# XiaoshuiHuang/GMF

Hardware: AMD Instinct MI355X
Metric: correspondences/sec (whole node) (higher is better)
Workload: dtype f32 (split-fp16 MFMA operands, fp32 accumulate; the cross products of the attention's two contractions, S = K Q'^T and O = P V, on block-scaled e4m3 operands wherever the device-side score guard allows)

## Files before the change

### gmf_amd/_lib.py

```python
from __future__ import annotations

import collections
import ctypes as C
import os
import threading
from typing import Dict, Optional

_HERE = os.path.dirname(os.path.abspath(__file__))
LIB_PATH = os.path.join(_HERE, "libgmf_hip.so")

_f32p = C.POINTER(C.c_float)
_i32p = C.POINTER(C.c_int)
_vp = C.c_void_p
_ll = C.c_longlong


class EncoderWeights(C.Structure):
    _fields_ = [
        ("num_layers", C.c_int),
        ("f1_ctx_wst", _vp), ("f1_ctx_vec", _vp),
        ("f1_attn_wst", _vp), ("f1_attn_vec", _vp),
        ("f1_ff_wst", _vp), ("f1_ff_vec", _vp),
        ("ctx_wst", _vp), ("ctx_vec", _vp), ("ctx_wst_stride", C.c_int), ("ctx_vec_stride", C.c_int),
        ("attn_wst", _vp), ("attn_vec", _vp), ("attn_wst_stride", C.c_int), ("attn_vec_stride", C.c_int),
# ... 76 lines not shown
    "gmf_last_error_string": (C.c_char_p, [_vp]),
    "gmf_workspace_bytes": (_ll, [_vp]),
    "gmf_set_workspace": (C.c_int, [_vp, _vp, _ll]),
    "gmf_workspace_wanted": (_ll, [_vp]),
    "gmf_status_read": (C.c_int, [_vp, C.POINTER(C.c_int), C.c_int]),
    "gmf_set_tuning": (C.c_int, [_vp, C.c_char_p, C.c_int]),
    "gmf_get_tuning": (C.c_int, [_vp, C.c_char_p, C.POINTER(C.c_int)]),
    "gmf_set_sigma_device": (C.c_int, [_vp, _vp]),
    "gmf_profile_enable": (C.c_int, [_vp, C.c_int]),
    "gmf_profile_read": (C.c_int, [_vp, C.POINTER(C.c_double), C.POINTER(C.c_int)]),
    "gmf_pack_rows_p32": (C.c_int, [_vp, _vp, _ll, _ll, _ll, C.c_int, C.c_int, C.c_int, _vp, _vp]),
    "gmf_unpack_rows_p32": (C.c_int, [_vp, _vp, C.c_int, C.c_int, C.c_int, _vp, _ll, _ll, _ll, _vp]),
    "gmf_pack_pts8": (C.c_int, [_vp, _vp, _vp, C.c_int, C.c_int, _vp, _vp]),
    "gmf_front_forward": (C.c_int, [_vp, C.c_int, _vp, _vp, _vp, _vp, _vp, _vp, _vp, C.c_int, C.c_int, _vp]),
    "gmf_scattn_forward": (C.c_int, [_vp, _vp, _vp, _vp, _vp, _vp, _vp, _vp, _vp, C.c_int, C.c_int, C.c_float, _vp]),
    "gmf_scattn_forward_dense": (C.c_int, [_vp, _vp, _vp, _vp, _vp, _vp, _vp, _vp, _vp, C.c_int, C.c_int, _vp]),
    "gmf_fusion_ctx_prepare": (C.c_int, [_vp, C.c_int, _vp, _vp, _vp, _vp, C.c_int, C.c_int, C.c_int, C.c_int, C.c_int, _vp]),
    "gmf_fusion_attn_forward": (C.c_int, [_vp, C.c_int, _vp, _vp, _vp, _vp, _vp, C.c_int, C.c_int, C.c_int, _vp]),
    "gmf_fusion_ff_forward": (C.c_int, [_vp, _vp, _vp, _vp, _vp, C.c_int, C.c_int, _vp]),
    "gmf_classifier_forward": (C.c_int, [_vp, _vp, _vp, _vp, _vp, _vp, _vp, C.c_int, C.c_int, _vp]),
    "gmf_encoder_pack_weights": (C.c_int, [_vp, C.POINTER(Tensor), C.c_int, C.c_int, C.c_int, C.POINTER(_vp)]),
    "gmf_packed_encoder_weights": (C.POINTER(EncoderWeights), [_vp]),
    "gmf_packed_encoder_info": (C.c_int, [_vp, _f32p, _f32p, _i32p, _f32p]),
    "gmf_packed_encoder_free": (None, [_vp]),
    "gmf_packed_encoder_bytes": (C.c_longlong, [_vp]),
    "gmf_packed_encoder_place": (C.c_int, [_vp, _vp, _vp, C.c_longlong, _vp]),
    "gmf_fusion_pack_weights": (C.c_int, [_vp, C.POINTER(Tensor), C.c_int, C.c_char_p, C.c_int, C.c_int, C.POINTER(_vp)]),
    "gmf_packed_fusion_weights": (C.POINTER(FusionWeights), [_vp]),
    "gmf_packed_fusion_free": (None, [_vp]),
    "gmf_packed_fusion_bytes": (C.c_longlong, [_vp]),
    "gmf_packed_fusion_place": (C.c_int, [_vp, _vp, _vp, C.c_longlong, _vp]),
    "gmf_encoder_forward": (C.c_int, [_vp, C.POINTER(EncoderWeights), _vp, _vp, _vp, _vp, _vp, C.c_int, C.c_int, C.c_int,
                                      _vp, _vp, _vp, _vp]),
    "gmf_encoder_forward_ragged": (C.c_int, [_vp, C.POINTER(EncoderWeights), _vp, _vp, _vp, _vp, _vp, _i32p, C.c_int, C.c_int,
                                             _vp, _vp, _vp, _vp]),
    "gmf_pose_head_ragged": (C.c_int, [_vp, C.POINTER(PoseParams), C.c_double, _vp, _vp, _vp, _vp, _i32p, C.c_int, _vp, _vp, _vp,
                                       _vp, _vp, _vp, _vp]),
    "gmf_nonlocal_block_forward": (C.c_int, [_vp, C.POINTER(EncoderWeights), C.c_int, C.c_int, _vp, _vp, _vp, _vp, _vp,
                                             C.c_int, C.c_int, C.c_int, _vp]),
    "gmf_fusion_layer_forward": (C.c_int, [_vp, C.c_int, C.c_int, C.c_int, _vp, _vp, _vp, _vp, _vp, _vp, _vp, _vp, _ll, _ll,
                                           _ll, _vp, _ll, _ll, _ll, C.c_int, C.c_int, C.c_int, _vp, _vp, _vp, _vp]),
    "gmf_pose_head": (C.c_int, [_vp, C.POINTER(PoseParams), _vp, _vp, _vp, _vp, _vp, C.c_int, C.c_int, _vp, _vp, _vp,
                                _vp, _vp, _vp, _vp]),
    "gmf_pick_seeds": (C.c_int, [_vp, _vp, _vp, C.c_int, C.c_int, C.c_float, C.c_int, C.c_int, _vp, _vp]),
    "gmf_knn_rows": (C.c_int, [_vp, _vp, _vp, C.c_int, C.c_int, C.c_int, C.c_int, _vp, _vp]),
    "gmf_knn_from_distances": (C.c_int, [_vp, _vp, C.c_int, C.c_int, C.c_int, C.c_int, _vp, _vp]),
    "gmf_nn_match": (C.c_int, [_vp, _vp, _vp, C.c_int, C.c_int, C.c_int, C.c_int, _vp, _vp, _vp]),
    "gmf_nn_match_batched": (C.c_int, [_vp, _vp, _vp, _i32p, _i32p, C.c_int, C.c_int, C.c_int, C.c_int, _vp, _vp, _vp]),
    "gmf_nn_match_mutual_batched": (C.c_int, [_vp, _vp, _vp, _i32p, _i32p, C.c_int, C.c_int, _vp, _vp, _vp, _vp]),
    "gmf_build_correspondences": (C.c_int, [_vp, _vp, _vp, _vp, _vp, _i32p, _i32p, C.c_int, C.c_int, C.c_int, C.c_int, _vp, C.c_float,
                                            _vp, _vp, _vp, _vp, _vp, _vp, _vp, _vp, _vp]),
    "gmf_matching_indices_count": (C.c_int, [_vp, _vp, _vp, _vp, _vp, C.c_int, _ll, _ll, _vp, C.c_double, _vp, _vp, C.POINTER(_ll), _vp]),
    "gmf_matching_indices_fill": (C.c_int, [_vp, _vp, _vp, _vp, _vp, C.c_int, _ll, _ll, _vp, C.c_double, _vp, _vp, _vp]),
    "gmf_inlier_input": (C.c_int, [_vp, _vp, _vp, _vp, _vp, C.c_int, _ll, _vp, _vp, _vp, _vp, C.c_int, _vp, _vp, C.c_int, _vp, _vp, _vp,
                                   _vp, _vp, _vp]),
    "gmf_procrustes_batched": (C.c_int, [_vp, _vp, _vp, _vp, C.c_int, C.c_int, C.c_float, _vp, _vp]),
    "gmf_post_refinement": (C.c_int, [_vp, _vp, _vp, _vp, C.c_int, C.c_int, C.c_float, C.c_int, _vp, _vp]),
    "gmf_weighted_procrustes": (C.c_int, [_vp, _vp, _vp, _vp, _vp, C.c_int, C.c_float, _vp, _vp, _vp]),
    "gmf_global_registration": (C.c_int, [_vp, _vp, _vp, _vp, _vp, C.c_int, C.c_float, C.c_float, C.c_int, C.c_int,
                                          C.c_double, _vp, _vp, _vp, C.c_int, _vp]),
    "gmf_similarity_matrix": (C.c_int, [_vp, _vp, C.c_int, C.c_int, C.c_float, _vp, C.c_int, _vp]),
    "gmf_spectral_matching_loss": (C.c_int, [_vp, _vp, C.c_int, _vp, C.c_int, C.c_int, C.c_int, _vp, _vp]),
    "gmf_spectral_matching_loss_fused": (C.c_int, [_vp, _vp, _vp, C.c_int, C.c_int, C.c_float, C.c_int, _vp, _vp]),
    "gmf_spectral_matching_backward": (C.c_int, [_vp, _vp, _vp, C.c_int, C.c_int, C.c_float, C.c_int, _vp, _vp, _vp]),
    "gmf_classification_loss": (C.c_int, [_vp, _vp, _vp, _vp, C.c_int, C.c_int, C.c_int, _vp, _vp]),
    "gmf_stem_forward": (C.c_int, [_vp, _vp, _ll, _ll, _ll, _ll, _vp, _vp, _vp, C.c_int, C.c_int, C.c_int, _vp]),
# ... 228 lines not shown
```

### gmf_amd/csrc/encoder_kernels.hip

```cpp
#include <algorithm>
#include <type_traits>
#include "enc_common.hpp"
#include "enc_ff.hpp"

namespace gmf {

template <int MODE>
__global__ void __launch_bounds__(256, 2)
k_front(const float* __restrict__ in, const float* __restrict__ wst, const float* __restrict__ vecs,
        float* __restrict__ f_out, float* __restrict__ q_out, float* __restrict__ k_out,
        float* __restrict__ v_out, int N, int tiles) {
  __shared__ __attribute__((aligned(16))) float lds[2 * kStageFloats];
  const int lane = threadIdx.x & 63, wave = threadIdx.x >> 6, h = lane >> 5, i = lane & 31;
  const int pair = blockIdx.y;
  const int tile_raw = blockIdx.x * kWavesPerWG + wave;
  const bool active = tile_raw < tiles;
  const int tile = active ? tile_raw : tiles - 1;
  const size_t toff = ((size_t)pair * tiles + tile) * (32 * C);

  constexpr bool FIRST = (MODE == 1);
  StageStream ss;
  if (MODE == 2) ss.init(lds, lds + kStageFloats, wave, kWavesPerWG, lane, wst + 4 * kStageFloats, 12);
  else ss.init(lds, lds + kStageFloats, wave, kWavesPerWG, lane, wst, 16);
  ss.prime();
// ... 424 lines not shown
               const PairTab* __restrict__ ptab) {
  __shared__ float tr[kCompatLdsFloats];
  compat_build_body<FMT>(tr, blockIdx.x, blockIdx.y, blockIdx.z, pts8, c_dense, N, tiles, inv_sig2, ptab);
}

GMF_DEVINL f32x16 mma3_part(int u, f32x16 acc, f16x8 ah, f16x8 al, f16x8 bh, f16x8 bl) {
  switch (u) {
    case 0: return mfma_h16(al, bh, acc);
    case 1: return mfma_h16(ah, bl, acc);
    default: return mfma_h16(ah, bh, acc);
  }
}


struct FusTile {
  const float* tile;
  GMF_DEVINL void load(float (&fz)[16], int mb, int lane, int h) const { load_block_p32(fz, tile, mb, lane); }
};

struct FusRegs {
  const float (&f)[CF];
  GMF_DEVINL void load(float (&fz)[16], int mb, int lane, int h) const {
#pragma unroll
    for (int r = 0; r < 16; ++r) fz[r] = f[16 * mb + r];
  }
};

constexpr int kTailVecFloats = 3 * C;
GMF_DEVINL void stage_tail_vecs(float* lvec, const float* __restrict__ vecs, const float* __restrict__ next_bias, int wave, int lane) {
  if (wave == 0) dma_piece_1k(vecs, lvec, lane);
  if (wave == 1 && next_bias && lane < 32) dma_piece_1k(next_bias, lvec + 2 * C, lane);
}

template <bool NEXT_PCN, class Stages, class Fus>
GMF_DEVINL void scattn_epilogue_h2(const float (&o)[CF], const bool active, Stages& ss, const float* __restrict__ vecs,
                                   const Fus& fus_tile, float* __restrict__ out_tile, const int lane, const int h,
                                   const float* __restrict__ next_bias = nullptr,
                                   unsigned* __restrict__ stat_next = nullptr, const int pair = 0, const bool row_valid = false) {
    FragH2<8> ox, featx;
    FragH2<4> m1x, m2x;
    if (active) ox.set(o);
#pragma unroll
    for (int mb = 0; mb < 2; ++mb) {
      const f16x8* lw = as_h2(ss.acquire());
      if (!active) continue;
      f32x16 acc = zero16();
      mma_wx_h2<8>(acc, lw, ox);
      float b[16], t1[16];
      load_vec_block(b, vecs, mb, h);
#pragma unroll
      for (int r = 0; r < 16; ++r) t1[r] = relu_nan(fmaf(acc[r], kH2Inv, b[r]));
      m1x.set_block(mb, t1);
    }
    {
      const f16x8* lw = as_h2(ss.acquire());
#pragma unroll
      for (int mb = 0; mb < 2; ++mb) {
        if (!active) continue;
        f32x16 acc = zero16();
        mma_wx_h2<4>(acc, lw + mb * (2 * 4 * 64), m1x);
        float b[16], t2[16];
        load_vec_block(b, vecs + 64, mb, h);
#pragma unroll
        for (int r = 0; r < 16; ++r) t2[r] = relu_nan(fmaf(acc[r], kH2Inv, b[r]));
        m2x.set_block(mb, t2);
      }
    }
#pragma unroll
    for (int st = 0; st < 2; ++st) {
      const f16x8* lw = as_h2(ss.acquire());
#pragma unroll
      for (int hb = 0; hb < 2; ++hb) {
        if (!active) continue;
        const int mb = 2 * st + hb;
        f32x16 acc = zero16();
        mma_wx_h2<4>(acc, lw + hb * (2 * 4 * 64), m2x);
        float b[16], fz[16], tt[16];
        load_vec_block(b, vecs + 128, mb, h);
        fus_tile.load(fz, mb, lane, h);
#pragma unroll
        for (int r = 0; r < 16; ++r) tt[r] = fmaf(acc[r], kH2Inv, b[r]) + fz[r];
        if (NEXT_PCN) featx.set_block(mb, tt);
        else if (active) store_block_p32(out_tile, mb, tt, lane);
      }
    }
    if (NEXT_PCN) {
      float ssq = 0.f;
#pragma unroll
      for (int mb = 0; mb < 4; ++mb) {
        const f16x8* lw = as_h2(ss.acquire());
        if (!active) continue;
        f32x16 acc = zero16();
        mma_wx_h2<8>(acc, lw, featx);
        float b[16], tt[16];
        load_vec_block(b, next_bias, mb, h);
#pragma unroll
        for (int r = 0; r < 16; ++r) { tt[r] = relu_nan(fmaf(acc[r], kH2Inv, b[r])); ssq = fmaf(tt[r], tt[r], ssq); }
        store_block_p32(out_tile, mb, tt, lane);
      }
      if (stat_next && active) pv_stat_raise(stat_next, pair, ssq, row_valid, lane);
    }
}

struct AttnItem { int item, ks; bool split, valid; };
GMF_DEVINL AttnItem attn_item(int L, int n_items, int n_full, int ksplits) {
  const int chunk = n_items >> 3, rem = n_items & 7, xcd = L & 7, kth = L >> 3;
  const int start = (xcd < rem) ? xcd * (chunk + 1) : rem * (chunk + 1) + (xcd - rem) * chunk;
  const int items = chunk + (xcd < rem ? 1 : 0);
  const int nf = min(n_full, items);
  if (kth < nf) return AttnItem{start + kth, 0, false, true};
  const int j = kth - nf, r = j / ksplits;
  return AttnItem{start + nf + r, j - r * ksplits, true, nf + r < items};
}

constexpr float kInvU16 = 1.0f / 65535.0f;
template <int NPROD = 3, int CFMT = 0, int WAVES = 4, bool PVF8 = false>
GMF_DEVINL void scattn_h2p_body(float* lds, const int bid, const float* __restrict__ q_img, const float* __restrict__ k_img,
                                const float* __restrict__ v_img, const float* __restrict__ fus, const float* __restrict__ wst,
                                const float* __restrict__ vecs, float* out, int N, int tiles, int wgs_per_pair,
                                const float* __restrict__ c_dense, int n_items, int n_full, int ksplits,
                                float* __restrict__ part_o, float* __restrict__ part_ml, const float* __restrict__ next_wst,
                                const float* __restrict__ next_bias, const PairTab* __restrict__ ptab = nullptr,
                                const unsigned* __restrict__ v_scale = nullptr,
                                const float* qf_img = nullptr, const float* __restrict__ qw_wst = nullptr,
                                const float* __restrict__ qw_bias = nullptr,
                                unsigned* __restrict__ stat_next = nullptr) {
  static_assert(!PVF8 || NPROD == 3, "the fp8 cross products belong to the three-product form");
  float* const ldsK = lds;
  float* const ldsV = lds + 2 * kStageFloats;
  const int lane = threadIdx.x & 63, h = lane >> 5;
  const int wave = __builtin_amdgcn_readfirstlane(threadIdx.x >> 6);
  const unsigned lane_off16 = lane * 16;
  const AttnItem it = attn_item(bid, n_items, n_full, ksplits);
  if (!it.valid) return;
  const bool split = it.split;
  const int ks = it.ks;
  const int slot = it.item / wgs_per_pair, qblock = it.item - slot * wgs_per_pair;
  const int pair = ptab ? ptab[slot].ord : slot;
  if (ptab) N = ptab[pair].n;
  const int tiles_p = ptab ? (N + 31) >> 5 : tiles;
  if (qblock * WAVES >= tiles_p) return;
  const int t_begin = split ? (tiles_p * ks) / ksplits : 0;
  const int t_end = split ? (tiles_p * (ks + 1)) / ksplits : tiles_p;
  const int tile_raw = qblock * WAVES + wave;
  const bool active = tile_raw < tiles_p;
  const int tile = active ? tile_raw : tiles_p - 1;
  const size_t pbase = (size_t)pair * tiles;
  const size_t toff = (pbase + tile) * (32 * C);

  f16x8 qh[8], ql[8];
  if (NPROD == 3 && WAVES == 4 && qf_img) {
    FragH2<8> fx;
    {
      float fq[CF];
      load_frag_p32<CF>(fq, qf_img + toff, lane);
      fx.set(fq);
    }
#pragma unroll
    for (int st = 0; st < 4; ++st) dma_4k_s(qw_wst + st * kStageFloats + wave * 1024, lds + st * kStageFloats + wave * 1024, lane_off16);
    asm volatile("s_waitcnt vmcnt(0)" ::: "memory");
// ... 418 lines not shown
      tile_step(t, s_a, s_b);
      tile_step(t + 1, s_b, s_a);
    }
    if (t + 1 < t_end) { tile_step(t, s_a, s_b); tile_last(t + 1, s_b); }
    else tile_last(t, s_a);
    }
  }
  if (split) {
    if (active) {
      float of[CF];
#pragma unroll
      for (int db = 0; db < 4; ++db)
#pragma unroll
        for (int r = 0; r < 16; ++r) of[16 * db + r] = oacc[db][r];
      const size_t n_tiles_all = (size_t)(n_items / wgs_per_pair) * tiles;
      const size_t pt = (size_t)ks * n_tiles_all + pbase + tile;
      store_frag_p32<CF>(part_o + pt * (32 * C), of, lane);
      const float lsum = xhalf_sum(l_half);
      if (h == 0) { part_ml[(pt * 32 + (lane & 31)) * 2] = m_run; part_ml[(pt * 32 + (lane & 31)) * 2 + 1] = lsum; }
    }
    return;
  }

  float o[CF];
  {
    const float inv = 1.0f / xhalf_sum(l_half);
#pragma unroll
    for (int db = 0; db < 4; ++db)
#pragma unroll
      for (int r = 0; r < 16; ++r) o[16 * db + r] = oacc[db][r] * inv;
  }
  __syncthreads();
  float* const lvec = lds + 2 * kStageFloats;
  stage_tail_vecs(lvec, vecs, next_wst ? next_bias : nullptr, wave, lane);
  StageStream ss;
  ss.init(lds, lds + kStageFloats, wave, WAVES, lane, wst, 5, next_wst, next_wst ? 4 : 0);
  ss.prime();
  const FusTile ft{fus + toff};
  if (next_wst) scattn_epilogue_h2<true>(o, active, ss, lvec, ft, out + toff, lane, h, lvec + 2 * C, stat_next, pair,
                                         tile_raw * 32 + (lane & 31) < N);
  else scattn_epilogue_h2<false>(o, active, ss, lvec, ft, out + toff, lane, h);
}

GMF_DEVINL bool attn_pv_on(const unsigned* __restrict__ v_scale, const PvGuard& guard, int bid, int n_items, int n_full, int ksplits,
                           int wgs_per_pair, const PairTab* __restrict__ ptab = nullptr) {
  if (!guard.stat) return v_scale != nullptr;
  const AttnItem it = attn_item(bid, n_items, n_full, ksplits);
  const int slot = it.valid ? it.item / wgs_per_pair : 0;
  return pv_planes_on(v_scale, guard, ptab ? ptab[slot].ord : slot);
}

template <int NPROD, int CFMT, bool PVF8 = false>
__global__ void __launch_bounds__(256, 2)
k_scattn_h2p(const float* __restrict__ q_img, const float* __restrict__ k_img, const float* __restrict__ v_img,
             const float* __restrict__ fus, const float* __restrict__ wst, const float* __restrict__ vecs,
             float* out, int N, int tiles, int wgs_per_pair, const float* __restrict__ c_dense,
             int n_items, int n_full, int ksplits, float* __restrict__ part_o, float* __restrict__ part_ml,
             const float* __restrict__ next_wst, const float* __restrict__ next_bias, const PairTab* __restrict__ ptab,
             const unsigned* __restrict__ v_scale, const float* qf_img, const float* __restrict__ qw_wst,
             const float* __restrict__ qw_bias, const PvGuard guard) {
  __shared__ __attribute__((aligned(16))) float lds[4 * kStageFloats];
  tail_priority(blockIdx.x, gridDim.x);
  if (!PVF8 || attn_pv_on(v_scale, guard, blockIdx.x, n_items, n_full, ksplits, wgs_per_pair, ptab))
    scattn_h2p_body<NPROD, CFMT, 4, PVF8>(lds, blockIdx.x, q_img, k_img, v_img, fus, wst, vecs, out, N, tiles, wgs_per_pair, c_dense, n_items,
                                          n_full, ksplits, part_o, part_ml, next_wst, next_bias, ptab, v_scale, qf_img, qw_wst, qw_bias,
                                          guard.stat_next);
  else
    scattn_h2p_body<NPROD, CFMT, 4, false>(lds, blockIdx.x, q_img, k_img, v_img, fus, wst, vecs, out, N, tiles, wgs_per_pair, c_dense, n_items,
                                           n_full, ksplits, part_o, part_ml, next_wst, next_bias, ptab, nullptr, qf_img, qw_wst, qw_bias,
                                           guard.stat_next);
}

__global__ void __launch_bounds__(256, 2)
k_scattn_fast(const float* __restrict__ q_img, const float* __restrict__ k_img, const float* __restrict__ v_img,
              const float* __restrict__ fus, const float* __restrict__ wst, const float* __restrict__ vecs,
              float* __restrict__ out, int N, int tiles, int wgs_per_pair, const float* __restrict__ c_half, int n_items,
              const float* __restrict__ next_wst, const float* __restrict__ next_bias) {
  constexpr int WAVES = 4;
  constexpr int kHiFloats = kStageFloats / 2;
  constexpr int kCFloats = 512;
  __shared__ __attribute__((aligned(16))) float lds[6 * kHiFloats + WAVES * 3 * kCFloats];
  float* const ldsK = lds;
  float* const ldsV = lds + 3 * kHiFloats;
  const int lane = threadIdx.x & 63, h = lane >> 5;
  const int wave = __builtin_amdgcn_readfirstlane(threadIdx.x >> 6);
  float* const ldsC = lds + 6 * kHiFloats + wave * 3 * kCFloats;
  const unsigned lane_off16 = lane * 16;
  const AttnItem it = attn_item(blockIdx.x, n_items, 0x7fffffff, 1);
  if (!it.valid) return;
  const int pair = it.item / wgs_per_pair, qblock = it.item - pair * wgs_per_pair;
  const int tile_raw = qblock * WAVES + wave;
  const bool active = tile_raw < tiles;
  const int tile = active ? tile_raw : tiles - 1;
  const size_t pbase = (size_t)pair * tiles;
  const size_t toff = (pbase + tile) * (32 * C);

  f16x8 qh[8];
  {
    const f16x8* qp = reinterpret_cast<const f16x8*>(q_img + (pbase + tile) * (size_t)kStageFloats) + lane;
#pragma unroll
    for (int s = 0; s < 8; ++s) qh[s] = qp[s * 64];
  }
  const float* gc = c_half + ((pbase + tile) * (size_t)tiles) * kCFloats;
// ... 121 lines not shown
  if (next_wst) scattn_epilogue_h2<true>(o, active, ss, lvec, ft, out + toff, lane, h, lvec + 2 * C);
  else scattn_epilogue_h2<false>(o, active, ss, lvec, ft, out + toff, lane, h);
}

template <int CFMT, bool PVF8 = false>
__global__ void __launch_bounds__(256, 2)
k_small_attn_ff(const int n_attn, const float* __restrict__ q_img, const float* __restrict__ k_img,
                const float* __restrict__ v_img, const float* __restrict__ tail_wst, const float* __restrict__ tail_vecs, int N,
                int tiles, int wgs_per_pair, const float* __restrict__ c_dense, int n_items, int ksplits,
                float* __restrict__ part_o, float* __restrict__ part_ml, const float* __restrict__ x1,
                const float* __restrict__ ff_wst, const float* __restrict__ ff_vecs, float* __restrict__ ff_part, int n_pairs,
                int ff_hs, const unsigned* __restrict__ v_scale, const PvGuard guard,
                const PairTab* __restrict__ ptab) {
  __shared__ __attribute__((aligned(16))) float lds[4 * kStageFloats];
  if ((int)blockIdx.x < n_attn) {
    if (!PVF8 || attn_pv_on(v_scale, guard, blockIdx.x, n_items, 0, ksplits, wgs_per_pair, ptab))
      scattn_h2p_body<3, CFMT, 4, PVF8>(lds, blockIdx.x, q_img, k_img, v_img, x1, tail_wst, tail_vecs, ff_part, N, tiles, wgs_per_pair, c_dense,
                                        n_items, 0, ksplits, part_o, part_ml, nullptr, nullptr, ptab, v_scale);
    else
      scattn_h2p_body<3, CFMT, 4, false>(lds, blockIdx.x, q_img, k_img, v_img, x1, tail_wst, tail_vecs, ff_part, N, tiles, wgs_per_pair, c_dense,
                                         n_items, 0, ksplits, part_o, part_ml, nullptr, nullptr, ptab, nullptr);
  } else {
    const int id = (int)blockIdx.x - n_attn;
    const int z = id % ff_hs, r = id / ff_hs;
    const int pair = r / wgs_per_pair, bx = r - pair * wgs_per_pair;
    if (ptab && bx * 4 >= ((ptab[pair].n + 31) >> 5)) return;
    fusion_ff_h2p_body<true>(lds, bx, pair, n_pairs, z, ff_hs, x1, ff_wst, ff_vecs, ff_part, tiles, ff_part);
  }
}

struct StagesPreloaded {
  const float* base;
  int used, lane;
  GMF_DEVINL void init(float* lds, int wave, int lane_, const float* g, int n_stages, const float* g2 = nullptr) {
    base = lds; used = 0; lane = lane_;
    for (int st = 0; st < n_stages; ++st)
#pragma unroll
      for (int q = 0; q < 4; ++q)
        dma_piece_1k(g + (size_t)st * kStageFloats + (wave + 4 * q) * 256, lds + st * kStageFloats + (wave + 4 * q) * 256, lane_);
    if (g2)
      for (int st = 0; st < 4; ++st)
#pragma unroll
        for (int q = 0; q < 4; ++q)
          dma_piece_1k(g2 + (size_t)st * kStageFloats + (wave + 4 * q) * 256, lds + (n_stages + st) * kStageFloats + (wave + 4 * q) * 256, lane_);
  }
  GMF_DEVINL const float4* acquire() {
    if (used == 0) {
      asm volatile("s_waitcnt vmcnt(0)" ::: "memory");
      __syncthreads();
    }
    const float* cur = base + used * kStageFloats;
    ++used;
    return reinterpret_cast<const float4*>(cur) + lane;
  }
};

__global__ void __launch_bounds__(256, 1)
k_scattn_merge(const float* __restrict__ part_o, const float* __restrict__ part_ml, const float* __restrict__ fus,
               const float* __restrict__ wst, const float* __restrict__ vecs, float* __restrict__ out, int tiles,
               int wgs_per_pair, int n_items, int n_full, int ksplits, const float* __restrict__ next_wst,
               const float* __restrict__ next_bias, const float* __restrict__ ff_part, int ff_hs, const float* __restrict__ x1,
               const float* __restrict__ ff_b2, unsigned* __restrict__ stat_next, int n_rows,
               const PairTab* __restrict__ ptab = nullptr) {
  __shared__ __attribute__((aligned(16))) float lds[9 * kStageFloats + kTailVecFloats];
  const int lane = threadIdx.x & 63, h = lane >> 5, i = lane & 31;
  const int wave = __builtin_amdgcn_readfirstlane(threadIdx.x >> 6);
  const AttnItem it = attn_item(blockIdx.x + 8 * min(n_full, (n_items >> 3) + ((int)(blockIdx.x & 7) < (n_items & 7) ? 1 : 0)),
                                n_items, n_full, 1);
  if (!it.valid) return;
  const int slot = it.item / wgs_per_pair;
  const int pair = ptab ? ptab[slot].ord : slot;
  if (ptab) n_rows = ptab[pair].n;
  const int tiles_p = ptab ? (n_rows + 31) >> 5 : tiles;
  if ((it.item - slot * wgs_per_pair) * 4 >= tiles_p) return;
  const int tile_raw = (it.item - slot * wgs_per_pair) * 4 + wave;
  const bool active = tile_raw < tiles_p;
  const int tile = active ? tile_raw : tiles_p - 1;
  const size_t n_tiles_all = (size_t)(n_items / wgs_per_pair) * tiles;
  const size_t pt0 = (size_t)pair * tiles + tile;
  const size_t toff = pt0 * (32 * C);
  float* const lvec = lds + 9 * kStageFloats;
  stage_tail_vecs(lvec, vecs, next_wst ? next_bias : nullptr, wave, lane);
  vecs = lvec;
  next_bias = lvec + 2 * C;
  StagesPreloaded ss;
  ss.init(lds, wave, lane, wst, 5, next_wst);
  float x2[CF];
  if (ff_part) {
    const float* pt = ff_part + toff;
    const size_t zs = n_tiles_all * (32 * C);
    float acc[CF], xr[CF];
    load_frag_p32<CF>(acc, pt, lane);
    load_frag_p32<CF>(xr, x1 + toff, lane);
    for (int z = 1; z < ff_hs; ++z) {
      float pz[CF];
      load_frag_p32<CF>(pz, pt + (size_t)z * zs, lane);
#pragma unroll
      for (int e = 0; e < CF; ++e) acc[e] += pz[e];
    }
#pragma unroll
    for (int mb = 0; mb < 4; ++mb) {
      float b[16];
      load_vec_block(b, ff_b2, mb, h);
#pragma unroll
      for (int r = 0; r < 16; ++r) x2[16 * mb + r] = fmaf(acc[16 * mb + r], kH2Inv, b[r]) + xr[16 * mb + r];
    }
  }
  float mk[8], lk[8];
  float M = -INFINITY;
#pragma unroll
  for (int k = 0; k < 8; ++k) {
    mk[k] = -INFINITY; lk[k] = 0.f;
    if (k < ksplits) {
      const float2 ml = *reinterpret_cast<const float2*>(part_ml + ((k * n_tiles_all + pt0) * 32 + i) * 2);
      mk[k] = ml.x; lk[k] = ml.y;
    }
  }
#pragma unroll
  for (int k = 0; k < 8; ++k) M = fmaxf(M, mk[k]);
  float o[CF];
#pragma unroll
  for (int e = 0; e < CF; ++e) o[e] = 0.f;
  float l = 0.f;
#pragma unroll
  for (int k0 = 0; k0 < 8; k0 += 4) {
    if (k0 >= ksplits) break;
    float ok[4][CF];
#pragma unroll
    for (int j = 0; j < 4; ++j)
      if (k0 + j < ksplits) load_frag_p32<CF>(ok[j], part_o + ((k0 + j) * n_tiles_all + pt0) * (32 * C), lane);
#pragma unroll
    for (int j = 0; j < 4; ++j) {
      if (k0 + j < ksplits) {
        const float wk = __builtin_amdgcn_exp2f(mk[k0 + j] - M);
        l = fmaf(lk[k0 + j], wk, l);
#pragma unroll
        for (int e = 0; e < CF; ++e) o[e] = fmaf(ok[j][e], wk, o[e]);
      }
    }
  }
  const float inv = 1.0f / l;
#pragma unroll
  for (int e = 0; e < CF; ++e) o[e] *= inv;
  if (ff_part) {
    const FusRegs fp{x2};
    if (next_wst) scattn_epilogue_h2<true>(o, active, ss, vecs, fp, out + toff, lane, h, next_bias, stat_next, pair, tile_raw * 32 + i < n_rows);
    else scattn_epilogue_h2<false>(o, active, ss, vecs, fp, out + toff, lane, h);
    return;
  }
  const FusTile ft{fus + toff};
  if (next_wst) scattn_epilogue_h2<true>(o, active, ss, vecs, ft, out + toff, lane, h, next_bias, stat_next, pair, tile_raw * 32 + i < n_rows);
  else scattn_epilogue_h2<false>(o, active, ss, vecs, ft, out + toff, lane, h);
}

__global__ void __launch_bounds__(256, 1)
k_scattn_merge_tile(const float* __restrict__ part_o, const float* __restrict__ part_ml, const float* __restrict__ wst,
                    const float* __restrict__ vecs, float* __restrict__ out, int tiles, int ksplits,
                    const float* __restrict__ next_wst, const float* __restrict__ next_bias, const float* __restrict__ ff_part,
                    int ff_hs, const float* __restrict__ x1, const float* __restrict__ ff_b2, unsigned* __restrict__ stat_next,
                    int n_rows,
                    const PairTab* __restrict__ ptab) {
  __shared__ __attribute__((aligned(16))) float lds[10 * kStageFloats];
  const int lane = threadIdx.x & 63, h = lane >> 5, i = lane & 31;
  const int wave = __builtin_amdgcn_readfirstlane(threadIdx.x >> 6);
  const int tile = blockIdx.x, pair = blockIdx.y;
  if (ptab) {
    n_rows = ptab[pair].n;
    if (tile >= ((n_rows + 31) >> 5)) return;
  }
  const size_t n_tiles_all = (size_t)gridDim.y * tiles;
  const size_t pt0 = (size_t)pair * tiles + tile;
  const size_t toff = pt0 * (32 * C);
  float* const xch = lds + 9 * kStageFloats;
  f16x8* const xh = reinterpret_cast<f16x8*>(xch);
  StagesPreloaded ss;
  ss.init(lds, wave, lane, wst, 5, next_wst);
// ... 383 lines not shown
  float w3[16];
  load_vec_block(w3, vecs + 64, 0, h);
  float part = 0.f;
#pragma unroll
  for (int r = 0; r < 16; ++r) part = fmaf(h2[r], w3[r], part);
  const float logit = xhalf_sum(part) + vecs[96];

  float ss2 = 0.f;
#pragma unroll
  for (int k = 0; k < CF; ++k) ss2 = fmaf(x[k], x[k], ss2);
  const float nrm2 = xhalf_sum(ss2);
  const bool bad_row = not_finite(nrm2);
  flag_status(status, active && row < N && (not_finite(logit) || bad_row), 1);
  const float inv = 1.0f / fmaxf(sqrtf(nrm2), 1e-12f);

  if (active && row < N) {
    const size_t ro = row0 + row;
    if (h == 0) logits[ro] = logit;
    float4* pn = reinterpret_cast<float4*>(feat_n + ro * C) + h;
#pragma unroll
    for (int g = 0; g < CF / 4; ++g)
      pn[2 * g] = bad_row ? make_float4(0.f, 0.f, 0.f, 0.f)
                          : make_float4(x[4 * g] * inv, x[4 * g + 1] * inv, x[4 * g + 2] * inv, x[4 * g + 3] * inv);
    if (feat_rm) {
      float4* pr = reinterpret_cast<float4*>(feat_rm + ro * C) + h;
#pragma unroll
      for (int g = 0; g < CF / 4; ++g) pr[2 * g] = make_float4(x[4 * g], x[4 * g + 1], x[4 * g + 2], x[4 * g + 3]);
    }
  }
}

__global__ void __launch_bounds__(256, 2)
k_seed_dist(const float* __restrict__ featn_img, const int* __restrict__ seeds, float* __restrict__ dist,
            int N, int tiles, int S, int chunks, const PairTab* __restrict__ ptab) {
  __shared__ __attribute__((aligned(16))) float lds[4 * kStageFloats];
  const int lane = threadIdx.x & 63, h = lane >> 5, i = lane & 31;
  const int wave = __builtin_amdgcn_readfirstlane(threadIdx.x >> 6);
  const int pair = blockIdx.y / chunks, chunk = blockIdx.y - pair * chunks;
  const int Nmax = N, Smax = S;
  N = pair_rows(ptab, pair, N);
  S = ptab ? ptab[pair].S : S;
  const int tiles_p = (N + 31) >> 5;
  if ((int)blockIdx.x * kWavesPerWG * 32 >= S) return;
  const int per = (tiles_p + chunks - 1) / chunks;
  const int t0 = chunk * per, t1 = min(tiles_p, t0 + per);
  const int seed_base = (blockIdx.x * kWavesPerWG + wave) * 32;
  const float* pair_img = featn_img + (size_t)pair * tiles * (32 * C);
  const int my = seed_base + i;
  const int row = (my < S) ? seeds[(size_t)pair * Smax + my] : 0;
  if (t0 >= t1) return;
  FragH2<8> sx;
  {
    const f16x8* rp = reinterpret_cast<const f16x8*>(pair_img + (size_t)(row >> 5) * kStageFloats) + h * 32 + (row & 31);
#pragma unroll
    for (int s8 = 0; s8 < 8; ++s8) { sx.h[s8] = rp[(0 * 8 + s8) * 64]; sx.l[s8] = rp[(1 * 8 + s8) * 64]; }
  }

  StageRing<4> ss;
  ss.init(lds, wave, lane, pair_img + (size_t)t0 * kStageFloats, t1 - t0);
  ss.prime();
  const int ld = tiles * 32;
  float* drow = dist + ((size_t)pair * Smax + seed_base + i) * ld + 4 * h;
  for (int t = t0; t < t1; ++t) {
    const f16x8* lk = as_h2(ss.acquire());
    f32x16 acc = zero16();
#pragma unroll
    for (int s8 = 0; s8 < 8; ++s8) {
      const f16x8 kh = lk[(0 * 8 + s8) * 64], kl = lk[(1 * 8 + s8) * 64];
// ... 112 lines not shown
}

hipError_t launch_scattn_fp32(const float* q, const float* k, const float* v, const float* pts8, const float* fus,
                              const float* wst, const float* vecs, float* out, int B, int N, int tiles, float sigma_d,
                              hipStream_t s) {
  hipLaunchKernelGGL(k_scattn<false>, tile_grid(tiles, B), dim3(256), 0, s, q, k, v, pts8, fus, wst, vecs, out, N, tiles,
                     1.0f / (sigma_d * sigma_d));
  return hipGetLastError();
}

hipError_t launch_small_attn_ff_merge(const float* q, const float* k, const float* v, const float* x1, const float* ff_wst,
                                      const float* ff_vecs, float* ff_part, int ff_hs, const float* tail_vecs, float* out, int B,
                                      int N, int tiles, int ksplits, hipStream_t s, const CompatCache* cc, bool tile_merge) {
  const int wpp = (tiles + 3) / 4, W = wpp * B;
  const int per_xcd = (W >> 3) + ((W & 7) ? 1 : 0);
  const int n_attn = 8 * per_xcd * ksplits, n_ff = W * ff_hs;
  if (cc->fmt == 2 && cc->v_scale)
    hipLaunchKernelGGL((k_small_attn_ff<2, true>), dim3(n_attn + n_ff), dim3(256), 0, s, n_attn, q, k, v, cc->tail_wst_h2, tail_vecs, N, tiles, wpp,
                       cc->dense, W, ksplits, cc->part_o, cc->part_ml, x1, ff_wst, ff_vecs, ff_part, B, ff_hs, cc->v_scale, cc->guard, cc->ptab);
  else if (cc->fmt == 2)
    hipLaunchKernelGGL(k_small_attn_ff<2>, dim3(n_attn + n_ff), dim3(256), 0, s, n_attn, q, k, v, cc->tail_wst_h2, tail_vecs, N, tiles, wpp,
                       cc->dense, W, ksplits, cc->part_o, cc->part_ml, x1, ff_wst, ff_vecs, ff_part, B, ff_hs, (const unsigned*)nullptr, PvGuard{}, cc->ptab);
  else if (cc->v_scale)
    hipLaunchKernelGGL((k_small_attn_ff<0, true>), dim3(n_attn + n_ff), dim3(256), 0, s, n_attn, q, k, v, cc->tail_wst_h2, tail_vecs, N, tiles, wpp,
                       cc->dense, W, ksplits, cc->part_o, cc->part_ml, x1, ff_wst, ff_vecs, ff_part, B, ff_hs, cc->v_scale, cc->guard, cc->ptab);
  else
    hipLaunchKernelGGL(k_small_attn_ff<0>, dim3(n_attn + n_ff), dim3(256), 0, s, n_attn, q, k, v, cc->tail_wst_h2, tail_vecs, N, tiles, wpp,
                       cc->dense, W, ksplits, cc->part_o, cc->part_ml, x1, ff_wst, ff_vecs, ff_part, B, ff_hs, (const unsigned*)nullptr, PvGuard{}, cc->ptab);
  if (tile_merge)
    hipLaunchKernelGGL(k_scattn_merge_tile, dim3(tiles, B), dim3(256), 0, s, cc->part_o, cc->part_ml, cc->tail_wst_h2, tail_vecs, out,
                       tiles, ksplits, cc->next_wst_h2, cc->next_bias, (const float*)ff_part, ff_hs, x1, ff_vecs + 2 * C + 2 * FFH,
                       cc->guard.stat_next, N, cc->ptab);
  else
    hipLaunchKernelGGL(k_scattn_merge, dim3(8 * per_xcd), dim3(256), 0, s, cc->part_o, cc->part_ml, x1, cc->tail_wst_h2, tail_vecs, out,
                       tiles, wpp, W, 0, ksplits, cc->next_wst_h2, cc->next_bias, (const float*)ff_part, ff_hs, x1,
                       ff_vecs + 2 * C + 2 * FFH, cc->guard.stat_next, N, cc->ptab);
  return hipGetLastError();
}

hipError_t launch_scattn_h2p(const float* q, const float* k, const float* v, const float* fus, const float* vecs, float* out, int B,
                             int N, int tiles, hipStream_t s, const CompatCache& cc, int n_full, int ksplits) {
  const int wpp = (tiles + 3) / 4, W = wpp * B;
  const int per_xcd = (W >> 3) + ((W & 7) ? 1 : 0);
  const int max_tail = std::max(0, per_xcd - n_full);
  const dim3 grid(8 * (std::min(n_full, per_xcd) + max_tail * ksplits));
  if (cc.half && max_tail == 0)
    hipLaunchKernelGGL(k_scattn_fast, dim3(8 * per_xcd), dim3(256), 0, s, q, k, v, fus, cc.tail_wst_h2, vecs, out, N, tiles, wpp, cc.dense, W,
                       cc.next_wst_h2, cc.next_bias);
  else if (cc.half)
    hipLaunchKernelGGL((k_scattn_h2p<1, 1>), grid, dim3(256), 0, s, q, k, v, fus, cc.tail_wst_h2, vecs, out, N, tiles, wpp, cc.dense, W,
                       n_full, ksplits, cc.part_o, cc.part_ml, cc.next_wst_h2, cc.next_bias, cc.ptab, (const unsigned*)nullptr, (const float*)nullptr, (const float*)nullptr, (const float*)nullptr, PvGuard{});
  else if (cc.fmt == 2 && cc.v_scale)
    hipLaunchKernelGGL((k_scattn_h2p<3, 2, true>), grid, dim3(256), 0, s, q, k, v, fus, cc.tail_wst_h2, vecs, out, N, tiles, wpp, cc.dense,
                       W, n_full, ksplits, cc.part_o, cc.part_ml, cc.next_wst_h2, cc.next_bias, cc.ptab, cc.v_scale, cc.qf_img, cc.qw_wst, cc.qw_bias, cc.guard);
  else if (cc.fmt == 2)
    hipLaunchKernelGGL((k_scattn_h2p<3, 2>), grid, dim3(256), 0, s, q, k, v, fus, cc.tail_wst_h2, vecs, out, N, tiles, wpp, cc.dense,
                       W, n_full, ksplits, cc.part_o, cc.part_ml, cc.next_wst_h2, cc.next_bias, cc.ptab, (const unsigned*)nullptr, cc.qf_img, cc.qw_wst, cc.qw_bias, PvGuard{});
  else if (cc.v_scale)
    hipLaunchKernelGGL((k_scattn_h2p<3, 0, true>), grid, dim3(256), 0, s, q, k, v, fus, cc.tail_wst_h2, vecs, out, N, tiles, wpp, cc.dense,
                       W, n_full, ksplits, cc.part_o, cc.part_ml, cc.next_wst_h2, cc.next_bias, cc.ptab, cc.v_scale, cc.qf_img, cc.qw_wst, cc.qw_bias, cc.guard);
  else
    hipLaunchKernelGGL((k_scattn_h2p<3, 0>), grid, dim3(256), 0, s, q, k, v, fus, cc.tail_wst_h2, vecs, out, N, tiles, wpp, cc.dense,
                       W, n_full, ksplits, cc.part_o, cc.part_ml, cc.next_wst_h2, cc.next_bias, cc.ptab, (const unsigned*)nullptr, cc.qf_img, cc.qw_wst, cc.qw_bias, PvGuard{});
  if (max_tail > 0)
    hipLaunchKernelGGL(k_scattn_merge, dim3(8 * max_tail), dim3(256), 0, s, cc.part_o, cc.part_ml, fus, cc.tail_wst_h2, vecs, out,
                       tiles, wpp, W, n_full, ksplits, cc.next_wst_h2, cc.next_bias, (const float*)nullptr, 0,
                       (const float*)nullptr, (const float*)nullptr, cc.guard.stat_next, N, cc.ptab);
  return hipGetLastError();
}

hipError_t launch_scattn_h2(const float* q, const float* k, const float* v, const float* pts8, const float* fus, const float* wst,
                            const float* vecs, float* out, int B, int N, int tiles, float sigma_d, hipStream_t s, const float* c_dense) {
  const float inv = 1.0f / (sigma_d * sigma_d);
  const int wpp = (tiles + 3) / 4;
  if (c_dense) hipLaunchKernelGGL(k_scattn_h2<true>, dim3(wpp * B), dim3(256), 0, s, q, k, v, pts8, fus, wst, vecs, out, N, tiles, inv, wpp, c_dense);
  else hipLaunchKernelGGL(k_scattn_h2<false>, dim3(wpp * B), dim3(256), 0, s, q, k, v, pts8, fus, wst, vecs, out, N, tiles, inv, wpp, c_dense);
  return hipGetLastError();
}

hipError_t launch_scattn_dense(const float* q, const float* k, const float* v, const float* compat, const float* fus,
                               const float* wst, const float* vecs, float* out, int B, int N, int tiles, hipStream_t s) {
  hipLaunchKernelGGL(k_scattn<true>, tile_grid(tiles, B), dim3(256), 0, s, q, k, v, compat, fus, wst, vecs, out, N, tiles, 0.f);
  return hipGetLastError();
}

hipError_t launch_ctx_prep(bool pe, const float* ctx, const float* wst, const float* vecs, float* out, int B, int T,
                           int ttiles, int sets, int wst_stride, int vec_stride, hipStream_t s) {
  if (pe) hipLaunchKernelGGL(k_ctx_prep<true>, tile_grid(ttiles, B, sets), dim3(256), 0, s, ctx, wst, vecs, out, T, ttiles, wst_stride, vec_stride);
  else hipLaunchKernelGGL(k_ctx_prep<false>, tile_grid(ttiles, B, sets), dim3(256), 0, s, ctx, wst, vecs, out, T, ttiles, wst_stride, vec_stride);
  return hipGetLastError();
}

hipError_t launch_fusion_attn(bool pe, const float* x, const float* ctx_img, const float* wst, const float* vecs,
                              float* x1, int B, int N, int tiles, int T, int ttiles, hipStream_t s) {
  if (pe) hipLaunchKernelGGL(k_fusion_attn<true>, tile_grid(tiles, B), dim3(256), 0, s, x, ctx_img, wst, vecs, x1, N, tiles, T, ttiles);
  else hipLaunchKernelGGL(k_fusion_attn<false>, tile_grid(tiles, B), dim3(256), 0, s, x, ctx_img, wst, vecs, x1, N, tiles, T, ttiles);
  return hipGetLastError();
}

hipError_t launch_fusion_ff(const float* x1, const float* wst, const float* vecs, float* x2, int B, int tiles, hipStream_t s) {
  hipLaunchKernelGGL(k_fusion_ff, tile_grid(tiles, B), dim3(256), 0, s, x1, wst, vecs, x2, tiles);
  return hipGetLastError();
}

hipError_t launch_head(const float* feat_img, const float* wst, const float* vecs, float* logits, float* feat_n,
                       float* feat_rm, int B, int N, int tiles, hipStream_t s, int* status, const PairTab* ptab, const unsigned* pv_stat,
                       const float* pv_thr2, int n_layers) {
  hipLaunchKernelGGL(k_head, tile_grid(tiles, B), dim3(256), 0, s, feat_img, wst, vecs, logits, feat_n, feat_rm, N, tiles, status, ptab,
                     pv_stat, pv_thr2, n_layers);
  return hipGetLastError();
}

hipError_t launch_seed_dist(const float* featn_img, const int* seeds, float* dist, int B, int N, int S, hipStream_t s, const PairTab* ptab) {
  const int tiles = (N + 31) / 32;
  const int sblocks = (S + 127) / 128;
  int chunks = 1;
  while (chunks < 16 && sblocks * B * chunks < 1024 && tiles / (2 * chunks) >= 4) chunks *= 2;
  hipLaunchKernelGGL(k_seed_dist, dim3(sblocks, B * chunks), dim3(256), 0, s, featn_img, seeds, dist, N, tiles, S, chunks, ptab);
  return hipGetLastError();
}

hipError_t launch_pack_p32(const float* src, float* dst, int B, int n_rows, int K, long sb, long sr, long sk, hipStream_t s, const PairTab* ptab) {
  const int tiles = (n_rows + 31) / 32;
  const long total4 = (long)B * tiles * (K / 8) * 64;
  hipLaunchKernelGGL(k_pack_p32, dim3((unsigned)((total4 + 255) / 256)), dim3(256), 0, s, src, dst, n_rows, tiles, K, sb, sr, sk, total4, ptab);
  return hipGetLastError();
}

hipError_t launch_pack_rows_h2(const float* src, float* dst, int B, int n_rows, hipStream_t s, const PairTab* ptab, const float* copy_src,
                               float* copy_dst, long n_copy) {
  const int tiles = (n_rows + 31) / 32;
  const long total = (long)B * tiles * 8 * 64;
  if (!copy_src || !copy_dst) n_copy = 0;
  if (n_copy > total) return hipErrorInvalidValue;
  hipLaunchKernelGGL(k_pack_rows_h2, dim3((unsigned)((total + 255) / 256)), dim3(256), 0, s, src, dst, n_rows, tiles, total, ptab, copy_src,
                     copy_dst, n_copy);
  return hipGetLastError();
}

hipError_t launch_unpack_p32(const float* src, float* dst, int B, int n_rows, int K, long sb, long sr, long sk, hipStream_t s, int* status) {
  const int tiles = (n_rows + 31) / 32;
  const long total4 = (long)B * tiles * (K / 8) * 64;
  hipLaunchKernelGGL(k_unpack_p32, dim3((unsigned)((total4 + 255) / 256)), dim3(256), 0, s, src, dst, n_rows, tiles, K, sb, sr, sk, total4, status);
  return hipGetLastError();
}

hipError_t launch_pack_pts8(const float* src, const float* tgt, float* dst, int B, int N, hipStream_t s, const PairTab* ptab,
                            unsigned* zero_words, int n_zero) {
  const int Npad = ((N + 31) / 32) * 32;
  const long total = (long)B * Npad;
  hipLaunchKernelGGL(k_pack_pts8, dim3((unsigned)((std::max(total, (long)n_zero) + 255) / 256)), dim3(256), 0, s, src, tgt, dst, N, Npad, total, ptab,
// ... 6 lines not shown
```

### gmf_amd/csrc/gmf_api.cpp

```cpp
#include "../../include/gmf_hip.h"

#include <hip/hip_runtime.h>

#include <cmath>
#include <cstdint>
#include <cstdio>
#include <algorithm>
#include <cstring>
#include <new>
#include <string>
#include <utility>
#include <vector>

#include "api_common.hpp"
#include "launchers_pose.hpp"
#include "launchers_solvers.hpp"
#include "launchers_spectral.hpp"
#include "launchers_pointcloud.hpp"
#include "launchers_sparse.hpp"
#include "launchers_dgr_input.hpp"
#include "launchers_correspondence.hpp"
#include "launchers_posegraph.hpp"

namespace {
// ... 195 lines not shown
    t.wide_attn_tile = value != 0;
    return GMF_OK;
  }
  if (std::strcmp(name, "small_merge_tile") == 0) {
    GMF_REQUIRE(value == 0 || value == 1, GMF_ERR_BAD_ARG, "set_tuning: small_merge_tile must be 0 or 1");
    t.small_merge_tile = value != 0;
    return GMF_OK;
  }
  if (std::strcmp(name, "mid_grid_roles") == 0) {
    GMF_REQUIRE(value >= 0 && value <= 4096, GMF_ERR_BAD_ARG, "set_tuning: mid_grid_roles out of range (0..4096)");
    t.mid_grid_roles = value;
    return GMF_OK;
  }
  if (std::strcmp(name, "q_in_attention") == 0) {
    GMF_REQUIRE(value == 0 || value == 1, GMF_ERR_BAD_ARG, "set_tuning: q_in_attention must be 0 or 1");
    t.q_in_attention = value != 0;
    return GMF_OK;
  }
  if (std::strcmp(name, "pv_fp8") == 0) {
    GMF_REQUIRE(value >= 0 && value <= 2, GMF_ERR_BAD_ARG, "set_tuning: pv_fp8 must be 0 (three f16 products), 1 (guarded, default) or 2 (always)");
    t.pv_fp8 = value;
    return GMF_OK;
  }
  if (std::strcmp(name, "compat_format") == 0) {
    GMF_REQUIRE(value == 0 || value == 2, GMF_ERR_BAD_ARG, "set_tuning: compat_format must be 0 (fp32) or 2 (16-bit fixed point of c)");
    t.compat_format = value;
    return GMF_OK;
  }
  if (std::strcmp(name, "precision") == 0) {
    GMF_REQUIRE(value >= 0 && value <= 2, GMF_ERR_BAD_ARG, "set_tuning: precision must be 0 (parity), 1 or 2 (throughput numerics)");
    t.precision = value;
    return GMF_OK;
  }
  if (std::strcmp(name, "spectral_col_splits") == 0) {
    GMF_REQUIRE(value >= 0 && value <= gmf::kSmMaxSplits, GMF_ERR_BAD_ARG, "set_tuning: spectral_col_splits out of range (0..32)");
    t.spectral_col_splits = value;
    return GMF_OK;
  }
  return fail(h, GMF_ERR_BAD_ARG, std::string("gmf: set_tuning: unknown knob ") + name);
}

int gmf_get_tuning(gmf_handle* h, const char* name, int* value) {
  GMF_REQUIRE(h && name && value, GMF_ERR_BAD_ARG, "get_tuning: null pointer");
  std::lock_guard<std::mutex> lock(h->mu);
  const gmf::Tuning& t = h->tune;
  const struct { const char* name; int v; } tab[] = {
      {"scattn_variant", t.scattn_variant}, {"front_output_split", t.front_split ? 1 : 0}, {"ff_hidden_splits", t.ff_split},
      {"attn_key_splits", t.key_splits}, {"attn_tail_split", t.tail_split ? 1 : 0}, {"small_grid_roles", t.small_roles ? 1 : 0},
      {"fused_linear", t.fused_linear ? 1 : 0}, {"compat_cache", t.use_cache ? 1 : 0}, {"conv_lds_patch", t.conv_patch}, {"conv_small_grid", t.conv_small ? 1 : 0}, {"small_prologue_roles", t.small_prologue ? 1 : 0}, {"small_fattn_tile", t.small_fattn_tile ? 1 : 0},
      {"nms_binned", t.nms_binned}, {"topk_select", t.topk_select ? 1 : 0}, {"wide_attn_tile", t.wide_attn_tile ? 1 : 0},
      {"small_merge_tile", t.small_merge_tile ? 1 : 0}, {"mid_grid_roles", t.mid_grid_roles}, {"pv_fp8", t.pv_fp8}, {"q_in_attention", t.q_in_attention ? 1 : 0},
      {"compat_format", t.compat_format}, {"precision", t.precision}, {"spectral_col_splits", t.spectral_col_splits}};
  for (const auto& e : tab) {
    if (std::strcmp(name, e.name) == 0) { *value = e.v; return GMF_OK; }
  }
  return fail(h, GMF_ERR_BAD_ARG, std::string("gmf: get_tuning: unknown knob ") + name);
}

int gmf_profile_enable(gmf_handle* h, int on) {
  GMF_REQUIRE(h, GMF_ERR_BAD_ARG, "profile_enable: null handle");
  h->profile = (on != 0);
  h->prof_used = 0;
  return GMF_OK;
}

int gmf_profile_read(gmf_handle* h, double* scattn_ms_total, int* scattn_launches) {
  GMF_REQUIRE(h && scattn_ms_total && scattn_launches, GMF_ERR_BAD_ARG, "profile_read: null pointer");
  SetDevice sd(h);
  double total = 0.0;
  for (size_t i = 0; i < h->prof_used; ++i) {
    GMF_HIP(hipEventSynchronize(h->prof_events[i].second));
    float ms = 0.f;
    GMF_HIP(hipEventElapsedTime(&ms, h->prof_events[i].first, h->prof_events[i].second));
    total += ms;
  }
  *scattn_ms_total = total;
  *scattn_launches = (int)h->prof_used;
  h->prof_used = 0;
  return GMF_OK;
}

void gmf_destroy(gmf_handle* h) {
  if (!h) return;
  for (auto& e : h->prof_events) { (void)hipEventDestroy(e.first); (void)hipEventDestroy(e.second); }
  int prev = -1;
// ... 313 lines not shown
    std::stable_sort(by_len.begin(), by_len.end(), [&](int a, int c) { return n_points[a] > n_points[c]; });
    const int runs = B < 8 ? 1 : 8;
    std::vector<std::vector<int>> run(runs);
    std::vector<double> load(runs, 0.0);
    std::vector<int> cap(runs);
    for (int r = 0; r < runs; ++r) cap[r] = B / runs + (r < B % runs ? 1 : 0);
    for (int b : by_len) {
      int best = -1;
      for (int r = 0; r < runs; ++r)
        if ((int)run[r].size() < cap[r] && (best < 0 || load[r] < load[best])) best = r;
      run[best].push_back(b);
      load[best] += (double)n_points[b] * (double)n_points[b];
    }
    int slot_i = 0;
    for (int r = 0; r < runs; ++r)
      for (int b : run[r]) tab[slot_i++].ord = b;
  }
  *n_max = nm;
  *n_sum = row;
  if (s_max) *s_max = sm;
  return GMF_OK;
}

static int upload_pair_table(gmf_handle* h, gmf::PairTab* dtab, int B, hipStream_t st) {
  gmf_handle::PtabSlot& slot = h->ptab_ring[h->ptab_cur];
  GMF_HIP(hipMemcpyAsync(dtab, slot.host, (size_t)B * sizeof(gmf::PairTab), hipMemcpyHostToDevice, st));
  GMF_HIP(hipEventRecord(slot.ev, st));
  slot.pending = true;
  return GMF_OK;
}

static int encoder_forward_impl(gmf_handle* h, const gmf_encoder_weights* w, const float* corr_pos, const float* src_keypts,
                                const float* tgt_keypts, const float* p_tokens, const float* q_tokens, int B, int N, int T,
                                float* logits, float* feat_n, float* feat, gmf_stream_t stream, const int* n_points);

int gmf_encoder_forward(gmf_handle* h, const gmf_encoder_weights* w, const float* corr_pos, const float* src_keypts,
                        const float* tgt_keypts, const float* p_tokens, const float* q_tokens, int B, int N, int T,
                        float* logits, float* feat_n, float* feat, gmf_stream_t stream) {
  GMF_REQUIRE(h, GMF_ERR_BAD_ARG, "encoder_forward: null handle");
  GMF_REQUIRE(B > 0 && N > 0 && T > 0, GMF_ERR_UNSUPPORTED_SHAPE, "encoder_forward: empty input");
  return encoder_forward_impl(h, w, corr_pos, src_keypts, tgt_keypts, p_tokens, q_tokens, B, N, T, logits, feat_n, feat, stream, nullptr);
}

int gmf_encoder_forward_ragged(gmf_handle* h, const gmf_encoder_weights* w, const float* corr_pos, const float* src_keypts,
                               const float* tgt_keypts, const float* p_tokens, const float* q_tokens, const int* n_points, int B,
                               int T, float* logits, float* feat_n, float* feat, gmf_stream_t stream) {
  GMF_REQUIRE(h, GMF_ERR_BAD_ARG, "encoder_forward_ragged: null handle");
  GMF_REQUIRE(n_points, GMF_ERR_BAD_ARG, "encoder_forward_ragged: null n_points");
  GMF_REQUIRE(B > 0 && T > 0, GMF_ERR_UNSUPPORTED_SHAPE, "encoder_forward_ragged: empty input");
  return encoder_forward_impl(h, w, corr_pos, src_keypts, tgt_keypts, p_tokens, q_tokens, B, 0, T, logits, feat_n, feat, stream, n_points);
}

static int encoder_forward_impl(gmf_handle* h, const gmf_encoder_weights* w, const float* corr_pos, const float* src_keypts,
                                const float* tgt_keypts, const float* p_tokens, const float* q_tokens, int B, int N, int T,
                                float* logits, float* feat_n, float* feat, gmf_stream_t stream, const int* n_points) {
  if (int rc = check_weights(h, w)) return rc;
  GMF_REQUIRE(corr_pos && src_keypts && tgt_keypts && p_tokens && q_tokens && logits && feat_n, GMF_ERR_BAD_ARG,
              "encoder_forward: null pointer");
  SetDevice sd(h, stream);
  hipStream_t st = S(stream);
  const bool ragged = n_points != nullptr;
  int min_tiles = 0;
  if (ragged) {
    long long n_sum = 0;
    if (int rc = build_pair_table(h, n_points, B, -1.0, 0, &N, &n_sum, nullptr)) return rc;
    min_tiles = tiles_of(*std::min_element(n_points, n_points + B));
  }
  const int L = w->num_layers;
  const int tiles = tiles_of(N), tt = tiles_of(T);
  const EncoderPlan p = plan_encoder(h->tune, w, B, N, T, L, min_tiles, cu_count());
  GMF_REQUIRE(p.fused() || !ragged, GMF_ERR_UNSUPPORTED_SHAPE,
              "encoder_forward_ragged: ragged batches run on the default path only (split-fp16 weight images, at least two layers, the "
              "compat cache, \"fused_linear\" = 1, \"scattn_variant\" = 18)");
  const size_t act = p.act, tok = p.tok;
  gmf::PairTab* ptab;
  float *featA, *featB, *f, *q, *k, *v, *x1, *x2, *pts8, *pimg, *qimg, *f1ctx, *x1t, *imgfeat, *ctxall, *c_dense, *ff_part, *part_o,
      *part_ml;
  unsigned *v_scale, *fstat;
  if (int rc = arena_carve(h, {arena_buf(ptab, ragged ? (size_t)B : 0), arena_buf(featA, act), arena_buf(featB, act), arena_buf(f, act),
                               arena_buf(q, act), arena_buf(k, act), arena_buf(v, act), arena_buf(x1, act), arena_buf(x2, act),
                               arena_buf(pts8, (size_t)B * tiles * 32 * 8), arena_buf(pimg, tok), arena_buf(qimg, tok),
                               arena_buf(f1ctx, tok), arena_buf(x1t, tok), arena_buf(imgfeat, tok),
                               arena_buf(ctxall, (size_t)(L > 0 ? L : 1) * tok),
                               arena_buf(v_scale, (size_t)B * tiles * 128),
                               arena_buf(fstat, (size_t)(L + 1) * B * gmf::kPvStatStride),
                               arena_buf(c_dense, p.cache_floats),
                               arena_buf(ff_part, p.max_splits == 8 ? 8 * act : 0),
                               arena_buf(part_o, p.max_splits * act),
// ... 12 lines not shown
                                    zero_words, n_zero));
    GMF_HIP(gmf::launch_pro_fattn_compat(q_tokens, f1ctx, w->f1_attn_wst_h2, w->f1_attn_vec, x1t, B, T, tt, pts8, c_dense, N, tiles,
                                         w->sigma_d, st, ptab));
    gmf::PvGuard g0;
    if (p.guard) g0.stat_next = fstat;
    GMF_HIP(gmf::launch_pro_ff_front(x1t, w->f1_ff_wst_h2, w->f1_ff_vec, imgfeat, B, tt, part_o, p.f1_ff_hs, corr_pos, w->front_wst_h2,
                                     w->front_vec, f, q, k, v, N, tiles, st, ptab, g0));
    if (p.f1_ff_hs > 1) GMF_HIP(gmf::launch_ff_reduce_h2(part_o, x1t, w->f1_ff_vec, imgfeat, B, tt, p.f1_ff_hs, st));
    GMF_HIP(gmf::launch_ctx_prep_h2(true, imgfeat, w->ctx_wst_h2, w->ctx_vec, ctxall, B, T, tt, L, w->ctx_wst_stride, w->ctx_vec_stride, st));
  } else {
    if (p.f1_h2) {
      GMF_HIP(gmf::launch_ctx_prep_h2(false, p_tokens, w->f1_ctx_wst_h2, w->f1_ctx_vec, f1ctx, B, T, tt, 1, 0, 0, st, true));
      GMF_HIP(gmf::launch_fusion_attn_h2(false, q_tokens, f1ctx, w->f1_attn_wst_h2, w->f1_attn_vec, x1t, B, T, tt, T, tt, st, true));
      GMF_HIP(gmf::launch_fusion_ff_h2(x1t, w->f1_ff_wst_h2, w->f1_ff_vec, imgfeat, B, tt, st, part_o, p.f1_ff_hs));
    } else {
      GMF_HIP(gmf::launch_pack_p32(p_tokens, pimg, B, T, kC, (long)T * kC, kC, 1, st));
      GMF_HIP(gmf::launch_pack_p32(q_tokens, qimg, B, T, kC, (long)T * kC, kC, 1, st));
      GMF_HIP(gmf::launch_ctx_prep(false, pimg, w->f1_ctx_wst, w->f1_ctx_vec, f1ctx, B, T, tt, 1, 0, 0, st));
      GMF_HIP(gmf::launch_fusion_attn(false, qimg, f1ctx, w->f1_attn_wst, w->f1_attn_vec, x1t, B, T, tt, T, tt, st));
      GMF_HIP(gmf::launch_fusion_ff(x1t, w->f1_ff_wst, w->f1_ff_vec, imgfeat, B, tt, st));
    }
    if (L > 0) {
      if (p.form != EncoderPlan::kFp32) GMF_HIP(gmf::launch_ctx_prep_h2(true, imgfeat, w->ctx_wst_h2, w->ctx_vec, ctxall, B, T, tt, L,
                                                                         w->ctx_wst_stride, w->ctx_vec_stride, st));
      else GMF_HIP(gmf::launch_ctx_prep(true, imgfeat, w->ctx_wst, w->ctx_vec, ctxall, B, T, tt, L, w->ctx_wst_stride,
                                        w->ctx_vec_stride, st));
    }
    GMF_HIP(gmf::launch_pack_pts8(src_keypts, tgt_keypts, pts8, B, N, st, ptab, zero_words, n_zero));
    if (p.cache) GMF_HIP(gmf::launch_compat_build(pts8, c_dense, B, N, tiles, w->sigma_d, p.fmt, st, ptab));
  }

  float* cur = featA;
  float* nxt = featB;
  if (p.fused()) {
    if (!p.prologue) {
      gmf::PvGuard g0;
      if (p.guard) g0.stat_next = fstat;
      GMF_HIP(gmf::launch_front_h2(3, p.front_split, corr_pos, w->front_wst_h2, w->front_vec, f, q, k, v, B, N, tiles, st, ptab, nullptr, g0));
    }
    for (int l = 0; l < L; ++l) {
      cc.guard = gmf::PvGuard{};
      if (p.guard) cc.guard = gmf::PvGuard{fstat + (size_t)l * B * gmf::kPvStatStride, w->pv_guard + l, fstat + (size_t)(l + 1) * B * gmf::kPvStatStride};
      const float* fw = w->front_wst_h2 + (size_t)l * w->front_wst_stride;
      const float* fv = w->front_vec + (size_t)l * w->front_vec_stride;
      const float* aw = w->attn_wst_h2 + (size_t)l * w->attn_wst_stride;
      const float* av = w->attn_vec + (size_t)l * w->attn_vec_stride;
      const float* ffw = w->ff_wst_h2 + (size_t)l * w->ff_wst_stride;
      const float* ffv = w->ff_vec + (size_t)l * w->ff_vec_stride;
      const float* ctx_l = ctxall + (size_t)l * tok;
      const bool last = (l + 1 == L);
      cc.tail_wst_h2 = w->tail_wst_h2 + (size_t)l * w->tail_wst_stride;
      cc.next_wst_h2 = last ? nullptr : w->front_wst_h2 + (size_t)(l + 1) * w->front_wst_stride;
      cc.next_bias = last ? nullptr : w->front_vec + (size_t)(l + 1) * w->front_vec_stride;
      if (p.form == EncoderPlan::kLinear) {
        cc.qf_img = p.q_in_attn ? f : nullptr;
        cc.qw_wst = p.q_in_attn ? fw + 4 * kTileFloats : nullptr;
        cc.qw_bias = p.q_in_attn ? fv + kC : nullptr;
        GMF_HIP(gmf::launch_linear_h2(p.roles, f, fw, fv, ctx_l, aw, av, ffw, ffv, p.q_in_attn ? nullptr : q, k, v, x2, B, N, tiles, T, tt,
                                      st, p.one_product, ptab, cc.v_scale, cc.guard));
      } else if (p.form == EncoderPlan::kSmall3) {
        GMF_HIP(gmf::launch_small_front_fattn(f, fw, fv, ctx_l, aw, av, q, k, v, x1, B, N, tiles, T, tt, st, cc.v_scale, cc.guard,
                                              h->tune.small_fattn_tile, ptab));
        hipEvent_t e0 = nullptr, e1 = nullptr;
        if (int rc = prof_begin(h, st, &e0, &e1)) return rc;
        GMF_HIP(gmf::launch_small_attn_ff_merge(q, k, v, x1, ffw, ffv, ff_part, p.ff_hs, w->tail_vec + (size_t)l * w->tail_vec_stride,
                                                last ? cur : f, B, N, tiles, p.attn_ks, st, &cc, h->tune.small_merge_tile));
        if (e1) GMF_HIP(hipEventRecord(e1, st));
        continue;
      } else {
        GMF_HIP(gmf::launch_front_h2(2, p.front_split, f, fw, fv, f, q, k, v, B, N, tiles, st, nullptr, cc.v_scale, cc.guard));
        GMF_HIP(gmf::launch_fusion_attn_h2(true, f, ctx_l, aw, av, x1, B, N, tiles, T, tt, st));
        GMF_HIP(gmf::launch_fusion_ff_h2(x1, ffw, ffv, x2, B, tiles, st, part_o, p.ff_hs));
      }
      if (int rc = run_scattn(h, w, p, l, q, k, v, pts8, x2, last ? cur : f, B, N, st, nullptr, cc)) return rc;
    }
    GMF_HIP(gmf::launch_head(cur, w->head_wst, w->head_vec, logits, feat_n, feat, B, N, tiles, st, h->status_dev, ptab,
                             p.guard ? fstat : nullptr, p.guard ? w->pv_guard : nullptr, L));
    return GMF_OK;
  }
  if (L == 0) {
    GMF_HIP(gmf::launch_front(1, corr_pos, w->front_wst, w->front_vec, cur, q, k, v, B, N, tiles, st));
  }
  for (int l = 0; l < L; ++l) {
    const float* in = (l == 0) ? corr_pos : cur;
    if (p.form == EncoderPlan::kStages)
      GMF_HIP(gmf::launch_front_h2(l == 0 ? 1 : 0, p.front_split, in, w->front_wst_h2 + (size_t)l * w->front_wst_stride,
                                   w->front_vec + (size_t)l * w->front_vec_stride, f, q, k, v, B, N, tiles, st));
    else GMF_HIP(gmf::launch_front(l == 0 ? 1 : 0, in, w->front_wst + (size_t)l * w->front_wst_stride,
                                   w->front_vec + (size_t)l * w->front_vec_stride, f, q, k, v, B, N, tiles, st));
    cc.tail_wst_h2 = w->tail_wst_h2 ? w->tail_wst_h2 + (size_t)l * w->tail_wst_stride : nullptr;
    if (int rc = run_block_tail(h, w, p, l, f, q, k, v, pts8, ctxall + (size_t)l * tok, x1, x2, nxt, B, N, T, st, nullptr, cc)) return rc;
    float* t = cur; cur = nxt; nxt = t;
  }
  GMF_HIP(gmf::launch_head(cur, w->head_wst, w->head_vec, logits, feat_n, feat, B, N, tiles, st, h->status_dev));
  return GMF_OK;
}

int gmf_nonlocal_block_forward(gmf_handle* h, const gmf_encoder_weights* w, int layer, int apply_pointcn,
                               const float* feat_img, const float* pts8, const float* attention,
                               const float* image_feat_img, float* out_img, int B, int N, int T, gmf_stream_t stream) {
  GMF_REQUIRE(h, GMF_ERR_BAD_ARG, "nonlocal_block_forward: null handle");
  if (int rc = check_weights(h, w)) return rc;
  GMF_REQUIRE(feat_img && image_feat_img && out_img, GMF_ERR_BAD_ARG, "nonlocal_block_forward: null pointer");
  GMF_REQUIRE((pts8 != nullptr) != (attention != nullptr), GMF_ERR_BAD_ARG, "nonlocal_block_forward: pass exactly one of pts8 / attention");
  GMF_REQUIRE(layer >= 0 && layer < w->num_layers, GMF_ERR_BAD_ARG, "nonlocal_block_forward: layer out of range");
  GMF_REQUIRE(B > 0 && N > 0 && T > 0, GMF_ERR_UNSUPPORTED_SHAPE, "nonlocal_block_forward: empty input");
  GMF_REQUIRE(apply_pointcn == 0 || apply_pointcn == 1, GMF_ERR_BAD_ARG, "nonlocal_block_forward: bad flag");
  SetDevice sd(h, stream);
  hipStream_t st = S(stream);
  const int tiles = tiles_of(N), tt = tiles_of(T);
  const EncoderPlan p = plan_encoder(h->tune, w, B, N, T, 1, 0, cu_count(), attention != nullptr);
  float *f, *q, *k, *v, *x1, *x2, *ctx;
  if (int rc = arena_carve(h, {arena_buf(f, p.act), arena_buf(q, p.act), arena_buf(k, p.act), arena_buf(v, p.act), arena_buf(x1, p.act),
                               arena_buf(x2, p.act), arena_buf(ctx, p.tok)}))
    return rc;
  if (p.form == EncoderPlan::kStages) {
    GMF_HIP(gmf::launch_front_h2(apply_pointcn ? 0 : 2, p.front_split, feat_img, w->front_wst_h2 + (size_t)layer * w->front_wst_stride,
                                 w->front_vec + (size_t)layer * w->front_vec_stride, f, q, k, v, B, N, tiles, st));
    GMF_HIP(gmf::launch_ctx_prep_h2(true, image_feat_img, w->ctx_wst_h2 + (size_t)layer * w->ctx_wst_stride,
                                    w->ctx_vec + (size_t)layer * w->ctx_vec_stride, ctx, B, T, tt, 1, 0, 0, st));
  } else {
    GMF_HIP(gmf::launch_front(apply_pointcn ? 0 : 2, feat_img, w->front_wst + (size_t)layer * w->front_wst_stride,
                              w->front_vec + (size_t)layer * w->front_vec_stride, f, q, k, v, B, N, tiles, st));
    GMF_HIP(gmf::launch_ctx_prep(true, image_feat_img, w->ctx_wst + (size_t)layer * w->ctx_wst_stride,
                                 w->ctx_vec + (size_t)layer * w->ctx_vec_stride, ctx, B, T, tt, 1, 0, 0, st));
  }
  gmf::CompatCache cc{nullptr, w->tail_wst_h2 ? w->tail_wst_h2 + (size_t)layer * w->tail_wst_stride : nullptr, nullptr, nullptr};
  return run_block_tail(h, w, p, layer, f, q, k, v, pts8, ctx, x1, x2, out_img, B, N, T, st, attention, cc);
// ... 49 lines not shown
    if (ff_wst_h2 && ff_hs_w > 1) {
      GMF_HIP(gmf::launch_fusion_ff_w_h2(x1, ff_wst_h2, ff_vec, x2, B, tiles, st, ff_part_w, ff_hs_w, out, o_sb, o_sr, o_sk, N, h->status_dev));
      return GMF_OK;
    }
    if (ff_wst_h2) GMF_HIP(gmf::launch_fusion_ff_w_h2(x1, ff_wst_h2, ff_vec, x2, B, tiles, st, ff_part_w, ff_hs_w));
    else GMF_HIP(gmf::launch_fusion_ff_w(x1, ff_wst, ff_vec, x2, B, tiles, st));
  }
  GMF_HIP(gmf::launch_unpack_p32(x2, out, B, N, latent_dim, o_sb, o_sr, o_sk, st, h->status_dev));
  return GMF_OK;
}

int gmf_pick_seeds(gmf_handle* h, const float* src_keypts, const float* scores, int B, int N, float nms_radius,
                   int use_nms, int num_seeds, int* seeds_out, gmf_stream_t stream) {
  GMF_REQUIRE(h && src_keypts && scores && seeds_out, GMF_ERR_BAD_ARG, "pick_seeds: null pointer");
  GMF_REQUIRE(B > 0 && N > 0 && num_seeds > 0 && num_seeds <= N, GMF_ERR_UNSUPPORTED_SHAPE, "pick_seeds: need 0 < num_seeds <= N");
  GMF_REQUIRE((size_t)num_seeds * 8 <= 156 * 1024, GMF_ERR_UNSUPPORTED_SHAPE, "pick_seeds: more than 19968 seeds (the winners' list lives in the LDS)");
  SetDevice sd(h, stream);
  hipStream_t st = S(stream);
  const float* keys = scores;
  float *kbuf, *scr;
  if (int rc = arena_carve(h, {arena_buf(kbuf, use_nms ? (size_t)B * N : 0), arena_buf(scr, use_nms ? gmf::nms_scratch_floats(B, N) : 0)}))
    return rc;
  if (use_nms) {
    GMF_HIP(gmf::launch_nms_keys(h->tune, src_keypts, scores, kbuf, B, N, nms_radius, st, scr));
    keys = kbuf;
  }
  GMF_HIP(gmf::launch_sort_topk(h->tune, keys, seeds_out, B, N, num_seeds, st));
  return GMF_OK;
}

static int pose_head_impl(gmf_handle* h, const gmf_pose_params* p, const float* feat_n, const float* src_keypts,
                          const float* tgt_keypts, const float* logits, const int* seeds_in, int B, int N, float* final_trans,
                          float* final_labels, int* seeds_out, int* knn_out, float* seed_trans, float* fitness,
                          gmf_stream_t stream, const int* n_points, double ratio);

int gmf_pose_head(gmf_handle* h, const gmf_pose_params* p, const float* feat_n, const float* src_keypts,
                  const float* tgt_keypts, const float* logits, const int* seeds_in, int B, int N, float* final_trans,
                  float* final_labels, int* seeds_out, int* knn_out, float* seed_trans, float* fitness,
                  gmf_stream_t stream) {
  GMF_REQUIRE(h && p, GMF_ERR_BAD_ARG, "pose_head: null pointer");
  GMF_REQUIRE(B > 0 && N > 1, GMF_ERR_UNSUPPORTED_SHAPE, "pose_head: need N > 1");
  return pose_head_impl(h, p, feat_n, src_keypts, tgt_keypts, logits, seeds_in, B, N, final_trans, final_labels, seeds_out, knn_out,
                        seed_trans, fitness, stream, nullptr, 0.0);
}

int gmf_pose_head_ragged(gmf_handle* h, const gmf_pose_params* p, double ratio, const float* feat_n, const float* src_keypts,
                         const float* tgt_keypts, const float* logits, const int* n_points, int B, float* final_trans,
                         float* final_labels, int* seeds_out, int* knn_out, float* seed_trans, float* fitness,
                         gmf_stream_t stream) {
  GMF_REQUIRE(h && p && n_points, GMF_ERR_BAD_ARG, "pose_head_ragged: null pointer");
  GMF_REQUIRE(B > 0, GMF_ERR_UNSUPPORTED_SHAPE, "pose_head_ragged: empty batch");
  GMF_REQUIRE(ratio > 0.0 && ratio <= 1.0, GMF_ERR_BAD_ARG, "pose_head_ragged: ratio must be in (0, 1]");
  GMF_REQUIRE(logits, GMF_ERR_BAD_ARG, "pose_head_ragged: the seeds come from the logits (no caller-provided seeds)");
  return pose_head_impl(h, p, feat_n, src_keypts, tgt_keypts, logits, nullptr, B, 0, final_trans, final_labels, seeds_out, knn_out,
                        seed_trans, fitness, stream, n_points, ratio);
}

static int pose_head_impl(gmf_handle* h, const gmf_pose_params* p, const float* feat_n, const float* src_keypts,
                          const float* tgt_keypts, const float* logits, const int* seeds_in, int B, int N, float* final_trans,
                          float* final_labels, int* seeds_out, int* knn_out, float* seed_trans, float* fitness,
                          gmf_stream_t stream, const int* n_points, double ratio) {
  GMF_REQUIRE(feat_n && src_keypts && tgt_keypts && final_trans && final_labels, GMF_ERR_BAD_ARG, "pose_head: null pointer");
  GMF_REQUIRE(seeds_in || logits, GMF_ERR_BAD_ARG, "pose_head: need logits or seeds_in");
  const bool ragged = n_points != nullptr;
  int Sn = p->num_seeds;
  const int k = p->k, iters = p->num_iterations;
  long long n_sum = (long long)B * N;
  SetDevice sd(h, stream);
  if (ragged) {
    if (int rc = build_pair_table(h, n_points, B, ratio, k, &N, &n_sum, &Sn)) return rc;
    for (int b = 0; b < B; ++b) {
      GMF_REQUIRE(n_points[b] > k, GMF_ERR_UNSUPPORTED_SHAPE, "pose_head_ragged: every pair needs more than k correspondences (k = min(k, N - 1) "
                                                               "per pair is not supported in a ragged batch: run such a pair on its own)");
      GMF_REQUIRE((int)((double)n_points[b] * ratio) >= 1, GMF_ERR_UNSUPPORTED_SHAPE, "pose_head_ragged: a pair would have no seed (int(n * ratio) = 0)");
    }
  }
  GMF_REQUIRE(B > 0 && N > 1, GMF_ERR_UNSUPPORTED_SHAPE, "pose_head: need N > 1");
  GMF_REQUIRE(Sn > 0 && Sn <= N, GMF_ERR_UNSUPPORTED_SHAPE, "pose_head: need 0 < num_seeds <= N");
  GMF_REQUIRE(k > 0 && k <= 64 && k <= N - 1, GMF_ERR_UNSUPPORTED_SHAPE, "pose_head: need 0 < k <= min(64, N-1)");
  GMF_REQUIRE(iters > 0 && iters <= 64, GMF_ERR_BAD_ARG, "pose_head: bad num_iterations");
  GMF_REQUIRE(seeds_in || (size_t)Sn * 8 <= 156 * 1024, GMF_ERR_UNSUPPORTED_SHAPE, "pose_head: more than 19968 seeds per pair (the winners' list lives in the LDS)");
  GMF_REQUIRE((p->sigma > 0.f || h->sigma_dev) && p->sigma_d > 0.f, GMF_ERR_BAD_ARG, "pose_head: sigma, sigma_d must be positive");
  hipStream_t st = S(stream);
  const size_t BS = (size_t)B * Sn;
  float *fimg, *dmat, *keys, *snaps, *sT, *fit;
  int *seeds, *knn, *counts, *best, *stop_it;
  unsigned char* conv;
  double* hsum;
  gmf::PairTab* ptab;
  if (int rc = arena_carve(h, {arena_buf(fimg, (size_t)B * tiles_of(N) * kTileFloats),
                               arena_buf(dmat, BS * tiles_of(N) * 32),
                               arena_buf(keys, (size_t)B * N), arena_buf(seeds, BS), arena_buf(knn, BS * k),
                               arena_buf(snaps, BS * iters * k), arena_buf(conv, BS * iters), arena_buf(sT, BS * 16),
                               arena_buf(counts, BS), arena_buf(fit, BS), arena_buf(best, (size_t)B), arena_buf(hsum, BS * 15),
                               arena_buf(stop_it, 1), arena_buf(ptab, ragged ? (size_t)B : 0)}))
    return rc;
  if (ragged) {
    if (int rc = upload_pair_table(h, ptab, B, st)) return rc;
    if (seeds_out) GMF_HIP(hipMemsetAsync(seeds_out, 0, BS * sizeof(int), st));
    if (knn_out) GMF_HIP(hipMemsetAsync(knn_out, 0, BS * k * sizeof(int), st));
    if (seed_trans) GMF_HIP(hipMemsetAsync(seed_trans, 0, BS * 16 * sizeof(float), st));
    if (fitness) GMF_HIP(hipMemsetAsync(fitness, 0, BS * sizeof(float), st));
  }
  if (seeds_out) seeds = seeds_out;
  if (knn_out) knn = knn_out;
  if (seed_trans) sT = seed_trans;
  if (fitness) fit = fitness;

  const int* seeds_use = seeds_in;
  const bool preset = !seeds_in && p->use_nms;
  GMF_HIP(gmf::launch_pack_rows_h2(feat_n, fimg, B, N, st, ptab, preset ? logits : nullptr, preset ? keys : nullptr,
                                   preset ? (ptab ? (long)n_sum : (long)B * N) : 0));
  if (!seeds_in) {
    const float* kk = logits;
    if (p->use_nms) {
      float* scr = (BS * N >= gmf::nms_scratch_floats(B, N)) ? dmat : nullptr;
      GMF_HIP(gmf::launch_nms_keys(h->tune, src_keypts, logits, keys, B, N, p->nms_radius, st, scr, ptab, (long)n_sum, true));
      kk = keys;
    }
    GMF_HIP(gmf::launch_sort_topk(h->tune, kk, seeds, B, N, Sn, st, ptab));
    seeds_use = seeds;
  } else if (seeds_out) {
    GMF_HIP(hipMemcpyAsync(seeds_out, seeds_in, BS * sizeof(int), hipMemcpyDeviceToDevice, st));
  }
  GMF_HIP(gmf::launch_seed_dist(fimg, seeds_use, dmat, B, N, Sn, st, ptab));
  GMF_HIP(gmf::launch_knn_seeds(feat_n, seeds_use, dmat, knn, B, N, Sn, k, st, ptab));
  GMF_HIP(gmf::launch_seed_power(feat_n, src_keypts, tgt_keypts, knn, snaps, conv, hsum, B, N, Sn, k, iters, p->sigma, p->sigma_d, st, ptab, h->sigma_dev));
  GMF_HIP(gmf::launch_seed_kabsch(src_keypts, tgt_keypts, knn, snaps, conv, sT, B, N, Sn, k, iters, hsum, stop_it, st, ptab));
  GMF_HIP(gmf::launch_score_hyp(src_keypts, tgt_keypts, sT, counts, B, N, Sn, p->inlier_threshold, st, ptab));
  GMF_HIP(gmf::launch_finalize_pose(src_keypts, tgt_keypts, sT, counts, fit, final_trans, final_labels, best, B, N, Sn,
                                    p->inlier_threshold, p->refine_threshold, p->refine_iters, st, ptab));
  return GMF_OK;
}

int gmf_knn_from_distances(gmf_handle* h, const float* dist, int B, int N, int Sn, int k, int* knn_out, gmf_stream_t stream) {
  GMF_REQUIRE(h && dist && knn_out, GMF_ERR_BAD_ARG, "knn_from_distances: null pointer");
  GMF_REQUIRE(B > 0 && N > 1 && Sn > 0 && k > 0 && k <= 63 && k <= N - 1, GMF_ERR_UNSUPPORTED_SHAPE,
              "knn_from_distances: need 0 < k <= min(63, N - 1)");
  SetDevice sd(h, stream);
  GMF_HIP(gmf::launch_knn_seeds(nullptr, nullptr, dist, knn_out, B, N, Sn, k, S(stream), nullptr));
  return GMF_OK;
}

int gmf_knn_rows(gmf_handle* h, const float* feat_n, const int* rows, int B, int N, int Sn, int k, int* knn_out,
                 gmf_stream_t stream) {
  GMF_REQUIRE(h && feat_n && rows && knn_out, GMF_ERR_BAD_ARG, "knn_rows: null pointer");
  GMF_REQUIRE(B > 0 && N > 1 && Sn > 0 && k > 0 && k <= N - 1, GMF_ERR_UNSUPPORTED_SHAPE, "knn_rows: need 0 < k <= N-1");
  SetDevice sd(h, stream);
  hipStream_t st = S(stream);
  if (k > 63) {
    GMF_REQUIRE((size_t)N * 4 <= 150 * 1024, GMF_ERR_UNSUPPORTED_SHAPE, "knn_rows: k > 63 needs N <= 38400 (the in-LDS kNN)");
    GMF_HIP(gmf::launch_knn_seeds(feat_n, rows, nullptr, knn_out, B, N, Sn, k, st));
    return GMF_OK;
  }
  const int tiles = tiles_of(N);
  const size_t ld = (size_t)tiles * 32;
  const size_t cap = (size_t)1 << 30;
  const bool whole = (size_t)B * Sn * ld <= cap;
  const int slice = whole ? Sn : (int)std::max<size_t>(1, std::min<size_t>((size_t)Sn, cap / ld));
  float *fimg, *dmat;
  if (int rc = arena_carve(h, {arena_buf(fimg, (size_t)B * tiles * kTileFloats), arena_buf(dmat, (size_t)(whole ? B : 1) * slice * ld)}))
// ... 908 lines not shown
```

### gmf_amd/csrc/launchers.hpp

```cpp
#pragma once
#include <hip/hip_runtime.h>

namespace gmf {

struct PairTab { int row0, n, S, k, ord, pad0, pad1, pad2; };

constexpr int kPvStatStride = 32;
struct PvGuard {
  const unsigned* stat = nullptr;
  const float* thr2 = nullptr;
  unsigned* stat_next = nullptr;
};

struct CompatCache {
  const float* dense;
  const float* tail_wst_h2;
  float* part_o;
  float* part_ml;
  const float* next_wst_h2 = nullptr;
  const float* next_bias = nullptr;
  bool half = false;
  const PairTab* ptab = nullptr;
  int fmt = 0;
  unsigned* v_scale = nullptr;
  const float* qf_img = nullptr;
  const float* qw_wst = nullptr;
  const float* qw_bias = nullptr;
  PvGuard guard;
};

struct Tuning {
  int scattn_variant = 18;
  bool use_cache = true;
  int key_splits = 0;
  bool tail_split = false;
  int ff_split = 0;
  bool front_split = true;
  bool wide_attn_tile = true;
  bool small_merge_tile = true;
  bool small_fattn_tile = true;
  bool small_roles = true;
  bool fused_linear = true;
  int conv_patch = 1;
  bool small_prologue = true;
  bool conv_small = true;
  int nms_binned = 1;
  bool topk_select = true;
  int mid_grid_roles = 512;
  bool q_in_attention = true;
  int pv_fp8 = 1;
  int compat_format = 0;
  int precision = 0;
  int spectral_col_splits = 0;
};

hipError_t launch_compat_build(const float* pts8, float* c_dense, int B, int N, int tiles, float sigma_d, int fmt, hipStream_t s,
                               const PairTab* ptab = nullptr);
hipError_t launch_front(int mode, const float* in, const float* wst, const float* vecs, float* f, float* q, float* k,
                        float* v, int B, int N, int tiles, hipStream_t s);
hipError_t launch_scattn_fp32(const float* q, const float* k, const float* v, const float* pts8, const float* fus,
                              const float* wst, const float* vecs, float* out, int B, int N, int tiles, float sigma_d,
                              hipStream_t s);
hipError_t launch_scattn_h2(const float* q, const float* k, const float* v, const float* pts8, const float* fus, const float* wst,
                            const float* vecs, float* out, int B, int N, int tiles, float sigma_d, hipStream_t s, const float* c_dense);
hipError_t launch_scattn_h2p(const float* q, const float* k, const float* v, const float* fus, const float* vecs, float* out, int B,
                             int N, int tiles, hipStream_t s, const CompatCache& cc, int n_full, int ksplits);
hipError_t launch_scattn_dense(const float* q, const float* k, const float* v, const float* compat, const float* fus,
                               const float* wst, const float* vecs, float* out, int B, int N, int tiles, hipStream_t s);
hipError_t launch_ctx_prep(bool pe, const float* ctx, const float* wst, const float* vecs, float* out, int B, int T,
                           int ttiles, int sets, int wst_stride, int vec_stride, hipStream_t s);
hipError_t launch_fusion_attn(bool pe, const float* x, const float* ctx_img, const float* wst, const float* vecs,
                              float* x1, int B, int N, int tiles, int T, int ttiles, hipStream_t s);
hipError_t launch_fusion_ff(const float* x1, const float* wst, const float* vecs, float* x2, int B, int tiles, hipStream_t s);
hipError_t launch_head(const float* feat_img, const float* wst, const float* vecs, float* logits, float* feat_n,
                       float* feat_rm, int B, int N, int tiles, hipStream_t s, int* status = nullptr, const PairTab* ptab = nullptr,
                       const unsigned* pv_stat = nullptr, const float* pv_thr2 = nullptr, int n_layers = 0);
hipError_t launch_ctx_prep_w(bool pe, const float* ctx, const float* wst, const float* vecs, float* out, int B, int T,
                             int ttiles, hipStream_t s);
hipError_t launch_fusion_attn_w(bool pe, const float* x, const float* ctx_img, const float* wst, const float* vecs,
                                float* x1, int B, int N, int tiles, int T, int ttiles, hipStream_t s);
hipError_t launch_fusion_ff_w(const float* x1, const float* wst, const float* vecs, float* x2, int B, int tiles, hipStream_t s);
hipError_t launch_ctx_prep_w_h2(bool pe, const float* ctx, const float* wst_h2, const float* vecs, float* out, int B, int T,
                                int ttiles, hipStream_t s, bool rowmajor = false);
hipError_t launch_fusion_attn_w_h2(bool pe, const float* x, const float* ctx_img, const float* wst_h2, const float* vecs,
                                   float* x1, int B, int N, int tiles, int T, int ttiles, hipStream_t s, bool tile_form = true);
hipError_t launch_fusion_ff_w_h2(const float* x1, const float* wst_h2, const float* vecs, float* x2, int B, int tiles, hipStream_t s,
                                 float* part = nullptr, int hs = 1, float* out_rm = nullptr, long o_sb = 0, long o_sr = 0,
                                 long o_sk = 0, int n_rows = 0, int* status = nullptr);
int plan_ff_split_w(int base_wgs);
hipError_t launch_front_h2(int mode, bool split, const float* in, const float* wst, const float* vecs, float* f, float* q, float* k,
                           float* v, int B, int N, int tiles, hipStream_t s, const PairTab* ptab = nullptr, unsigned* v_scale = nullptr,
                           PvGuard guard = {});
hipError_t launch_linear_h2(bool roles, const float* f, const float* front_wst, const float* front_vec, const float* ctx_img,
                            const float* attn_wst, const float* attn_vec, const float* ff_wst, const float* ff_vec, float* q,
                            float* k, float* v, float* x2, int B, int N, int tiles, int T, int ttiles, hipStream_t s, bool one_product = false,
                            const PairTab* ptab = nullptr, unsigned* v_scale = nullptr, PvGuard guard = {});
hipError_t launch_small_front_fattn(const float* f, const float* front_wst, const float* front_vec, const float* ctx_img,
                                    const float* attn_wst, const float* attn_vec, float* q, float* k, float* v, float* x1, int B,
                                    int N, int tiles, int T, int ttiles, hipStream_t s, unsigned* v_scale = nullptr, PvGuard guard = {},
                                    bool tile_role = true, const PairTab* ptab = nullptr);
hipError_t launch_small_attn_ff_merge(const float* q, const float* k, const float* v, const float* x1, const float* ff_wst,
                                      const float* ff_vecs, float* ff_part, int ff_hs, const float* tail_vecs, float* out, int B,
                                      int N, int tiles, int ksplits, hipStream_t s, const CompatCache* cc, bool tile_merge = true);
hipError_t launch_ctx_prep_h2(bool pe, const float* ctx, const float* wst, const float* vecs, float* out, int B, int T,
                              int ttiles, int sets, int wst_stride, int vec_stride, hipStream_t s, bool rowmajor = false);
hipError_t launch_fusion_attn_h2(bool pe, const float* x, const float* ctx_img, const float* wst, const float* vecs,
                                 float* x1, int B, int N, int tiles, int T, int ttiles, hipStream_t s, bool rowmajor = false);
hipError_t launch_pro_ctx_pts(const float* p_tokens, const float* wst, const float* vecs, float* f1ctx, int B, int T, int ttiles,
                              const float* src, const float* tgt, float* pts8, int N, hipStream_t s, const PairTab* ptab,
                              unsigned* zero_words, int n_zero);
hipError_t launch_pro_fattn_compat(const float* q_tokens, const float* f1ctx, const float* wst, const float* vecs, float* x1t, int B,
                                   int T, int ttiles, const float* pts8, float* c_dense, int N, int tiles, float sigma_d,
                                   hipStream_t s, const PairTab* ptab);
hipError_t launch_pro_ff_front(const float* x1t, const float* wst, const float* vecs, float* imgfeat, int B, int ttiles, float* part,
                               int hs, const float* corr_pos, const float* fwst, const float* fvecs, float* f, float* q, float* k,
                               float* v, int N, int tiles, hipStream_t s, const PairTab* ptab, PvGuard guard);
hipError_t launch_ff_reduce_h2(const float* part, const float* x1, const float* vecs, float* x2, int B, int tiles, int hs, hipStream_t s);
hipError_t launch_fusion_ff_h2(const float* x1, const float* wst, const float* vecs, float* x2, int B, int tiles, hipStream_t s,
                               float* part = nullptr, int hs = 1);
int padded_desc_width(int d);
hipError_t launch_nn_match(const float* F0, const float* F1, float* f0_img, float* f1_img, float* norm2, unsigned long long* best, int* idx,
                           float* dist, int N0, int N1, int d, int mode, hipStream_t s);
struct MatchPair { int row0, n0, key0, n1, tile0, stage0, stages, wg0, wgx, ks, pad0, pad1; };
struct MatchTotals { long tiles0, stages, wgs, rows0; int tps; };
bool plan_nn_match_batched(const int* off0, const int* off1, int B, int K, MatchPair* tab, MatchTotals* tot);
hipError_t launch_nn_match_batched(const float* F0, const float* F1, float* f0_img, float* f1_img, float* norm2, unsigned long long* best,
                                   const MatchPair* tab, int B, const MatchTotals& tot, int d, int mode, int global_index, int* idx,
                                   float* dist, hipStream_t s);
hipError_t launch_seed_dist(const float* featn_img, const int* seeds, float* dist, int B, int N, int S, hipStream_t s, const PairTab* ptab = nullptr);
hipError_t launch_pack_p32(const float* src, float* dst, int B, int n_rows, int K, long sb, long sr, long sk, hipStream_t s, const PairTab* ptab = nullptr);
hipError_t launch_pack_rows_h2(const float* src, float* dst, int B, int n_rows, hipStream_t s, const PairTab* ptab = nullptr,
                               const float* copy_src = nullptr, float* copy_dst = nullptr, long n_copy = 0);
hipError_t launch_unpack_p32(const float* src, float* dst, int B, int n_rows, int K, long sb, long sr, long sk, hipStream_t s, int* status = nullptr);
hipError_t launch_pack_pts8(const float* src, const float* tgt, float* dst, int B, int N, hipStream_t s, const PairTab* ptab = nullptr,
                            unsigned* zero_words = nullptr, int n_zero = 0);

size_t similarity_image_floats(int B, int N);
int sm_fused_parts_per_pair(int B, int N);
int sm_parts_per_pair(int B, int N);
int classification_parts(int B, int N);
int transformation_slices(int B, int N);
hipError_t launch_similarity_matrix(const float* feat_n, float* img, float* M, int B, int N, int ldm, float sigma,
                                    hipStream_t s, const float* sigma_dev = nullptr);
hipError_t launch_sm_loss_fused(const float* feat_n, const float* gt, float* img, double* part, double* pair_loss, int B,
                                int N, float sigma, int balanced, float* out, hipStream_t s, const float* sigma_dev = nullptr);
hipError_t launch_sm_loss(const float* M, int ldm, const float* gt, double* part, double* pair_loss, int B, int N,
                          int balanced, float* out, hipStream_t s);
int sm_backward_parts(int B, int N);
hipError_t launch_sm_backward(const float* feat_n, const float* gt, float* img, float* timg, float* consts, double* dsig_part,
                              int B, int N, float sigma, int balanced, float* dF, float* dsigma, hipStream_t s,
                              const float* sigma_dev = nullptr);
hipError_t launch_classification_loss(const float* pred, const float* gt, const float* weight, double* part, int B, int N,
                                      int balanced, float* out, hipStream_t s);
hipError_t launch_transformation_loss(const float* trans, const float* gt_trans, const float* src, const float* tgt,
                                      const float* probs, double* part, int B, int N, float re_thre, float te_thre,
                                      float* out, hipStream_t s);

int gemm_ksplits(bool ta, bool tb, const float* A, const float* B, int M, int N, int K, long lda, long ldb, long sA, long sB,
                 int batch);
hipError_t launch_gemm_f32(bool ta, bool tb, const float* A, const float* B, float* C, const float* bias, const float* R, int M, int N,
                           int K, long lda, long ldb, long ldc, long sA, long sB, long sC, int batch, float alpha, float* part,
                           int ksplits, int relu, hipStream_t s);
// ... 36 lines not shown
```

### gmf_amd/csrc/launchers_pose.hpp

```cpp
#pragma once
#include <hip/hip_runtime.h>
#include "launchers.hpp"

namespace gmf {

hipError_t launch_nms_keys(const Tuning& tune, const float* src, const float* scores, float* keys, int B, int N, float R, hipStream_t s,
                           float* scratch = nullptr,
                           const PairTab* ptab = nullptr, long total_rows = 0,
                           bool keys_preset = false);
size_t nms_scratch_floats(int B, int N);
hipError_t launch_sort_topk(const Tuning& tune, const float* keys, int* out_idx, int B, int N, int S, hipStream_t s, const PairTab* ptab = nullptr);
hipError_t launch_knn_seeds(const float* feat_n, const int* seeds, const float* dist_in, int* knn_idx, int B, int N, int S,
                            int k, hipStream_t s, const PairTab* ptab = nullptr);
hipError_t launch_seed_power(const float* feat_n , const float* src, const float* tgt, const int* knn_idx, float* snaps,
                             unsigned char* conv, double* hsum, int B, int N, int S, int k, int iters, float sigma,
                             float sigma_d, hipStream_t s, const PairTab* ptab = nullptr, const float* sigma_dev = nullptr);
hipError_t launch_seed_kabsch(const float* src, const float* tgt, const int* knn_idx, const float* snaps,
                              const unsigned char* conv, float* seed_T, int B, int N, int S, int k, int iters,
                              const double* hsum, int* stop_scratch, hipStream_t s, const PairTab* ptab = nullptr);
hipError_t launch_stop_iteration(const unsigned char* conv, int B, int S, int iters, int* stop_out, hipStream_t s);
hipError_t launch_score_hyp(const float* src, const float* tgt, const float* seed_T, int* counts, int B, int N, int S,
                            float tau, hipStream_t s, const PairTab* ptab = nullptr);
hipError_t launch_finalize_pose(const float* src, const float* tgt, const float* seed_T, const int* counts, float* fitness,
                                float* final_T, float* labels, int* best, int B, int N, int S, float tau, float refine_thr,
                                int refine_iters, hipStream_t s, const PairTab* ptab = nullptr);
hipError_t launch_post_refine(const float* T_in, const float* src, const float* tgt, float* T_out, int B, int N, float thr,
                              int iters, hipStream_t s);
hipError_t launch_rigid_transform(const float* A, const float* Bp, const float* w, float* T, int n, int k,
                                  float weight_threshold, hipStream_t s);
hipError_t launch_weighted_procrustes(const float* X, const float* Y, const float* w, const int* offsets, int B, float eps,
                                      float* R, float* t, hipStream_t s);
hipError_t launch_global_registration(const float* X, const float* Y, const float* w, const int* offsets, int B, float eps,
                                      float qsize, int max_iter, int max_break, double ratio, float* R, float* t,
                                      float* stats, int max_n, hipStream_t s);

hipError_t launch_tl_backward(const float* trans, const float* src, const float* tgt, const float* probs, float* g_trans,
                              int B, int N, hipStream_t s);
hipError_t launch_pose_best_backward(const float* feat_n, const float* src, const float* tgt, const int* knn_idx,
                                     const float* fitness, const float* snaps, const unsigned char* conv, const float* g_T,
                                     float* g_feat, float* g_sigma, int B, int N, int S, int k, int iters, float sigma,
                                     float sigma_d, const int* stop_batch, hipStream_t s, const float* sigma_dev = nullptr);
hipError_t launch_wp_backward(const float* X, const float* Y, const float* w, const int* offsets, int B, float eps,
                              const float* g_R, const float* g_t, float* g_w, hipStream_t s);

}
```

### gmf_amd/csrc/pose_kernels.hip

```cpp
#include <hip/hip_runtime.h>
#include <stdint.h>
#include <math.h>
#include <algorithm>
#include <type_traits>

#include "launchers_pose.hpp"
#include "mfma_core.hpp"
#include "kabsch.hpp"

namespace gmf {

#define GMF_DEVINL __device__ __forceinline__

GMF_DEVINL int pair_seeds(const PairTab* pt, int pair, int S) { return pt ? pt[pair].S : S; }

GMF_DEVINL void write_T(float* T, const double* R, const double* ca, const double* cb) {
#pragma unroll
  for (int r = 0; r < 3; ++r) {
    const float r0 = (float)R[3 * r], r1 = (float)R[3 * r + 1], r2 = (float)R[3 * r + 2];
    T[4 * r + 0] = r0; T[4 * r + 1] = r1; T[4 * r + 2] = r2;
    T[4 * r + 3] = (float)cb[r] - (r0 * (float)ca[0] + r1 * (float)ca[1] + r2 * (float)ca[2]);
  }
  T[12] = 0.f; T[13] = 0.f; T[14] = 0.f; T[15] = 1.f;
}
// ... 635 lines not shown
  float last_v = -INFINITY; int last_i = -1;
  for (int it = 0; it <= k; ++it) {
    float rv = INFINITY; int ri = 0x7fffffff;
    for (int j = tid; j < N; j += 256) {
      const float v = dr[j];
      const bool behind = v > last_v || (v == last_v && j > last_i);
      if (behind && (v < rv || (v == rv && j < ri))) { rv = v; ri = j; }
    }
#pragma unroll
    for (int o = 32; o > 0; o >>= 1) {
      const float ov = __shfl_xor(rv, o, 64); const int oi = __shfl_xor(ri, o, 64);
      if (ov < rv || (ov == rv && oi < ri)) { rv = ov; ri = oi; }
    }
    const int buf = it & 1;
    if (lane == 0) { red_v[buf][wave] = rv; red_i[buf][wave] = ri; }
    __syncthreads();
    float wv = red_v[buf][0]; int wi = red_i[buf][0];
#pragma unroll
    for (int w = 1; w < 4; ++w) {
      const float ov = red_v[buf][w]; const int oi = red_i[buf][w];
      if (ov < wv || (ov == wv && oi < wi)) { wv = ov; wi = oi; }
    }
    if (it > 0 && tid == 0) out[it - 1] = (wi < N) ? wi : min(it, N - 1);
    last_v = wv; last_i = wi;
  }
}

constexpr int kKMax = 64;

__global__ void __launch_bounds__(64, 3)
k_seed_power(const float* __restrict__ feat_n, const float* __restrict__ src, const float* __restrict__ tgt,
             const int* __restrict__ knn_idx, float* __restrict__ snaps, unsigned char* __restrict__ conv,
             double* __restrict__ hsum, int N, int S, int k, int iters, float inv_sigma2, float inv_sigmad2,
             const PairTab* __restrict__ ptab, const float* __restrict__ sigma_dev) {
  inv_sigma2 = sigma_inv2(inv_sigma2, sigma_dev);
  extern __shared__ __attribute__((aligned(16))) float seed_smem[];
  float* const P = seed_smem;
  float* const vec = P + kKMax * 8;
  float* const Mx = vec + kKMax;
  const int ld = k + 1;
  const int pair = blockIdx.y, s = blockIdx.x, a = threadIdx.x;
  const int lane = a, h = lane >> 5, i = lane & 31;
  if (s >= pair_seeds(ptab, pair, S)) return;
  const int* nb = knn_idx + ((size_t)pair * S + s) * k;
  const size_t row0 = pair_row0(ptab, pair, N);
  N = gmf::pair_rows(ptab, pair, N);
  const float* pair_rows = feat_n + row0 * 128;
  {
    float4 z = make_float4(0.f, 0.f, 0.f, 0.f);
    float4* Pz = reinterpret_cast<float4*>(P);
    Pz[2 * a] = z; Pz[2 * a + 1] = z;
  }
  if (a < k) {
    const int j = nb[a];
    const float* ps = src + (row0 + j) * 3;
    const float* pt = tgt + (row0 + j) * 3;
    P[a * 8 + 0] = ps[0]; P[a * 8 + 1] = ps[1]; P[a * 8 + 2] = ps[2];
    P[a * 8 + 4] = pt[0]; P[a * 8 + 5] = pt[1]; P[a * 8 + 6] = pt[2];
  }
  auto row_frag = [&](float (&x)[64], const int row) {
    if (row >= 0 && row < N) {
      const float4* p = reinterpret_cast<const float4*>(pair_rows + (size_t)row * 128) + h;
#pragma unroll
      for (int g = 0; g < 16; ++g) {
        const float4 t = p[8 * (g >> 2) + 2 * (g & 3)];
        x[4 * g + 0] = t.x; x[4 * g + 1] = t.y; x[4 * g + 2] = t.z; x[4 * g + 3] = t.w;
      }
// ... 29 lines not shown
        Mx[ar * ld + b] = m;
        if (mirror) Mx[b * ld + ar] = m;
      }
    }
  };
  gmf::f16x8 ah[8], al[8], bh[8], bl[8];
#pragma unroll
  for (int s8 = 0; s8 < 8; ++s8) { gmf::split8h(fa + 8 * s8, ah[s8], al[s8]); gmf::split8h(fb + 8 * s8, bh[s8], bl[s8]); }
  {
    gmf::f32x16 g = gmf::zero16();
#pragma unroll
    for (int s8 = 0; s8 < 8; ++s8) gmf::mma3(g, ah[s8], al[s8], ah[s8], al[s8]);
    emit_tile(g, 0, 0, false);
  }
  if (k > 32) {
    gmf::f32x16 g = gmf::zero16();
#pragma unroll
    for (int s8 = 0; s8 < 8; ++s8) {
      g = gmf::mfma_h16(bh[s8], al[s8], g);
      g = gmf::mfma_h16(bl[s8], ah[s8], g);
      g = gmf::mfma_h16(bh[s8], ah[s8], g);
    }
    emit_tile(g, 1, 0, true);
    g = gmf::zero16();
#pragma unroll
    for (int s8 = 0; s8 < 8; ++s8) gmf::mma3(g, bh[s8], bl[s8], bh[s8], bl[s8]);
    emit_tile(g, 1, 1, false);
  }
  vec[a] = 1.0f;
  __syncthreads();
  float last = 1.0f;
  float* sn = snaps + ((size_t)pair * S + s) * iters * k;
  unsigned char* cv = conv + ((size_t)pair * S + s) * iters;
  auto power = [&](auto kk_tag) {
    constexpr int KK = decltype(kk_tag)::value;
    float mrow[KK];
#pragma unroll
    for (int b = 0; b < KK; ++b) mrow[b] = (a < k && b < k) ? Mx[a * ld + b] : 0.f;
    const float4* v4 = reinterpret_cast<const float4*>(vec);
    for (int it = 0; it < iters; ++it) {
      float v = 0.f;
#pragma unroll
      for (int q = 0; q < KK / 4; ++q) {
        const float4 t = v4[q];
        v = fmaf(mrow[4 * q + 0], t.x, v); v = fmaf(mrow[4 * q + 1], t.y, v);
        v = fmaf(mrow[4 * q + 2], t.z, v); v = fmaf(mrow[4 * q + 3], t.w, v);
      }
      float n2 = (a < k) ? v * v : 0.f;
#pragma unroll
      for (int o = 32; o > 0; o >>= 1) n2 += __shfl_xor(n2, o, 64);
      v = v / (sqrtf(n2) + 1e-6f);
      const bool close = (a >= k) || (fabsf(v - last) <= 1e-8f + 1e-5f * fabsf(last));
      const bool all_close = __all(close);
      __syncthreads();
      if (a < k) { vec[a] = v; sn[it * k + a] = v; }
      if (a == 0) cv[it] = all_close ? 1 : 0;
      last = v;
      __syncthreads();
    }
  };
  if (k <= 40) power(std::integral_constant<int, 40>{});
  else power(std::integral_constant<int, 64>{});
  if (!hsum) return;
  {
    float sv = 0.f;
    for (int r = 0; r < k; ++r) sv += vec[r];
    const float inv = 1.0f / (sv + 1e-6f);
    float wf = (a < k) ? last * inv : 0.f;
    wf = (wf < 0.f) ? 0.f : wf;
    const double w = wf;
    double pa[3], pb[3];
#pragma unroll
    for (int c = 0; c < 3; ++c) { pa[c] = (a < k) ? P[a * 8 + c] : 0.0; pb[c] = (a < k) ? P[a * 8 + 4 + c] : 0.0; }
    const double sw = wave_sum(w);
    double ca[3], cb[3];
#pragma unroll
    for (int c = 0; c < 3; ++c) { ca[c] = wave_sum(w * pa[c]) / (sw + 1e-6); cb[c] = wave_sum(w * pb[c]) / (sw + 1e-6); }
    double H[9];
#pragma unroll
    for (int r = 0; r < 3; ++r)
#pragma unroll
      for (int c = 0; c < 3; ++c) H[3 * r + c] = wave_sum(w * (pa[r] - ca[r]) * (pb[c] - cb[c]));
    if (a < 15) {
      double* o = hsum + ((size_t)pair * S + s) * 15;
      double val = 0.0;
#pragma unroll
      for (int e = 0; e < 15; ++e) if (a == e) val = (e < 3) ? ca[e] : (e < 6) ? cb[e - 3] : H[e - 6];
      o[a] = val;
    }
  }
}

__global__ void __launch_bounds__(1024)
k_stop_iteration(const unsigned char* __restrict__ conv, int total_seeds, int iters, int* __restrict__ stop_out) {
  __shared__ unsigned long long red[16];
// ... 2 lines not shown
  const size_t n16 = total >> 4;
  const uint4* c16 = reinterpret_cast<const uint4*>(conv);
  for (size_t c = threadIdx.x; c < n16; c += blockDim.x) {
    const uint4 v = c16[c];
    const unsigned w[4] = {v.x, v.y, v.z, v.w};
    int it = (int)((c << 4) % (size_t)iters);
#pragma unroll
    for (int q = 0; q < 4; ++q)
#pragma unroll
      for (int e = 0; e < 4; ++e) {
        if (((w[q] >> (8 * e)) & 0xffu) == 0) bad |= 1ull << it;
        it = (it + 1 == iters) ? 0 : it + 1;
      }
  }
  for (size_t p = (n16 << 4) + threadIdx.x; p < total; p += blockDim.x)
    if (conv[p] == 0) bad |= 1ull << (int)(p % (size_t)iters);
#pragma unroll
  for (int o = 32; o > 0; o >>= 1) bad |= __shfl_xor(bad, o, 64);
  if ((threadIdx.x & 63) == 0) red[threadIdx.x >> 6] = bad;
  __syncthreads();
  if (threadIdx.x == 0) {
    for (int w = 1; w < (int)(blockDim.x >> 6); ++w) bad |= red[w];
    int first = iters - 1;
    for (int it = 0; it < iters - 1; ++it)
      if (!((bad >> it) & 1ull)) { first = it; break; }
    *stop_out = first;
  }
}

__global__ void __launch_bounds__(64)
k_seed_kabsch(const float* __restrict__ src, const float* __restrict__ tgt, const int* __restrict__ knn_idx,
              const float* __restrict__ snaps, const unsigned char* __restrict__ conv, float* __restrict__ seed_T,
              int N, int S, int k, int iters, const double* __restrict__ hsum, const int* __restrict__ stop_batch,
              const PairTab* __restrict__ ptab) {
  __shared__ int stop_it;
  const int pair = blockIdx.y;
  const int S_p = pair_seeds(ptab, pair, S);
  if ((int)blockIdx.x * 64 >= S_p) return;
  if (threadIdx.x == 0) stop_it = iters - 1;
  __syncthreads();
  if (stop_batch) {
    if (threadIdx.x == 0) stop_it = *stop_batch;
  } else {
    const unsigned char* cv = conv + (size_t)pair * S * iters;
    int first = iters - 1;
    for (int it = 0; it < iters - 1; ++it) {
      bool ok = true;
      for (int s2 = threadIdx.x; s2 < S_p; s2 += 64) ok = ok && (cv[(size_t)s2 * iters + it] != 0);
      if (__all(ok)) { first = it; break; }
    }
    if (threadIdx.x == 0) stop_it = first;
  }
  __syncthreads();
  const int s = blockIdx.x * 64 + threadIdx.x;
  if (s >= S_p) return;
  if (hsum && stop_it == iters - 1) {
    const double* hs = hsum + ((size_t)pair * S + s) * 15;
    double ca[3], cb[3], H[9], R[9];
#pragma unroll
    for (int e = 0; e < 3; ++e) { ca[e] = hs[e]; cb[e] = hs[3 + e]; }
#pragma unroll
    for (int e = 0; e < 9; ++e) H[e] = hs[6 + e];
    kabsch_rotation_from_H(H, R);
    write_T(seed_T + ((size_t)pair * S + s) * 16, R, ca, cb);
    return;
  }
  const int* nb = knn_idx + ((size_t)pair * S + s) * k;
  const float* v = snaps + (((size_t)pair * S + s) * iters + stop_it) * k;
  float sv = 0.f;
  for (int r = 0; r < k; ++r) sv += v[r];
  const float inv = 1.0f / (sv + 1e-6f);
  const float* ps = src + pair_row0(ptab, pair, N) * 3;
  const float* pt = tgt + pair_row0(ptab, pair, N) * 3;
  double sw = 0, ca[3] = {0, 0, 0}, cb[3] = {0, 0, 0};
// ... 571 lines not shown
                            int k, hipStream_t s, const PairTab* ptab) {
  const int ld = ((N + 31) / 32) * 32;
  if (dist_in && N > 256 * 64) {
    hipLaunchKernelGGL(k_knn_select_stream, dim3(S, B), dim3(256), 0, s, dist_in, knn_idx, N, S, k, ptab, ld);
    return hipGetLastError();
  }
  if ((size_t)N * 4 > 150 * 1024) return hipErrorInvalidValue;
  {
    hipError_t e = hipFuncSetAttribute(reinterpret_cast<const void*>(k_knn_seeds), hipFuncAttributeMaxDynamicSharedMemorySize, 150 * 1024);
    if (e != hipSuccess) return e;
  }
  if (dist_in && N <= 256 * 8) {
    hipLaunchKernelGGL(k_knn_select_fast<8>, dim3(S, B), dim3(256), 0, s, dist_in, knn_idx, N, S, k, ptab, ld);
    return hipGetLastError();
  }
  if (dist_in && N <= 256 * 20) {
    hipLaunchKernelGGL(k_knn_select_fast<20>, dim3(S, B), dim3(256), 0, s, dist_in, knn_idx, N, S, k, ptab, ld);
    return hipGetLastError();
  }
  if (dist_in && N <= 256 * 32) {
    hipLaunchKernelGGL(k_knn_select_fast<32>, dim3(S, B), dim3(256), 0, s, dist_in, knn_idx, N, S, k, ptab, ld);
    return hipGetLastError();
  }
  if (dist_in && N <= 256 * 64) {
    hipLaunchKernelGGL(k_knn_select_fast<64>, dim3(S, B), dim3(256), 0, s, dist_in, knn_idx, N, S, k, ptab, ld);
    return hipGetLastError();
  }
  hipLaunchKernelGGL(k_knn_seeds, dim3(S, B), dim3(256), (size_t)N * 4, s, feat_n, seeds, dist_in, knn_idx, N, S, k, ptab, ld);
  return hipGetLastError();
}

hipError_t launch_seed_power(const float* feat_n, const float* src, const float* tgt, const int* knn_idx, float* snaps,
                             unsigned char* conv, double* hsum, int B, int N, int S, int k, int iters, float sigma,
                             float sigma_d, hipStream_t s, const PairTab* ptab, const float* sigma_dev) {
  if (k > kKMax) return hipErrorInvalidValue;
  const size_t lds_bytes = (size_t)(kKMax * 8 + kKMax + k * (k + 1)) * sizeof(float);
  hipLaunchKernelGGL(k_seed_power, dim3(S, B), dim3(64), lds_bytes, s, feat_n, src, tgt, knn_idx, snaps, conv, hsum, N, S, k,
                     iters, 1.0f / (sigma * sigma), 1.0f / (sigma_d * sigma_d), ptab, sigma_dev);
  return hipGetLastError();
}

hipError_t launch_seed_kabsch(const float* src, const float* tgt, const int* knn_idx, const float* snaps,
                              const unsigned char* conv, float* seed_T, int B, int N, int S, int k, int iters,
                              const double* hsum, int* stop_scratch, hipStream_t s, const PairTab* ptab) {
  const int* stop_batch = nullptr;
  if (B > 1 && stop_scratch && !ptab) {
    hipLaunchKernelGGL(k_stop_iteration, dim3(1), dim3(1024), 0, s, conv, B * S, iters, stop_scratch);
    stop_batch = stop_scratch;
  }
  hipLaunchKernelGGL(k_seed_kabsch, dim3((S + 63) / 64, B), dim3(64), 0, s, src, tgt, knn_idx, snaps, conv, seed_T, N, S, k, iters,
                     hsum, stop_batch, ptab);
  return hipGetLastError();
}

hipError_t launch_stop_iteration(const unsigned char* conv, int B, int S, int iters, int* stop_out, hipStream_t s) {
  hipLaunchKernelGGL(k_stop_iteration, dim3(1), dim3(1024), 0, s, conv, B * S, iters, stop_out);
  return hipGetLastError();
}

hipError_t launch_score_hyp(const float* src, const float* tgt, const float* seed_T, int* counts, int B, int N, int S,
                            float tau, hipStream_t s, const PairTab* ptab) {
  float t = tau * tau;
  if (tau > 0.f) {
    while (sqrtf(t) >= tau && t > 0.f) t = nextafterf(t, 0.f);
    while (sqrtf(t) < tau) t = nextafterf(t, INFINITY);
  } else {
    t = 0.f;
  }
  hipLaunchKernelGGL(k_score_hyp, dim3((S + kHypPerWG - 1) / kHypPerWG, B), dim3(256), 0, s, src, tgt, seed_T, counts, N, S, t, ptab);
  return hipGetLastError();
}

hipError_t launch_finalize_pose(const float* src, const float* tgt, const float* seed_T, const int* counts, float* fitness,
                                float* final_T, float* labels, int* best, int B, int N, int S, float tau, float refine_thr,
                                int refine_iters, hipStream_t s, const PairTab* ptab) {
  hipLaunchKernelGGL(k_finalize_pose, dim3(B), dim3(N <= 2048 ? 256 : 1024), 0, s, src, tgt, seed_T, counts, fitness, final_T, labels, best, N, S,
                     tau, refine_thr, refine_iters, ptab);
  return hipGetLastError();
}

hipError_t launch_post_refine(const float* T_in, const float* src, const float* tgt, float* T_out, int B, int N, float thr,
                              int iters, hipStream_t s) {
  hipLaunchKernelGGL(k_post_refine, dim3(B), dim3(N <= 2048 ? 256 : 1024), 0, s, T_in, src, tgt, T_out, N, thr, iters);
  return hipGetLastError();
// ... 25 lines not shown
```

### gmf_amd/pointdsc.py

```python
from __future__ import annotations

import torch
import torch.nn.functional as F
from torch import nn

from . import _lib, packing
from ._util import WeightWatcher, handle_and_stream, params_version, require_cuda_f32
from .fusion_layer import FusionLayer
from .losses import similarity_matrix


class _BasicBlock(nn.Module):
    def __init__(self, inp, planes, stride=1):
        super().__init__()
        self.conv1 = nn.Conv2d(inp, planes, 3, stride, 1, bias=False)
        self.bn1 = nn.BatchNorm2d(planes)
        self.relu = nn.ReLU(inplace=True)
        self.conv2 = nn.Conv2d(planes, planes, 3, 1, 1, bias=False)
        self.bn2 = nn.BatchNorm2d(planes)
        self.downsample = None
        if stride != 1 or inp != planes:
            self.downsample = nn.Sequential(nn.Conv2d(inp, planes, 1, stride, bias=False), nn.BatchNorm2d(planes))

    def forward(self, x):
# ... 356 lines not shown
        key = (self._watch.version(), device)
        if self._packed is None or self._packed_version != key:
            self._packed = packing.PackedEncoder(self._hot_state(), self.encoder.num_layers, device)
            self._packed_version = key
        return self._packed

    def set_precision(self, mode: str):
        levels = {"parity": 0, "parity_strict": 0, "throughput": 1, "throughput_max": 2}
        if mode not in levels:
            raise ValueError("gmf_amd.PointDSC.set_precision: mode must be 'parity', 'parity_strict', 'throughput' or 'throughput_max'")
        self._precision = levels[mode]
        self._strict = mode == "parity_strict"

    def _call_tuned(self, h, fn, *args):
        import ctypes as C
        want = {}
        if getattr(self, "_precision", 0):
            want[b"precision"] = self._precision
        if getattr(self, "_strict", False):
            want[b"pv_fp8"] = 0
        prev = {}
        for knob, val in want.items():
            cur = C.c_int(0)
            h.call("gmf_get_tuning", knob, C.byref(cur))
            if cur.value != val:
                prev[knob] = cur.value
                h.call("gmf_set_tuning", knob, val)
        try:
            h.call(fn, *args)
        finally:
            for knob, val in prev.items():
                h.call("gmf_set_tuning", knob, val)

    def encode(self, corr_pos, src_keypts, tgt_keypts, p_tokens, q_tokens, want_features=False):
        if self.training:
            raise RuntimeError("gmf_amd.PointDSC.encode is the eval() inference path (BatchNorm folded from running statistics); in train() "
                               "mode call the module with autograd enabled (the differentiable forward), or call eval() first")
        corr_pos = require_cuda_f32(corr_pos, "corr_pos").contiguous()
        src = require_cuda_f32(src_keypts, "src_keypts").contiguous()
        tgt = require_cuda_f32(tgt_keypts, "tgt_keypts").contiguous()
        p_tokens = require_cuda_f32(p_tokens, "p_tokens").contiguous()
        q_tokens = require_cuda_f32(q_tokens, "q_tokens").contiguous()
        B, N, D = corr_pos.shape
        T = p_tokens.shape[1]
        if D != self.encoder.layer0.weight.shape[1]:
            raise RuntimeError(f"gmf_amd.PointDSC: corr_pos last dim {D} != in_dim {self.encoder.layer0.weight.shape[1]}")
        if p_tokens.shape != (B, T, 128) or q_tokens.shape != (B, T, 128):
            raise RuntimeError("gmf_amd.PointDSC: image tokens must be [B,T,128] for both images")
        if src.shape != (B, N, 3) or tgt.shape != (B, N, 3):
            raise RuntimeError("gmf_amd.PointDSC: src_keypts/tgt_keypts must be [B,N,3]")
        pw = self._weights(corr_pos.device)
        dev = corr_pos.device
        logits = torch.empty((B, N), device=dev)
        feat_n = torch.empty((B, N, 128), device=dev)
        feat = torch.empty((B, N, 128), device=dev) if want_features else None
        h, st = handle_and_stream(corr_pos, check=True)
        self._call_tuned(h, "gmf_encoder_forward", pw.struct, corr_pos.data_ptr(), src.data_ptr(), tgt.data_ptr(),
                         p_tokens.data_ptr(), q_tokens.data_ptr(), B, N, T, logits.data_ptr(), feat_n.data_ptr(),
                         None if feat is None else feat.data_ptr(), st)
        return logits, feat_n, feat

    def _pose_params(self, N, testing, sigmas=None, device=None):
        S = int(N * self.ratio)
        k = min(self.k, N - 1)
        pp = _lib.PoseParams()
        pp.num_seeds, pp.k, pp.num_iterations = S, k, self.num_iterations
        pp.use_nms = 1 if testing else 0
        pp.refine_iters = 20 if testing else 0
        if sigmas is None:
            pw = self._weights(device)
            sigmas = (pw.sigma, pw.sigma_d)
        pp.sigma, pp.sigma_d = sigmas
        pp.inlier_threshold, pp.nms_radius = float(self.inlier_threshold), float(self.nms_radius)
        pp.refine_threshold = 0.10 if self.inlier_threshold == 0.10 else 1.2
        return pp, S, k

    def pose_head(self, feat_n, src_keypts, tgt_keypts, logits, testing, seeds=None, return_aux=False, sigmas=None):
        B, N, _ = feat_n.shape
        pp, S, k = self._pose_params(N, testing, sigmas, feat_n.device)
        dev = feat_n.device
        final_T = torch.empty((B, 4, 4), device=dev)
        labels = torch.empty((B, N), device=dev)
        seeds_out = torch.empty((B, S), device=dev, dtype=torch.int32)
        aux = {}
        if return_aux:
            aux = {"knn_idx": torch.empty((B, S, k), device=dev, dtype=torch.int32),
                   "seed_trans": torch.empty((B, S, 4, 4), device=dev), "fitness": torch.empty((B, S), device=dev)}
        seeds_in = None if seeds is None else seeds.to(torch.int32).contiguous()
        h, st = handle_and_stream(feat_n)
        h.call("gmf_pose_head", pp, feat_n.data_ptr(), src_keypts.data_ptr(), tgt_keypts.data_ptr(), logits.data_ptr(),
               None if seeds_in is None else seeds_in.data_ptr(), B, N, final_T.data_ptr(), labels.data_ptr(),
               seeds_out.data_ptr(), aux["knn_idx"].data_ptr() if return_aux else None,
               aux["seed_trans"].data_ptr() if return_aux else None, aux["fitness"].data_ptr() if return_aux else None, st)
        aux["seeds"] = seeds_out
        return final_T, labels, aux

    def _forward_train(self, data):
        from . import train as T
        corr_pos = require_cuda_f32(data["corr_pos"], "corr_pos")
        src = require_cuda_f32(data["src_keypts"], "src_keypts").contiguous()
        tgt = require_cuda_f32(data["tgt_keypts"], "tgt_keypts").contiguous()
        if "p_tokens" in data:
            p_tok, q_tok = data["p_tokens"], data["q_tokens"]
        else:
            enc = self.encoder.image_encoder
            p_tok = enc(data["p_image"]).flatten(2).permute(0, 2, 1).contiguous()
            q_tok = enc(data["q_image"]).flatten(2).permute(0, 2, 1).contiguous()
        B, N, _ = corr_pos.shape
        if getattr(self, "sigma_on_device", False):
            if getattr(self, "_sigma_d_host", None) is None:
                self._sigma_d_host = float(self.sigma_spat)
            sigma, sigma_d = T.SIGMA_ON_DEVICE, self._sigma_d_host
        else:
            sigma, sigma_d = float(self.sigma.detach()), float(self.sigma_spat)
        compat = T.compat_dense(src, tgt, sigma_d)
        feat = T.encoder_train(self.encoder, corr_pos, compat, p_tok, q_tok)
        feat_n = T.normalize_rows(feat.reshape(B * N, -1)).reshape(B, N, -1)
        M = T.similarity_matrix_train(feat_n, self.sigma, sigma)
        logits = T.classifier_train(self.classification, feat)
        self.last_logits, self.last_features = logits, feat_n
        final_trans = T.pose_head_train(self, feat_n, self.sigma, src, tgt, logits.detach().contiguous(), (sigma, sigma_d))
        return {"final_trans": final_trans, "final_labels": logits, "M": M}

    def forward_ragged(self, data):
        if self.training:
            raise RuntimeError("gmf_amd.PointDSC.forward_ragged is the eval() test-mode path")
# ... 34 lines not shown
        final_T = torch.empty((B, 4, 4), device=dev)
        labels = torch.empty(total, device=dev)
        pp, _, _ = self._pose_params(max(n_points), True, None, dev)
        h, st = handle_and_stream(cp, check=True)
        self._call_tuned(h, "gmf_encoder_forward_ragged", pw.struct, cp.data_ptr(), sk.data_ptr(), tk.data_ptr(), p_tok.data_ptr(),
                         q_tok.data_ptr(), npts, B, T, logits.data_ptr(), feat_n.data_ptr(), None, st)
        h.call("gmf_pose_head_ragged", pp, float(self.ratio), feat_n.data_ptr(), sk.data_ptr(), tk.data_ptr(), logits.data_ptr(), npts, B,
               final_T.data_ptr(), labels.data_ptr(), None, None, None, None, st)
        self.last_logits, self.last_features = logits, feat_n
        return {"final_trans": final_T, "final_labels": list(torch.split(labels, n_points)), "logits": list(torch.split(logits, n_points)),
                "M": None}

    def forward(self, data):
        if isinstance(data.get("corr_pos"), (list, tuple)) or "n_points" in data:
            return self.forward_ragged(data)
        if self.training and torch.is_grad_enabled():
            if "testing" in data.keys():
                raise RuntimeError("gmf_amd.PointDSC: test mode (`testing` key) in train() mode with autograd enabled - call eval() "
                                   "or torch.no_grad() for inference")
            return self._forward_train(data)
        corr_pos, src_keypts, tgt_keypts = data["corr_pos"], data["src_keypts"], data["tgt_keypts"]
        testing = "testing" in data.keys()
        if "p_tokens" in data:
            p_tok, q_tok = data["p_tokens"], data["q_tokens"]
        else:
            with torch.no_grad():
                p_img, q_img = data["p_image"], data["q_image"]
                if p_img.shape == q_img.shape:
                    tok = self.encoder.image_tokens(torch.cat([p_img, q_img]))
                    p_tok, q_tok = tok[:p_img.shape[0]], tok[p_img.shape[0]:]
                else:
                    p_tok, q_tok = self.encoder.image_tokens(p_img), self.encoder.image_tokens(q_img)
        with torch.no_grad():
            logits, feat_n, feat = self.encode(corr_pos, src_keypts, tgt_keypts, p_tok, q_tok, want_features=not testing)
            self.last_logits, self.last_features = logits, feat_n
            src = src_keypts.contiguous()
            tgt = tgt_keypts.contiguous()
            final_trans, labels, _ = self.pose_head(feat_n, src, tgt, logits, testing)
            M = None
            if not testing:
                M = similarity_matrix(feat_n, self._weights(feat_n.device).sigma)
        return {"final_trans": final_trans, "final_labels": labels if testing else logits, "M": M}

    def pick_seeds(self, dists, scores, R, max_num, src_keypts=None):
        if src_keypts is None:
            raise RuntimeError("gmf_amd.PointDSC.pick_seeds: pass src_keypts=...; the N x N `dists` matrix is never materialised")
        src = require_cuda_f32(src_keypts, "src_keypts").contiguous()
        scores = require_cuda_f32(scores, "scores").contiguous()
        B, N = scores.shape
        out = torch.empty((B, max_num), device=src.device, dtype=torch.int32)
        h, st = handle_and_stream(src)
        h.call("gmf_pick_seeds", src.data_ptr(), scores.data_ptr(), B, N, float(R), 1, int(max_num), out.data_ptr(), st)
        return out.long()

    def post_refinement(self, initial_trans, src_keypts, tgt_keypts, weights=None):
        T = require_cuda_f32(initial_trans, "initial_trans").contiguous()
        src = require_cuda_f32(src_keypts, "src_keypts").contiguous()
        tgt = require_cuda_f32(tgt_keypts, "tgt_keypts").contiguous()
        B, N = src.shape[0], src.shape[1]
        out = torch.empty_like(T)
        thr = 0.10 if self.inlier_threshold == 0.10 else 1.2
        h, st = handle_and_stream(T)
        h.call("gmf_post_refinement", T.data_ptr(), src.data_ptr(), tgt.data_ptr(), B, N, thr, 20, out.data_ptr(), st)
        return out
```

### include/gmf_hip.h

```cpp
#ifndef GMF_HIP_H_
#define GMF_HIP_H_

#ifdef __cplusplus
extern "C" {
#endif

typedef struct gmf_handle gmf_handle;
typedef void* gmf_stream_t;

enum {
  GMF_OK = 0,
  GMF_ERR_BAD_ARG = -1,
  GMF_ERR_UNSUPPORTED_SHAPE = -2,
  GMF_ERR_HIP = -3,
  GMF_ERR_NO_DEVICE = -4,
  GMF_ERR_OOM = -5,
  GMF_ERR_WORKSPACE = -6
};

#define GMF_ABI_VERSION 5

int gmf_abi_version(void);
int gmf_create(int device, gmf_handle** out);
void gmf_destroy(gmf_handle* h);
// ... 64 lines not shown
  int ndim;
  long long shape[4];
} gmf_tensor;
#define GMF_PACK_DEVICE_TENSORS 1
#define GMF_PACK_STANDALONE_BLOCK 2
#define GMF_PACK_HOST_BLOCK 4
typedef struct gmf_packed_encoder gmf_packed_encoder;
int gmf_encoder_pack_weights(gmf_handle* h, const gmf_tensor* tensors, int n_tensors, int num_layers, int flags,
                             gmf_packed_encoder** out);
const struct gmf_encoder_weights* gmf_packed_encoder_weights(const gmf_packed_encoder* p);
int gmf_packed_encoder_info(const gmf_packed_encoder* p, float* sigma, float* sigma_d, int* split_fp16, float* max_abs_scaled);
void gmf_packed_encoder_free(gmf_packed_encoder* p);
long long gmf_packed_encoder_bytes(const gmf_packed_encoder* p);
int gmf_packed_encoder_place(gmf_handle* h, gmf_packed_encoder* p, void* device_dst, long long bytes, gmf_stream_t stream);

typedef struct gmf_fusion_weights {
  int latent_dim, d_head, pe, split_fp16;
  float max_abs_scaled;
  const float *ctx_wst, *ctx_vec, *attn_wst, *attn_vec, *ff_wst, *ff_vec;
  const float *ctx_wst_h2, *attn_wst_h2, *ff_wst_h2;
} gmf_fusion_weights;
typedef struct gmf_packed_fusion gmf_packed_fusion;
int gmf_fusion_pack_weights(gmf_handle* h, const gmf_tensor* tensors, int n_tensors, const char* prefix, int pe, int flags,
                            gmf_packed_fusion** out);
const gmf_fusion_weights* gmf_packed_fusion_weights(const gmf_packed_fusion* p);
void gmf_packed_fusion_free(gmf_packed_fusion* p);
long long gmf_packed_fusion_bytes(const gmf_packed_fusion* p);
int gmf_packed_fusion_place(gmf_handle* h, gmf_packed_fusion* p, void* device_dst, long long bytes, gmf_stream_t stream);

int gmf_encoder_forward(gmf_handle* h, const gmf_encoder_weights* w, const float* corr_pos, const float* src_keypts,
                        const float* tgt_keypts, const float* p_tokens, const float* q_tokens, int B, int N, int T,
                        float* logits, float* feat_n, float* feat, gmf_stream_t stream);

int gmf_encoder_forward_ragged(gmf_handle* h, const gmf_encoder_weights* w, const float* corr_pos, const float* src_keypts,
                               const float* tgt_keypts, const float* p_tokens, const float* q_tokens, const int* n_points, int B,
                               int T, float* logits, float* feat_n, float* feat, gmf_stream_t stream);

int gmf_nonlocal_block_forward(gmf_handle* h, const gmf_encoder_weights* w, int layer, int apply_pointcn,
                               const float* feat_img, const float* pts8, const float* attention,
                               const float* image_feat_img, float* out_img, int B, int N, int T, gmf_stream_t stream);

int gmf_fusion_layer_forward(gmf_handle* h, int pe, int latent_dim, int d_head, const float* ctx_wst, const float* ctx_vec,
                             const float* attn_wst, const float* attn_vec, const float* ff_wst, const float* ff_vec,
                             const float* data, const float* queries, long long q_sb, long long q_sr, long long q_sk,
                             float* out, long long o_sb, long long o_sr, long long o_sk, int B, int N, int T,
                             gmf_stream_t stream, const float* ff_wst_h2, const float* ctx_wst_h2, const float* attn_wst_h2);

typedef struct gmf_pose_params {
  int num_seeds;
  int k;
  int num_iterations;
  int use_nms;
  int refine_iters;
  float sigma;
  float sigma_d;
  float inlier_threshold;
  float nms_radius;
  float refine_threshold;
} gmf_pose_params;

int gmf_pose_head(gmf_handle* h, const gmf_pose_params* p, const float* feat_n, const float* src_keypts,
                  const float* tgt_keypts, const float* logits, const int* seeds_in, int B, int N, float* final_trans,
                  float* final_labels, int* seeds_out, int* knn_out, float* seed_trans, float* fitness,
                  gmf_stream_t stream);

int gmf_pose_head_ragged(gmf_handle* h, const gmf_pose_params* p, double ratio, const float* feat_n, const float* src_keypts,
                         const float* tgt_keypts, const float* logits, const int* n_points, int B, float* final_trans,
                         float* final_labels, int* seeds_out, int* knn_out, float* seed_trans, float* fitness,
                         gmf_stream_t stream);

int gmf_pick_seeds(gmf_handle* h, const float* src_keypts, const float* scores, int B, int N, float nms_radius,
                   int use_nms, int num_seeds, int* seeds_out, gmf_stream_t stream);

int gmf_knn_rows(gmf_handle* h, const float* feat_n, const int* rows, int B, int N, int S, int k, int* knn_out,
                 gmf_stream_t stream);

int gmf_knn_from_distances(gmf_handle* h, const float* dist, int B, int N, int S, int k, int* knn_out, gmf_stream_t stream);

int gmf_nn_match(gmf_handle* h, const float* F0, const float* F1, int N0, int N1, int d, int mode, int* idx_out,
                 float* dist_out, gmf_stream_t stream);

int gmf_nn_match_batched(gmf_handle* h, const float* F0, const float* F1, const int* off0, const int* off1, int B, int d, int mode,
                         int global_index, int* idx_out, float* dist_out, gmf_stream_t stream);

int gmf_nn_match_mutual_batched(gmf_handle* h, const float* F0, const float* F1, const int* off0, const int* off1, int B, int d,
                                int* idx_out, float* dist_out, unsigned char* mutual_out, gmf_stream_t stream);

int gmf_build_correspondences(gmf_handle* h, const float* F0, const float* F1, const float* src_keypts, const float* tgt_keypts,
                              const int* off0, const int* off1, int B, int d, int use_mutual, int in_dim, const float* gt_trans,
                              float inlier_threshold, int* out_offsets, long long* corr_out, float* src_out, float* tgt_out,
                              float* corr_pos_out, float* src_desc_out, float* tgt_desc_out, float* labels_out, gmf_stream_t stream);

int gmf_matching_indices_count(gmf_handle* h, const float* xyz0, const int* off0, const float* xyz1, const int* off1, int B,
                               long long total0, long long total1, const double* T, double radius, long long* row_start,
                               long long* pair_offsets, long long* num_pairs, gmf_stream_t stream);
int gmf_matching_indices_fill(gmf_handle* h, const float* xyz0, const int* off0, const float* xyz1, const int* off1, int B,
                              long long total0, long long total1, const double* T, double radius, const long long* row_start,
// ... 192 lines not shown
```

Measured before the change: 9.764 million.

## Fuse classifier head and seed image packing into last attention epilogue

Adds a HEAD variant of the scattered-attention epilogue and merge kernel. For the last encoder layer, it computes the classifier MLP logits, the L2-normalised features and an fp16 hi/lo seed image directly in registers, so no separate head kernel or repacking pass is needed. The pose head gets a seeded entry point that reuses this image and the NMS keys, and the stop-iteration kernel is replaced with a device word zeroed in the seed-distance kernel. The risks are extra register pressure in the attention kernel and new API paths and buffers that must stay consistent across the encoder and the pose head.

```diff
diff --git a/gmf_amd/_lib.py b/gmf_amd/_lib.py
--- a/gmf_amd/_lib.py
+++ b/gmf_amd/_lib.py
@@ -132,6 +132,11 @@
     "gmf_packed_fusion_place": (C.c_int, [_vp, _vp, _vp, C.c_longlong, _vp]),
     "gmf_encoder_forward": (C.c_int, [_vp, C.POINTER(EncoderWeights), _vp, _vp, _vp, _vp, _vp, C.c_int, C.c_int, C.c_int,
                                       _vp, _vp, _vp, _vp]),
+    "gmf_seed_image_floats": (_ll, [C.c_int, C.c_int]),
+    "gmf_encoder_forward_seeded": (C.c_int, [_vp, C.POINTER(EncoderWeights), _vp, _vp, _vp, _vp, _vp, C.c_int, C.c_int, C.c_int,
+                                             _vp, _vp, _vp, _vp, _vp, _vp]),
+    "gmf_pose_head_seeded": (C.c_int, [_vp, C.POINTER(PoseParams), _vp, _vp, _vp, _vp, _vp, C.c_int, C.c_int, _vp, _vp, _vp, _vp, _vp,
+                                       _vp, _vp, _vp, _vp]),
     "gmf_encoder_forward_ragged": (C.c_int, [_vp, C.POINTER(EncoderWeights), _vp, _vp, _vp, _vp, _vp, _i32p, C.c_int, C.c_int,
                                              _vp, _vp, _vp, _vp]),
     "gmf_pose_head_ragged": (C.c_int, [_vp, C.POINTER(PoseParams), C.c_double, _vp, _vp, _vp, _vp, _i32p, C.c_int, _vp, _vp, _vp,
diff --git a/gmf_amd/csrc/encoder_kernels.hip b/gmf_amd/csrc/encoder_kernels.hip
--- a/gmf_amd/csrc/encoder_kernels.hip
+++ b/gmf_amd/csrc/encoder_kernels.hip
@@ -480,11 +480,97 @@
   if (wave == 1 && next_bias && lane < 32) dma_piece_1k(next_bias, lvec + 2 * C, lane);
 }
 
-template <bool NEXT_PCN, class Stages, class Fus>
+struct HeadRows {
+  const HeadFuse* hd;
+  const float* vecs;
+  size_t row0;
+  int row, n_rows;
+  size_t img_tile;
+};
+
+template <class Stages>
+GMF_DEVINL void head_rows_epilogue(const float (&x)[CF], const bool active, Stages& ss, const HeadRows& hr, const int lane, const int h) {
+  const HeadFuse& hd = *hr.hd;
+  float h1[16], h2[16];
+  float logit = 0.f, nrm2 = 0.f;
+  {
+    const float4* lw = ss.acquire();
+    if (active) {
+      f32x16 acc = zero16();
+      mma_wx<CF>(acc, lw, x);
+      float b[16];
+      load_vec_block(b, hr.vecs, 0, h);
+#pragma unroll
+      for (int r = 0; r < 16; ++r) h1[r] = fmaxf(acc[r] + b[r], 0.f);
+    }
+  }
+  {
+    const float4* lw = ss.acquire();
+    if (active) {
+      f32x16 acc = zero16();
+      mma_wx<16>(acc, lw, h1);
+      float b[16];
+      load_vec_block(b, hr.vecs + 32, 0, h);
+#pragma unroll
+      for (int r = 0; r < 16; ++r) h2[r] = fmaxf(acc[r] + b[r], 0.f);
+      float w3[16];
+      load_vec_block(w3, hr.vecs + 64, 0, h);
+      float part = 0.f;
+#pragma unroll
+      for (int r = 0; r < 16; ++r) part = fmaf(h2[r], w3[r], part);
+      logit = xhalf_sum(part) + hr.vecs[96];
+      float ss2 = 0.f;
+#pragma unroll
+      for (int k = 0; k < CF; ++k) ss2 = fmaf(x[k], x[k], ss2);
+      nrm2 = xhalf_sum(ss2);
+    }
+  }
+  const bool in_pair = active && hr.row < hr.n_rows;
+  const bool bad_row = not_finite(nrm2);
+  flag_status(hd.status, in_pair && (not_finite(logit) || bad_row), 1);
+  if (!active) return;
+  const float inv = 1.0f / fmaxf(sqrtf(nrm2), 1e-12f);
+  const bool zero_row = bad_row || !in_pair;
+  if (in_pair) {
+    const size_t ro = hr.row0 + hr.row;
+    if (h == 0) {
+      hd.logits[ro] = logit;
+      if (hd.keys) hd.keys[ro] = logit;
+    }
+    float4* pn = reinterpret_cast<float4*>(hd.feat_n + ro * C) + h;
+#pragma unroll
+    for (int g = 0; g < CF / 4; ++g)
+      pn[2 * g] = bad_row ? make_float4(0.f, 0.f, 0.f, 0.f)
+                          : make_float4(x[4 * g] * inv, x[4 * g + 1] * inv, x[4 * g + 2] * inv, x[4 * g + 3] * inv);
+    if (hd.feat_rm) {
+      float4* pr = reinterpret_cast<float4*>(hd.feat_rm + ro * C) + h;
+#pragma unroll
+      for (int g = 0; g < CF / 4; ++g) pr[2 * g] = make_float4(x[4 * g], x[4 * g + 1], x[4 * g + 2], x[4 * g + 3]);
+    }
+  }
+  if (hd.seed_img) {
+    f16x8* img = reinterpret_cast<f16x8*>(hd.seed_img + hr.img_tile * kStageFloats);
+#pragma unroll
+    for (int s8 = 0; s8 < 8; ++s8) {
+      float v[8];
+#pragma unroll
+      for (int j = 0; j < 8; ++j) v[j] = zero_row ? 0.f : x[8 * s8 + j] * inv;
+      f16x8 hi, lo;
+      split8h(v, hi, lo);
+      img[(0 * 8 + s8) * 64 + lane] = hi;
+      img[(1 * 8 + s8) * 64 + lane] = lo;
+    }
+  }
+}
+
+template <bool NEXT_PCN, class Stages, class Fus, bool HEAD = false>
 GMF_DEVINL void scattn_epilogue_h2(const float (&o)[CF], const bool active, Stages& ss, const float* __restrict__ vecs,
                                    const Fus& fus_tile, float* __restrict__ out_tile, const int lane, const int h,
                                    const float* __restrict__ next_bias = nullptr,
-                                   unsigned* __restrict__ stat_next = nullptr, const int pair = 0, const bool row_valid = false) {
+                                   unsigned* __restrict__ stat_next = nullptr, const int pair = 0, const bool row_valid = false,
+                                   const HeadRows* head = nullptr) {
+    static_assert(!(NEXT_PCN && HEAD), "the head follows the last layer");
+    float headx[HEAD ? CF : 1];
     FragH2<8> ox, featx;
     FragH2<4> m1x, m2x;
     if (active) ox.set(o);
@@ -529,9 +615,13 @@
 #pragma unroll
         for (int r = 0; r < 16; ++r) tt[r] = fmaf(acc[r], kH2Inv, b[r]) + fz[r];
         if (NEXT_PCN) featx.set_block(mb, tt);
-        else if (active) store_block_p32(out_tile, mb, tt, lane);
-      }
-    }
+        else if (HEAD) {
+#pragma unroll
+          for (int r = 0; r < 16; ++r) headx[16 * mb + r] = tt[r];
+        } else if (active) store_block_p32(out_tile, mb, tt, lane);
+      }
+    }
+    if constexpr (HEAD) head_rows_epilogue(headx, active, ss, *head, lane, h);
     if (NEXT_PCN) {
       float ssq = 0.f;
 #pragma unroll
@@ -562,7 +652,7 @@
 }
 
 constexpr float kInvU16 = 1.0f / 65535.0f;
-template <int NPROD = 3, int CFMT = 0, int WAVES = 4, bool PVF8 = false>
+template <int NPROD = 3, int CFMT = 0, int WAVES = 4, bool PVF8 = false, bool HEAD = false>
 GMF_DEVINL void scattn_h2p_body(float* lds, const int bid, const float* __restrict__ q_img, const float* __restrict__ k_img,
                                 const float* __restrict__ v_img, const float* __restrict__ fus, const float* __restrict__ wst,
                                 const float* __restrict__ vecs, float* out, int N, int tiles, int wgs_per_pair,
@@ -572,8 +662,10 @@
                                 const unsigned* __restrict__ v_scale = nullptr,
                                 const float* qf_img = nullptr, const float* __restrict__ qw_wst = nullptr,
                                 const float* __restrict__ qw_bias = nullptr,
-                                unsigned* __restrict__ stat_next = nullptr) {
+                                unsigned* __restrict__ stat_next = nullptr,
+                                const HeadFuse* head = nullptr) {
   static_assert(!PVF8 || NPROD == 3, "the fp8 cross products belong to the three-product form");
+  static_assert(!HEAD || (NPROD == 3 && WAVES == 4), "the head runs behind the parity epilogue");
   float* const ldsK = lds;
   float* const ldsV = lds + 2 * kStageFloats;
   const int lane = threadIdx.x & 63, h = lane >> 5;
@@ -1058,6 +1150,23 @@
   }
   __syncthreads();
   float* const lvec = lds + 2 * kStageFloats;
+  if (HEAD && head->wst) {
+    if (head->pv_stat && head->status && qblock == 0 && threadIdx.x == 0) {
+      bool tripped = false;
+      for (int l = 0; l < head->n_layers; ++l)
+        tripped |= !(__uint_as_float(head->pv_stat[((size_t)l * head->n_pairs + pair) * kPvStatStride]) <= head->pv_thr2[l]);
+      if (tripped) __hip_atomic_fetch_or(head->status, 2, __ATOMIC_RELAXED, __HIP_MEMORY_SCOPE_SYSTEM);
+    }
+    stage_tail_vecs(lvec, vecs, head->vecs, wave, lane);
+    StageStream ss;
+    ss.init(lds, lds + kStageFloats, wave, WAVES, lane, wst, 5, head->wst, 2);
+    ss.prime();
+    const FusTile ft{fus + toff};
+    const HeadRows hr{head, lvec + 2 * C, ptab ? (size_t)ptab[pair].row0 : (size_t)pair * N, tile_raw * 32 + (lane & 31), N, pbase + tile};
+    if constexpr (HEAD)
+      scattn_epilogue_h2<false, StageStream, FusTile, true>(o, active, ss, lvec, ft, nullptr, lane, h, nullptr, nullptr, pair, false, &hr);
+    return;
+  }
   stage_tail_vecs(lvec, vecs, next_wst ? next_bias : nullptr, wave, lane);
   StageStream ss;
   ss.init(lds, lds + kStageFloats, wave, WAVES, lane, wst, 5, next_wst, next_wst ? 4 : 0);
@@ -1084,17 +1193,18 @@
              int n_items, int n_full, int ksplits, float* __restrict__ part_o, float* __restrict__ part_ml,
              const float* __restrict__ next_wst, const float* __restrict__ next_bias, const PairTab* __restrict__ ptab,
              const unsigned* __restrict__ v_scale, const float* qf_img, const float* __restrict__ qw_wst,
-             const float* __restrict__ qw_bias, const PvGuard guard) {
+             const float* __restrict__ qw_bias, const PvGuard guard, const HeadFuse head) {
   __shared__ __attribute__((aligned(16))) float lds[4 * kStageFloats];
+  constexpr bool HEAD = NPROD == 3 && CFMT == 0;
   tail_priority(blockIdx.x, gridDim.x);
   if (!PVF8 || attn_pv_on(v_scale, guard, blockIdx.x, n_items, n_full, ksplits, wgs_per_pair, ptab))
-    scattn_h2p_body<NPROD, CFMT, 4, PVF8>(lds, blockIdx.x, q_img, k_img, v_img, fus, wst, vecs, out, N, tiles, wgs_per_pair, c_dense, n_items,
-                                          n_full, ksplits, part_o, part_ml, next_wst, next_bias, ptab, v_scale, qf_img, qw_wst, qw_bias,
-                                          guard.stat_next);
+    scattn_h2p_body<NPROD, CFMT, 4, PVF8, HEAD>(lds, blockIdx.x, q_img, k_img, v_img, fus, wst, vecs, out, N, tiles, wgs_per_pair, c_dense, n_items,
+                                                n_full, ksplits, part_o, part_ml, next_wst, next_bias, ptab, v_scale, qf_img, qw_wst, qw_bias,
+                                                guard.stat_next, &head);
   else
-    scattn_h2p_body<NPROD, CFMT, 4, false>(lds, blockIdx.x, q_img, k_img, v_img, fus, wst, vecs, out, N, tiles, wgs_per_pair, c_dense, n_items,
-                                           n_full, ksplits, part_o, part_ml, next_wst, next_bias, ptab, nullptr, qf_img, qw_wst, qw_bias,
-                                           guard.stat_next);
+    scattn_h2p_body<NPROD, CFMT, 4, false, HEAD>(lds, blockIdx.x, q_img, k_img, v_img, fus, wst, vecs, out, N, tiles, wgs_per_pair, c_dense, n_items,
+                                                 n_full, ksplits, part_o, part_ml, next_wst, next_bias, ptab, nullptr, qf_img, qw_wst, qw_bias,
+                                                 guard.stat_next, &head);
 }
 
 __global__ void __launch_bounds__(256, 2)
@@ -1282,14 +1392,14 @@
 struct StagesPreloaded {
   const float* base;
   int used, lane;
-  GMF_DEVINL void init(float* lds, int wave, int lane_, const float* g, int n_stages, const float* g2 = nullptr) {
+  GMF_DEVINL void init(float* lds, int wave, int lane_, const float* g, int n_stages, const float* g2 = nullptr, int n2 = 4) {
     base = lds; used = 0; lane = lane_;
     for (int st = 0; st < n_stages; ++st)
 #pragma unroll
       for (int q = 0; q < 4; ++q)
         dma_piece_1k(g + (size_t)st * kStageFloats + (wave + 4 * q) * 256, lds + st * kStageFloats + (wave + 4 * q) * 256, lane_);
     if (g2)
-      for (int st = 0; st < 4; ++st)
+      for (int st = 0; st < n2; ++st)
 #pragma unroll
         for (int q = 0; q < 4; ++q)
           dma_piece_1k(g2 + (size_t)st * kStageFloats + (wave + 4 * q) * 256, lds + (n_stages + st) * kStageFloats + (wave + 4 * q) * 256, lane_);
@@ -1305,13 +1415,14 @@
   }
 };
 
+template <bool HEAD>
 __global__ void __launch_bounds__(256, 1)
 k_scattn_merge(const float* __restrict__ part_o, const float* __restrict__ part_ml, const float* __restrict__ fus,
                const float* __restrict__ wst, const float* __restrict__ vecs, float* __restrict__ out, int tiles,
                int wgs_per_pair, int n_items, int n_full, int ksplits, const float* __restrict__ next_wst,
                const float* __restrict__ next_bias, const float* __restrict__ ff_part, int ff_hs, const float* __restrict__ x1,
                const float* __restrict__ ff_b2, unsigned* __restrict__ stat_next, int n_rows,
-               const PairTab* __restrict__ ptab = nullptr) {
+               const PairTab* __restrict__ ptab, const HeadFuse head) {
   __shared__ __attribute__((aligned(16))) float lds[9 * kStageFloats + kTailVecFloats];
   const int lane = threadIdx.x & 63, h = lane >> 5, i = lane & 31;
   const int wave = __builtin_amdgcn_readfirstlane(threadIdx.x >> 6);
@@ -1330,11 +1441,12 @@
   const size_t pt0 = (size_t)pair * tiles + tile;
   const size_t toff = pt0 * (32 * C);
   float* const lvec = lds + 9 * kStageFloats;
-  stage_tail_vecs(lvec, vecs, next_wst ? next_bias : nullptr, wave, lane);
+  stage_tail_vecs(lvec, vecs, HEAD ? head.vecs : next_wst ? next_bias : nullptr, wave, lane);
   vecs = lvec;
   next_bias = lvec + 2 * C;
   StagesPreloaded ss;
-  ss.init(lds, wave, lane, wst, 5, next_wst);
+  if (HEAD) ss.init(lds, wave, lane, wst, 5, head.wst, 2);
+  else ss.init(lds, wave, lane, wst, 5, next_wst);
   float x2[CF];
   if (ff_part) {
     const float* pt = ff_part + toff;
@@ -1392,6 +1504,18 @@
   const float inv = 1.0f / l;
 #pragma unroll
   for (int e = 0; e < CF; ++e) o[e] *= inv;
+  if constexpr (HEAD) {
+    if (head.pv_stat && head.status && it.item == slot * wgs_per_pair && threadIdx.x == 0) {
+      bool tripped = false;
+      for (int l = 0; l < head.n_layers; ++l)
+        tripped |= !(__uint_as_float(head.pv_stat[((size_t)l * head.n_pairs + pair) * kPvStatStride]) <= head.pv_thr2[l]);
+      if (tripped) __hip_atomic_fetch_or(head.status, 2, __ATOMIC_RELAXED, __HIP_MEMORY_SCOPE_SYSTEM);
+    }
+    const HeadRows hr{&head, next_bias, ptab ? (size_t)ptab[pair].row0 : (size_t)pair * n_rows, tile_raw * 32 + i, n_rows, pt0};
+    const FusTile ft{fus + toff};
+    scattn_epilogue_h2<false, StagesPreloaded, FusTile, true>(o, active, ss, vecs, ft, nullptr, lane, h, nullptr, nullptr, pair, false, &hr);
+    return;
+  }
   if (ff_part) {
     const FusRegs fp{x2};
     if (next_wst) scattn_epilogue_h2<true>(o, active, ss, vecs, fp, out + toff, lane, h, next_bias, stat_next, pair, tile_raw * 32 + i < n_rows);
@@ -1841,8 +1965,9 @@
 
 __global__ void __launch_bounds__(256, 2)
 k_seed_dist(const float* __restrict__ featn_img, const int* __restrict__ seeds, float* __restrict__ dist,
-            int N, int tiles, int S, int chunks, const PairTab* __restrict__ ptab) {
+            int N, int tiles, int S, int chunks, const PairTab* __restrict__ ptab, unsigned long long* __restrict__ zero_word) {
   __shared__ __attribute__((aligned(16))) float lds[4 * kStageFloats];
+  if (zero_word && blockIdx.x == 0 && blockIdx.y == 0 && threadIdx.x == 0) *zero_word = 0ull;
   const int lane = threadIdx.x & 63, h = lane >> 5, i = lane & 31;
   const int wave = __builtin_amdgcn_readfirstlane(threadIdx.x >> 6);
   const int pair = blockIdx.y / chunks, chunk = blockIdx.y - pair * chunks;
@@ -2021,11 +2146,13 @@
                        tiles, ksplits, cc->next_wst_h2, cc->next_bias, (const float*)ff_part, ff_hs, x1, ff_vecs + 2 * C + 2 * FFH,
                        cc->guard.stat_next, N, cc->ptab);
   else
-    hipLaunchKernelGGL(k_scattn_merge, dim3(8 * per_xcd), dim3(256), 0, s, cc->part_o, cc->part_ml, x1, cc->tail_wst_h2, tail_vecs, out,
+    hipLaunchKernelGGL(k_scattn_merge<false>, dim3(8 * per_xcd), dim3(256), 0, s, cc->part_o, cc->part_ml, x1, cc->tail_wst_h2, tail_vecs, out,
                        tiles, wpp, W, 0, ksplits, cc->next_wst_h2, cc->next_bias, (const float*)ff_part, ff_hs, x1,
-                       ff_vecs + 2 * C + 2 * FFH, cc->guard.stat_next, N, cc->ptab);
+                       ff_vecs + 2 * C + 2 * FFH, cc->guard.stat_next, N, cc->ptab, HeadFuse{});
   return hipGetLastError();
 }
+
+bool scattn_h2p_fuses_head(const CompatCache& cc) { return !cc.half && cc.fmt == 0; }
 
 hipError_t launch_scattn_h2p(const float* q, const float* k, const float* v, const float* fus, const float* vecs, float* out, int B,
                              int N, int tiles, hipStream_t s, const CompatCache& cc, int n_full, int ksplits) {
@@ -2033,28 +2160,33 @@
   const int per_xcd = (W >> 3) + ((W & 7) ? 1 : 0);
   const int max_tail = std::max(0, per_xcd - n_full);
   const dim3 grid(8 * (std::min(n_full, per_xcd) + max_tail * ksplits));
+  if (cc.head.wst && (!scattn_h2p_fuses_head(cc) || cc.next_wst_h2)) return hipErrorInvalidValue;
   if (cc.half && max_tail == 0)
     hipLaunchKernelGGL(k_scattn_fast, dim3(8 * per_xcd), dim3(256), 0, s, q, k, v, fus, cc.tail_wst_h2, vecs, out, N, tiles, wpp, cc.dense, W,
                        cc.next_wst_h2, cc.next_bias);
   else if (cc.half)
     hipLaunchKernelGGL((k_scattn_h2p<1, 1>), grid, dim3(256), 0, s, q, k, v, fus, cc.tail_wst_h2, vecs, out, N, tiles, wpp, cc.dense, W,
-                       n_full, ksplits, cc.part_o, cc.part_ml, cc.next_wst_h2, cc.next_bias, cc.ptab, (const unsigned*)nullptr, (const float*)nullptr, (const float*)nullptr, (const float*)nullptr, PvGuard{});
+                       n_full, ksplits, cc.part_o, cc.part_ml, cc.next_wst_h2, cc.next_bias, cc.ptab, (const unsigned*)nullptr, (const float*)nullptr, (const float*)nullptr, (const float*)nullptr, PvGuard{}, HeadFuse{});
   else if (cc.fmt == 2 && cc.v_scale)
     hipLaunchKernelGGL((k_scattn_h2p<3, 2, true>), grid, dim3(256), 0, s, q, k, v, fus, cc.tail_wst_h2, vecs, out, N, tiles, wpp, cc.dense,
-                       W, n_full, ksplits, cc.part_o, cc.part_ml, cc.next_wst_h2, cc.next_bias, cc.ptab, cc.v_scale, cc.qf_img, cc.qw_wst, cc.qw_bias, cc.guard);
+                       W, n_full, ksplits, cc.part_o, cc.part_ml, cc.next_wst_h2, cc.next_bias, cc.ptab, cc.v_scale, cc.qf_img, cc.qw_wst, cc.qw_bias, cc.guard, HeadFuse{});
   else if (cc.fmt == 2)
     hipLaunchKernelGGL((k_scattn_h2p<3, 2>), grid, dim3(256), 0, s, q, k, v, fus, cc.tail_wst_h2, vecs, out, N, tiles, wpp, cc.dense,
-                       W, n_full, ksplits, cc.part_o, cc.part_ml, cc.next_wst_h2, cc.next_bias, cc.ptab, (const unsigned*)nullptr, cc.qf_img, cc.qw_wst, cc.qw_bias, PvGuard{});
+                       W, n_full, ksplits, cc.part_o, cc.part_ml, cc.next_wst_h2, cc.next_bias, cc.ptab, (const unsigned*)nullptr, cc.qf_img, cc.qw_wst, cc.qw_bias, PvGuard{}, HeadFuse{});
   else if (cc.v_scale)
     hipLaunchKernelGGL((k_scattn_h2p<3, 0, true>), grid, dim3(256), 0, s, q, k, v, fus, cc.tail_wst_h2, vecs, out, N, tiles, wpp, cc.dense,
-                       W, n_full, ksplits, cc.part_o, cc.part_ml, cc.next_wst_h2, cc.next_bias, cc.ptab, cc.v_scale, cc.qf_img, cc.qw_wst, cc.qw_bias, cc.guard);
+                       W, n_full, ksplits, cc.part_o, cc.part_ml, cc.next_wst_h2, cc.next_bias, cc.ptab, cc.v_scale, cc.qf_img, cc.qw_wst, cc.qw_bias, cc.guard, cc.head);
   else
     hipLaunchKernelGGL((k_scattn_h2p<3, 0>), grid, dim3(256), 0, s, q, k, v, fus, cc.tail_wst_h2, vecs, out, N, tiles, wpp, cc.dense,
-                       W, n_full, ksplits, cc.part_o, cc.part_ml, cc.next_wst_h2, cc.next_bias, cc.ptab, (const unsigned*)nullptr, cc.qf_img, cc.qw_wst, cc.qw_bias, PvGuard{});
-  if (max_tail > 0)
-    hipLaunchKernelGGL(k_scattn_merge, dim3(8 * max_tail), dim3(256), 0, s, cc.part_o, cc.part_ml, fus, cc.tail_wst_h2, vecs, out,
+                       W, n_full, ksplits, cc.part_o, cc.part_ml, cc.next_wst_h2, cc.next_bias, cc.ptab, (const unsigned*)nullptr, cc.qf_img, cc.qw_wst, cc.qw_bias, PvGuard{}, cc.head);
+  if (max_tail > 0 && cc.head.wst)
+    hipLaunchKernelGGL(k_scattn_merge<true>, dim3(8 * max_tail), dim3(256), 0, s, cc.part_o, cc.part_ml, fus, cc.tail_wst_h2, vecs,
+                       (float*)nullptr, tiles, wpp, W, n_full, ksplits, (const float*)nullptr, (const float*)nullptr, (const float*)nullptr, 0,
+                       (const float*)nullptr, (const float*)nullptr, (unsigned*)nullptr, N, cc.ptab, cc.head);
+  else if (max_tail > 0)
+    hipLaunchKernelGGL(k_scattn_merge<false>, dim3(8 * max_tail), dim3(256), 0, s, cc.part_o, cc.part_ml, fus, cc.tail_wst_h2, vecs, out,
                        tiles, wpp, W, n_full, ksplits, cc.next_wst_h2, cc.next_bias, (const float*)nullptr, 0,
-                       (const float*)nullptr, (const float*)nullptr, cc.guard.stat_next, N, cc.ptab);
+                       (const float*)nullptr, (const float*)nullptr, cc.guard.stat_next, N, cc.ptab, HeadFuse{});
   return hipGetLastError();
 }
 
@@ -2100,12 +2232,13 @@
   return hipGetLastError();
 }
 
-hipError_t launch_seed_dist(const float* featn_img, const int* seeds, float* dist, int B, int N, int S, hipStream_t s, const PairTab* ptab) {
+hipError_t launch_seed_dist(const float* featn_img, const int* seeds, float* dist, int B, int N, int S, hipStream_t s, const PairTab* ptab,
+                            unsigned long long* zero_word) {
   const int tiles = (N + 31) / 32;
   const int sblocks = (S + 127) / 128;
   int chunks = 1;
   while (chunks < 16 && sblocks * B * chunks < 1024 && tiles / (2 * chunks) >= 4) chunks *= 2;
-  hipLaunchKernelGGL(k_seed_dist, dim3(sblocks, B * chunks), dim3(256), 0, s, featn_img, seeds, dist, N, tiles, S, chunks, ptab);
+  hipLaunchKernelGGL(k_seed_dist, dim3(sblocks, B * chunks), dim3(256), 0, s, featn_img, seeds, dist, N, tiles, S, chunks, ptab, zero_word);
   return hipGetLastError();
 }
 
diff --git a/gmf_amd/csrc/gmf_api.cpp b/gmf_amd/csrc/gmf_api.cpp
--- a/gmf_amd/csrc/gmf_api.cpp
+++ b/gmf_amd/csrc/gmf_api.cpp
@@ -251,6 +251,11 @@
     t.precision = value;
     return GMF_OK;
   }
+  if (std::strcmp(name, "fused_head") == 0) {
+    GMF_REQUIRE(value == 0 || value == 1, GMF_ERR_BAD_ARG, "set_tuning: fused_head must be 0 or 1");
+    t.fused_head = value != 0;
+    return GMF_OK;
+  }
   if (std::strcmp(name, "spectral_col_splits") == 0) {
     GMF_REQUIRE(value >= 0 && value <= gmf::kSmMaxSplits, GMF_ERR_BAD_ARG, "set_tuning: spectral_col_splits out of range (0..32)");
     t.spectral_col_splits = value;
@@ -269,7 +274,8 @@
       {"fused_linear", t.fused_linear ? 1 : 0}, {"compat_cache", t.use_cache ? 1 : 0}, {"conv_lds_patch", t.conv_patch}, {"conv_small_grid", t.conv_small ? 1 : 0}, {"small_prologue_roles", t.small_prologue ? 1 : 0}, {"small_fattn_tile", t.small_fattn_tile ? 1 : 0},
       {"nms_binned", t.nms_binned}, {"topk_select", t.topk_select ? 1 : 0}, {"wide_attn_tile", t.wide_attn_tile ? 1 : 0},
       {"small_merge_tile", t.small_merge_tile ? 1 : 0}, {"mid_grid_roles", t.mid_grid_roles}, {"pv_fp8", t.pv_fp8}, {"q_in_attention", t.q_in_attention ? 1 : 0},
-      {"compat_format", t.compat_format}, {"precision", t.precision}, {"spectral_col_splits", t.spectral_col_splits}};
+      {"compat_format", t.compat_format}, {"precision", t.precision}, {"spectral_col_splits", t.spectral_col_splits},
+      {"fused_head", t.fused_head ? 1 : 0}};
   for (const auto& e : tab) {
     if (std::strcmp(name, e.name) == 0) { *value = e.v; return GMF_OK; }
   }
@@ -649,7 +655,20 @@
 
 static int encoder_forward_impl(gmf_handle* h, const gmf_encoder_weights* w, const float* corr_pos, const float* src_keypts,
                                 const float* tgt_keypts, const float* p_tokens, const float* q_tokens, int B, int N, int T,
-                                float* logits, float* feat_n, float* feat, gmf_stream_t stream, const int* n_points);
+                                float* logits, float* feat_n, float* feat, gmf_stream_t stream, const int* n_points,
+                                float* seed_img = nullptr, float* nms_keys = nullptr);
+
+long long gmf_seed_image_floats(int B, int N) { return (B > 0 && N > 0) ? (long long)B * tiles_of(N) * kTileFloats : 0; }
+
+int gmf_encoder_forward_seeded(gmf_handle* h, const gmf_encoder_weights* w, const float* corr_pos, const float* src_keypts,
+                               const float* tgt_keypts, const float* p_tokens, const float* q_tokens, int B, int N, int T,
+                               float* logits, float* feat_n, float* feat, float* seed_img, float* nms_keys, gmf_stream_t stream) {
+  GMF_REQUIRE(h, GMF_ERR_BAD_ARG, "encoder_forward_seeded: null handle");
+  GMF_REQUIRE(seed_img, GMF_ERR_BAD_ARG, "encoder_forward_seeded: null seed_img (gmf_encoder_forward is the call without one)");
+  GMF_REQUIRE(B > 0 && N > 0 && T > 0, GMF_ERR_UNSUPPORTED_SHAPE, "encoder_forward_seeded: empty input");
+  return encoder_forward_impl(h, w, corr_pos, src_keypts, tgt_keypts, p_tokens, q_tokens, B, N, T, logits, feat_n, feat, stream, nullptr,
+                              seed_img, nms_keys);
+}
 
 int gmf_encoder_forward(gmf_handle* h, const gmf_encoder_weights* w, const float* corr_pos, const float* src_keypts,
                         const float* tgt_keypts, const float* p_tokens, const float* q_tokens, int B, int N, int T,
@@ -670,7 +689,8 @@
 
 static int encoder_forward_impl(gmf_handle* h, const gmf_encoder_weights* w, const float* corr_pos, const float* src_keypts,
                                 const float* tgt_keypts, const float* p_tokens, const float* q_tokens, int B, int N, int T,
-                                float* logits, float* feat_n, float* feat, gmf_stream_t stream, const int* n_points) {
+                                float* logits, float* feat_n, float* feat, gmf_stream_t stream, const int* n_points,
+                                float* seed_img, float* nms_keys) {
   if (int rc = check_weights(h, w)) return rc;
   GMF_REQUIRE(corr_pos && src_keypts && tgt_keypts && p_tokens && q_tokens && logits && feat_n, GMF_ERR_BAD_ARG,
               "encoder_forward: null pointer");
@@ -749,12 +769,21 @@
 
   float* cur = featA;
   float* nxt = featB;
+  auto seed_image = [&]() -> int {
+    if (!seed_img) return GMF_OK;
+    GMF_HIP(gmf::launch_pack_rows_h2(feat_n, seed_img, B, N, st, ptab, nms_keys ? logits : nullptr, nms_keys, nms_keys ? (long)B * N : 0));
+    return GMF_OK;
+  };
   if (p.fused()) {
     if (!p.prologue) {
       gmf::PvGuard g0;
       if (p.guard) g0.stat_next = fstat;
       GMF_HIP(gmf::launch_front_h2(3, p.front_split, corr_pos, w->front_wst_h2, w->front_vec, f, q, k, v, B, N, tiles, st, ptab, nullptr, g0));
     }
+    gmf::HeadFuse head{w->head_wst, w->head_vec, logits, feat_n, feat, seed_img, nms_keys, h->status_dev,
+                       p.guard ? fstat : nullptr, p.guard ? w->pv_guard : nullptr, L, B};
+    const bool head_fused = h->tune.fused_head && L > 0 && p.pipelined && p.form != EncoderPlan::kSmall3 &&
+                            gmf::scattn_h2p_fuses_head(cc);
     for (int l = 0; l < L; ++l) {
       cc.guard = gmf::PvGuard{};
       if (p.guard) cc.guard = gmf::PvGuard{fstat + (size_t)l * B * gmf::kPvStatStride, w->pv_guard + l, fstat + (size_t)(l + 1) * B * gmf::kPvStatStride};
@@ -766,6 +795,7 @@
       const float* ffv = w->ff_vec + (size_t)l * w->ff_vec_stride;
       const float* ctx_l = ctxall + (size_t)l * tok;
       const bool last = (l + 1 == L);
+      cc.head = (last && head_fused) ? head : gmf::HeadFuse{};
       cc.tail_wst_h2 = w->tail_wst_h2 + (size_t)l * w->tail_wst_stride;
       cc.next_wst_h2 = last ? nullptr : w->front_wst_h2 + (size_t)(l + 1) * w->front_wst_stride;
       cc.next_bias = last ? nullptr : w->front_vec + (size_t)(l + 1) * w->front_vec_stride;
@@ -791,9 +821,10 @@
       }
       if (int rc = run_scattn(h, w, p, l, q, k, v, pts8, x2, last ? cur : f, B, N, st, nullptr, cc)) return rc;
     }
+    if (head_fused) return GMF_OK;
     GMF_HIP(gmf::launch_head(cur, w->head_wst, w->head_vec, logits, feat_n, feat, B, N, tiles, st, h->status_dev, ptab,
                              p.guard ? fstat : nullptr, p.guard ? w->pv_guard : nullptr, L));
-    return GMF_OK;
+    return seed_image();
   }
   if (L == 0) {
     GMF_HIP(gmf::launch_front(1, corr_pos, w->front_wst, w->front_vec, cur, q, k, v, B, N, tiles, st));
@@ -810,7 +841,7 @@
     float* t = cur; cur = nxt; nxt = t;
   }
   GMF_HIP(gmf::launch_head(cur, w->head_wst, w->head_vec, logits, feat_n, feat, B, N, tiles, st, h->status_dev));
-  return GMF_OK;
+  return seed_image();
 }
 
 int gmf_nonlocal_block_forward(gmf_handle* h, const gmf_encoder_weights* w, int layer, int apply_pointcn,
@@ -926,7 +957,19 @@
 static int pose_head_impl(gmf_handle* h, const gmf_pose_params* p, const float* feat_n, const float* src_keypts,
                           const float* tgt_keypts, const float* logits, const int* seeds_in, int B, int N, float* final_trans,
                           float* final_labels, int* seeds_out, int* knn_out, float* seed_trans, float* fitness,
-                          gmf_stream_t stream, const int* n_points, double ratio);
+                          gmf_stream_t stream, const int* n_points, double ratio, const float* seed_img = nullptr,
+                          float* nms_keys = nullptr);
+
+int gmf_pose_head_seeded(gmf_handle* h, const gmf_pose_params* p, const float* feat_n, const float* src_keypts,
+                         const float* tgt_keypts, const float* logits, const int* seeds_in, int B, int N, const float* seed_img,
+                         float* nms_keys, float* final_trans, float* final_labels, int* seeds_out, int* knn_out, float* seed_trans,
+                         float* fitness, gmf_stream_t stream) {
+  GMF_REQUIRE(h && p, GMF_ERR_BAD_ARG, "pose_head_seeded: null pointer");
+  GMF_REQUIRE(seed_img, GMF_ERR_BAD_ARG, "pose_head_seeded: null seed_img (gmf_pose_head is the call without one)");
+  GMF_REQUIRE(B > 0 && N > 1, GMF_ERR_UNSUPPORTED_SHAPE, "pose_head_seeded: need N > 1");
+  return pose_head_impl(h, p, feat_n, src_keypts, tgt_keypts, logits, seeds_in, B, N, final_trans, final_labels, seeds_out, knn_out,
+                        seed_trans, fitness, stream, nullptr, 0.0, seed_img, nms_keys);
+}
 
 int gmf_pose_head(gmf_handle* h, const gmf_pose_params* p, const float* feat_n, const float* src_keypts,
                   const float* tgt_keypts, const float* logits, const int* seeds_in, int B, int N, float* final_trans,
@@ -953,7 +996,7 @@
 static int pose_head_impl(gmf_handle* h, const gmf_pose_params* p, const float* feat_n, const float* src_keypts,
                           const float* tgt_keypts, const float* logits, const int* seeds_in, int B, int N, float* final_trans,
                           float* final_labels, int* seeds_out, int* knn_out, float* seed_trans, float* fitness,
-                          gmf_stream_t stream, const int* n_points, double ratio) {
+                          gmf_stream_t stream, const int* n_points, double ratio, const float* seed_img, float* nms_keys) {
   GMF_REQUIRE(feat_n && src_keypts && tgt_keypts && final_trans && final_labels, GMF_ERR_BAD_ARG, "pose_head: null pointer");
   GMF_REQUIRE(seeds_in || logits, GMF_ERR_BAD_ARG, "pose_head: need logits or seeds_in");
   const bool ragged = n_points != nullptr;
@@ -981,14 +1024,16 @@
   int *seeds, *knn, *counts, *best, *stop_it;
   unsigned char* conv;
   double* hsum;
+  unsigned long long* stop_word;
   gmf::PairTab* ptab;
-  if (int rc = arena_carve(h, {arena_buf(fimg, (size_t)B * tiles_of(N) * kTileFloats),
+  if (int rc = arena_carve(h, {arena_buf(fimg, seed_img ? 0 : (size_t)B * tiles_of(N) * kTileFloats),
                                arena_buf(dmat, BS * tiles_of(N) * 32),
-                               arena_buf(keys, (size_t)B * N), arena_buf(seeds, BS), arena_buf(knn, BS * k),
+                               arena_buf(keys, nms_keys ? 0 : (size_t)B * N), arena_buf(seeds, BS), arena_buf(knn, BS * k),
                                arena_buf(snaps, BS * iters * k), arena_buf(conv, BS * iters), arena_buf(sT, BS * 16),
                                arena_buf(counts, BS), arena_buf(fit, BS), arena_buf(best, (size_t)B), arena_buf(hsum, BS * 15),
-                               arena_buf(stop_it, 1), arena_buf(ptab, ragged ? (size_t)B : 0)}))
+                               arena_buf(stop_it, 1), arena_buf(stop_word, 1), arena_buf(ptab, ragged ? (size_t)B : 0)}))
     return rc;
+  if (!(h->tune.fused_head && B > 1 && !ragged)) stop_word = nullptr;
   if (ragged) {
     if (int rc = upload_pair_table(h, ptab, B, st)) return rc;
     if (seeds_out) GMF_HIP(hipMemsetAsync(seeds_out, 0, BS * sizeof(int), st));
@@ -1003,13 +1048,16 @@
 
   const int* seeds_use = seeds_in;
   const bool preset = !seeds_in && p->use_nms;
-  GMF_HIP(gmf::launch_pack_rows_h2(feat_n, fimg, B, N, st, ptab, preset ? logits : nullptr, preset ? keys : nullptr,
-                                   preset ? (ptab ? (long)n_sum : (long)B * N) : 0));
+  const float* fimg_use = seed_img ? seed_img : fimg;
+  if (nms_keys) keys = nms_keys;
+  if (!seed_img)
+    GMF_HIP(gmf::launch_pack_rows_h2(feat_n, fimg, B, N, st, ptab, preset ? logits : nullptr, preset ? keys : nullptr,
+                                     preset ? (ptab ? (long)n_sum : (long)B * N) : 0));
   if (!seeds_in) {
     const float* kk = logits;
     if (p->use_nms) {
       float* scr = (BS * N >= gmf::nms_scratch_floats(B, N)) ? dmat : nullptr;
-      GMF_HIP(gmf::launch_nms_keys(h->tune, src_keypts, logits, keys, B, N, p->nms_radius, st, scr, ptab, (long)n_sum, true));
+      GMF_HIP(gmf::launch_nms_keys(h->tune, src_keypts, logits, keys, B, N, p->nms_radius, st, scr, ptab, (long)n_sum, !seed_img || nms_keys));
       kk = keys;
     }
     GMF_HIP(gmf::launch_sort_topk(h->tune, kk, seeds, B, N, Sn, st, ptab));
@@ -1017,10 +1065,11 @@
   } else if (seeds_out) {
     GMF_HIP(hipMemcpyAsync(seeds_out, seeds_in, BS * sizeof(int), hipMemcpyDeviceToDevice, st));
   }
-  GMF_HIP(gmf::launch_seed_dist(fimg, seeds_use, dmat, B, N, Sn, st, ptab));
+  GMF_HIP(gmf::launch_seed_dist(fimg_use, seeds_use, dmat, B, N, Sn, st, ptab, stop_word));
   GMF_HIP(gmf::launch_knn_seeds(feat_n, seeds_use, dmat, knn, B, N, Sn, k, st, ptab));
-  GMF_HIP(gmf::launch_seed_power(feat_n, src_keypts, tgt_keypts, knn, snaps, conv, hsum, B, N, Sn, k, iters, p->sigma, p->sigma_d, st, ptab, h->sigma_dev));
-  GMF_HIP(gmf::launch_seed_kabsch(src_keypts, tgt_keypts, knn, snaps, conv, sT, B, N, Sn, k, iters, hsum, stop_it, st, ptab));
+  GMF_HIP(gmf::launch_seed_power(feat_n, src_keypts, tgt_keypts, knn, snaps, conv, hsum, B, N, Sn, k, iters, p->sigma, p->sigma_d, st, ptab, h->sigma_dev,
+                                 stop_word));
+  GMF_HIP(gmf::launch_seed_kabsch(src_keypts, tgt_keypts, knn, snaps, conv, sT, B, N, Sn, k, iters, hsum, stop_it, st, ptab, stop_word));
   GMF_HIP(gmf::launch_score_hyp(src_keypts, tgt_keypts, sT, counts, B, N, Sn, p->inlier_threshold, st, ptab));
   GMF_HIP(gmf::launch_finalize_pose(src_keypts, tgt_keypts, sT, counts, fit, final_trans, final_labels, best, B, N, Sn,
                                     p->inlier_threshold, p->refine_threshold, p->refine_iters, st, ptab));
diff --git a/gmf_amd/csrc/launchers.hpp b/gmf_amd/csrc/launchers.hpp
--- a/gmf_amd/csrc/launchers.hpp
+++ b/gmf_amd/csrc/launchers.hpp
@@ -10,6 +10,20 @@
   const unsigned* stat = nullptr;
   const float* thr2 = nullptr;
   unsigned* stat_next = nullptr;
+};
+
+struct HeadFuse {
+  const float* wst = nullptr;
+  const float* vecs = nullptr;
+  float* logits = nullptr;
+  float* feat_n = nullptr;
+  float* feat_rm = nullptr;
+  float* seed_img = nullptr;
+  float* keys = nullptr;
+  int* status = nullptr;
+  const unsigned* pv_stat = nullptr;
+  const float* pv_thr2 = nullptr;
+  int n_layers = 0, n_pairs = 0;
 };
 
 struct CompatCache {
@@ -27,6 +41,7 @@
   const float* qw_wst = nullptr;
   const float* qw_bias = nullptr;
   PvGuard guard;
+  HeadFuse head;
 };
 
 struct Tuning {
@@ -51,6 +66,7 @@
   int pv_fp8 = 1;
   int compat_format = 0;
   int precision = 0;
+  bool fused_head = true;
   int spectral_col_splits = 0;
 };
 
@@ -65,6 +81,7 @@
                             const float* vecs, float* out, int B, int N, int tiles, float sigma_d, hipStream_t s, const float* c_dense);
 hipError_t launch_scattn_h2p(const float* q, const float* k, const float* v, const float* fus, const float* vecs, float* out, int B,
                              int N, int tiles, hipStream_t s, const CompatCache& cc, int n_full, int ksplits);
+bool scattn_h2p_fuses_head(const CompatCache& cc);
 hipError_t launch_scattn_dense(const float* q, const float* k, const float* v, const float* compat, const float* fus,
                                const float* wst, const float* vecs, float* out, int B, int N, int tiles, hipStream_t s);
 hipError_t launch_ctx_prep(bool pe, const float* ctx, const float* wst, const float* vecs, float* out, int B, int T,
@@ -127,7 +144,8 @@
 hipError_t launch_nn_match_batched(const float* F0, const float* F1, float* f0_img, float* f1_img, float* norm2, unsigned long long* best,
                                    const MatchPair* tab, int B, const MatchTotals& tot, int d, int mode, int global_index, int* idx,
                                    float* dist, hipStream_t s);
-hipError_t launch_seed_dist(const float* featn_img, const int* seeds, float* dist, int B, int N, int S, hipStream_t s, const PairTab* ptab = nullptr);
+hipError_t launch_seed_dist(const float* featn_img, const int* seeds, float* dist, int B, int N, int S, hipStream_t s, const PairTab* ptab = nullptr,
+                            unsigned long long* zero_word = nullptr);
 hipError_t launch_pack_p32(const float* src, float* dst, int B, int n_rows, int K, long sb, long sr, long sk, hipStream_t s, const PairTab* ptab = nullptr);
 hipError_t launch_pack_rows_h2(const float* src, float* dst, int B, int n_rows, hipStream_t s, const PairTab* ptab = nullptr,
                                const float* copy_src = nullptr, float* copy_dst = nullptr, long n_copy = 0);
diff --git a/gmf_amd/csrc/launchers_pose.hpp b/gmf_amd/csrc/launchers_pose.hpp
--- a/gmf_amd/csrc/launchers_pose.hpp
+++ b/gmf_amd/csrc/launchers_pose.hpp
@@ -14,10 +14,12 @@
                             int k, hipStream_t s, const PairTab* ptab = nullptr);
 hipError_t launch_seed_power(const float* feat_n , const float* src, const float* tgt, const int* knn_idx, float* snaps,
                              unsigned char* conv, double* hsum, int B, int N, int S, int k, int iters, float sigma,
-                             float sigma_d, hipStream_t s, const PairTab* ptab = nullptr, const float* sigma_dev = nullptr);
+                             float sigma_d, hipStream_t s, const PairTab* ptab = nullptr, const float* sigma_dev = nullptr,
+                             unsigned long long* stop_word = nullptr);
 hipError_t launch_seed_kabsch(const float* src, const float* tgt, const int* knn_idx, const float* snaps,
                               const unsigned char* conv, float* seed_T, int B, int N, int S, int k, int iters,
-                              const double* hsum, int* stop_scratch, hipStream_t s, const PairTab* ptab = nullptr);
+                              const double* hsum, int* stop_scratch, hipStream_t s, const PairTab* ptab = nullptr,
+                              const unsigned long long* stop_word = nullptr);
 hipError_t launch_stop_iteration(const unsigned char* conv, int B, int S, int iters, int* stop_out, hipStream_t s);
 hipError_t launch_score_hyp(const float* src, const float* tgt, const float* seed_T, int* counts, int B, int N, int S,
                             float tau, hipStream_t s, const PairTab* ptab = nullptr);
diff --git a/gmf_amd/csrc/pose_kernels.hip b/gmf_amd/csrc/pose_kernels.hip
--- a/gmf_amd/csrc/pose_kernels.hip
+++ b/gmf_amd/csrc/pose_kernels.hip
@@ -691,7 +691,7 @@
 k_seed_power(const float* __restrict__ feat_n, const float* __restrict__ src, const float* __restrict__ tgt,
              const int* __restrict__ knn_idx, float* __restrict__ snaps, unsigned char* __restrict__ conv,
              double* __restrict__ hsum, int N, int S, int k, int iters, float inv_sigma2, float inv_sigmad2,
-             const PairTab* __restrict__ ptab, const float* __restrict__ sigma_dev) {
+             const PairTab* __restrict__ ptab, const float* __restrict__ sigma_dev, unsigned long long* __restrict__ stop_word) {
   inv_sigma2 = sigma_inv2(inv_sigma2, sigma_dev);
   extern __shared__ __attribute__((aligned(16))) float seed_smem[];
   float* const P = seed_smem;
@@ -787,6 +787,7 @@
   float last = 1.0f;
   float* sn = snaps + ((size_t)pair * S + s) * iters * k;
   unsigned char* cv = conv + ((size_t)pair * S + s) * iters;
+  unsigned long long not_close = 0;
   auto power = [&](auto kk_tag) {
     constexpr int KK = decltype(kk_tag)::value;
     float mrow[KK];
@@ -810,12 +811,16 @@
       __syncthreads();
       if (a < k) { vec[a] = v; sn[it * k + a] = v; }
       if (a == 0) cv[it] = all_close ? 1 : 0;
+      if (!all_close) not_close |= 1ull << it;
       last = v;
       __syncthreads();
     }
   };
   if (k <= 40) power(std::integral_constant<int, 40>{});
   else power(std::integral_constant<int, 64>{});
+  if (stop_word && a == 0 && not_close &&
+      (__hip_atomic_load(stop_word, __ATOMIC_RELAXED, __HIP_MEMORY_SCOPE_AGENT) & not_close) != not_close)
+    __hip_atomic_fetch_or(stop_word, not_close, __ATOMIC_RELAXED, __HIP_MEMORY_SCOPE_AGENT);
   if (!hsum) return;
   {
     float sv = 0.f;
@@ -884,14 +889,22 @@
 k_seed_kabsch(const float* __restrict__ src, const float* __restrict__ tgt, const int* __restrict__ knn_idx,
               const float* __restrict__ snaps, const unsigned char* __restrict__ conv, float* __restrict__ seed_T,
               int N, int S, int k, int iters, const double* __restrict__ hsum, const int* __restrict__ stop_batch,
-              const PairTab* __restrict__ ptab) {
+              const PairTab* __restrict__ ptab, const unsigned long long* __restrict__ stop_word) {
   __shared__ int stop_it;
   const int pair = blockIdx.y;
   const int S_p = pair_seeds(ptab, pair, S);
   if ((int)blockIdx.x * 64 >= S_p) return;
   if (threadIdx.x == 0) stop_it = iters - 1;
   __syncthreads();
-  if (stop_batch) {
+  if (stop_word) {
+    if (threadIdx.x == 0) {
+      const unsigned long long bad = *stop_word;
+      int first = iters - 1;
+      for (int it = 0; it < iters - 1; ++it)
+        if (!((bad >> it) & 1ull)) { first = it; break; }
+      stop_it = first;
+    }
+  } else if (stop_batch) {
     if (threadIdx.x == 0) stop_it = *stop_batch;
   } else {
     const unsigned char* cv = conv + (size_t)pair * S * iters;
@@ -1529,24 +1542,26 @@
 
 hipError_t launch_seed_power(const float* feat_n, const float* src, const float* tgt, const int* knn_idx, float* snaps,
                              unsigned char* conv, double* hsum, int B, int N, int S, int k, int iters, float sigma,
-                             float sigma_d, hipStream_t s, const PairTab* ptab, const float* sigma_dev) {
+                             float sigma_d, hipStream_t s, const PairTab* ptab, const float* sigma_dev, unsigned long long* stop_word) {
   if (k > kKMax) return hipErrorInvalidValue;
   const size_t lds_bytes = (size_t)(kKMax * 8 + kKMax + k * (k + 1)) * sizeof(float);
   hipLaunchKernelGGL(k_seed_power, dim3(S, B), dim3(64), lds_bytes, s, feat_n, src, tgt, knn_idx, snaps, conv, hsum, N, S, k,
-                     iters, 1.0f / (sigma * sigma), 1.0f / (sigma_d * sigma_d), ptab, sigma_dev);
+                     iters, 1.0f / (sigma * sigma), 1.0f / (sigma_d * sigma_d), ptab, sigma_dev, stop_word);
   return hipGetLastError();
 }
 
 hipError_t launch_seed_kabsch(const float* src, const float* tgt, const int* knn_idx, const float* snaps,
                               const unsigned char* conv, float* seed_T, int B, int N, int S, int k, int iters,
-                              const double* hsum, int* stop_scratch, hipStream_t s, const PairTab* ptab) {
+                              const double* hsum, int* stop_scratch, hipStream_t s, const PairTab* ptab,
+                              const unsigned long long* stop_word) {
   const int* stop_batch = nullptr;
-  if (B > 1 && stop_scratch && !ptab) {
+  if (B <= 1 || ptab) stop_word = nullptr;
+  if (B > 1 && stop_scratch && !ptab && !stop_word) {
     hipLaunchKernelGGL(k_stop_iteration, dim3(1), dim3(1024), 0, s, conv, B * S, iters, stop_scratch);
     stop_batch = stop_scratch;
   }
   hipLaunchKernelGGL(k_seed_kabsch, dim3((S + 63) / 64, B), dim3(64), 0, s, src, tgt, knn_idx, snaps, conv, seed_T, N, S, k, iters,
-                     hsum, stop_batch, ptab);
+                     hsum, stop_batch, ptab, stop_word);
   return hipGetLastError();
 }
 
diff --git a/gmf_amd/pointdsc.py b/gmf_amd/pointdsc.py
--- a/gmf_amd/pointdsc.py
+++ b/gmf_amd/pointdsc.py
@@ -412,7 +412,17 @@
             for knob, val in prev.items():
                 h.call("gmf_set_tuning", knob, val)
 
-    def encode(self, corr_pos, src_keypts, tgt_keypts, p_tokens, q_tokens, want_features=False):
+    def _seed_buffers(self, dev, B, N, keys):
+        cache = self.__dict__.setdefault("_seed_cache", {})
+        key = (str(dev), B, N)
+        if key not in cache:
+            cache.clear()
+            n_img = int(_lib.load_library().gmf_seed_image_floats(B, N))
+            cache[key] = (torch.empty(n_img, device=dev), torch.empty((B, N), device=dev))
+        img, k = cache[key]
+        return img, (k if keys else None)
+
+    def encode(self, corr_pos, src_keypts, tgt_keypts, p_tokens, q_tokens, want_features=False, seed_buffers=None):
         if self.training:
             raise RuntimeError("gmf_amd.PointDSC.encode is the eval() inference path (BatchNorm folded from running statistics); in train() "
                                "mode call the module with autograd enabled (the differentiable forward), or call eval() first")
@@ -435,6 +445,12 @@
         feat_n = torch.empty((B, N, 128), device=dev)
         feat = torch.empty((B, N, 128), device=dev) if want_features else None
         h, st = handle_and_stream(corr_pos, check=True)
+        if seed_buffers is not None:
+            img, keys = seed_buffers
+            self._call_tuned(h, "gmf_encoder_forward_seeded", pw.struct, corr_pos.data_ptr(), src.data_ptr(), tgt.data_ptr(),
+                             p_tokens.data_ptr(), q_tokens.data_ptr(), B, N, T, logits.data_ptr(), feat_n.data_ptr(),
+                             None if feat is None else feat.data_ptr(), img.data_ptr(), None if keys is None else keys.data_ptr(), st)
+            return logits, feat_n, feat
         self._call_tuned(h, "gmf_encoder_forward", pw.struct, corr_pos.data_ptr(), src.data_ptr(), tgt.data_ptr(),
                          p_tokens.data_ptr(), q_tokens.data_ptr(), B, N, T, logits.data_ptr(), feat_n.data_ptr(),
                          None if feat is None else feat.data_ptr(), st)
@@ -455,7 +471,7 @@
         pp.refine_threshold = 0.10 if self.inlier_threshold == 0.10 else 1.2
         return pp, S, k
 
-    def pose_head(self, feat_n, src_keypts, tgt_keypts, logits, testing, seeds=None, return_aux=False, sigmas=None):
+    def pose_head(self, feat_n, src_keypts, tgt_keypts, logits, testing, seeds=None, return_aux=False, sigmas=None, seed_buffers=None):
         B, N, _ = feat_n.shape
         pp, S, k = self._pose_params(N, testing, sigmas, feat_n.device)
         dev = feat_n.device
@@ -468,10 +484,15 @@
                    "seed_trans": torch.empty((B, S, 4, 4), device=dev), "fitness": torch.empty((B, S), device=dev)}
         seeds_in = None if seeds is None else seeds.to(torch.int32).contiguous()
         h, st = handle_and_stream(feat_n)
-        h.call("gmf_pose_head", pp, feat_n.data_ptr(), src_keypts.data_ptr(), tgt_keypts.data_ptr(), logits.data_ptr(),
-               None if seeds_in is None else seeds_in.data_ptr(), B, N, final_T.data_ptr(), labels.data_ptr(),
-               seeds_out.data_ptr(), aux["knn_idx"].data_ptr() if return_aux else None,
-               aux["seed_trans"].data_ptr() if return_aux else None, aux["fitness"].data_ptr() if return_aux else None, st)
+        outs = (final_T.data_ptr(), labels.data_ptr(), seeds_out.data_ptr(), aux["knn_idx"].data_ptr() if return_aux else None,
+                aux["seed_trans"].data_ptr() if return_aux else None, aux["fitness"].data_ptr() if return_aux else None, st)
+        ins = (pp, feat_n.data_ptr(), src_keypts.data_ptr(), tgt_keypts.data_ptr(), logits.data_ptr(),
+               None if seeds_in is None else seeds_in.data_ptr(), B, N)
+        if seed_buffers is not None:
+            img, keys = seed_buffers
+            h.call("gmf_pose_head_seeded", *ins, img.data_ptr(), None if keys is None else keys.data_ptr(), *outs)
+        else:
+            h.call("gmf_pose_head", *ins, *outs)
         aux["seeds"] = seeds_out
         return final_T, labels, aux
 
@@ -572,11 +593,13 @@
                 else:
                     p_tok, q_tok = self.encoder.image_tokens(p_img), self.encoder.image_tokens(q_img)
         with torch.no_grad():
-            logits, feat_n, feat = self.encode(corr_pos, src_keypts, tgt_keypts, p_tok, q_tok, want_features=not testing)
+            B, N = corr_pos.shape[0], corr_pos.shape[1]
+            bufs = self._seed_buffers(corr_pos.device, B, N, keys=testing) if N > 1 else None
+            logits, feat_n, feat = self.encode(corr_pos, src_keypts, tgt_keypts, p_tok, q_tok, want_features=not testing, seed_buffers=bufs)
             self.last_logits, self.last_features = logits, feat_n
             src = src_keypts.contiguous()
             tgt = tgt_keypts.contiguous()
-            final_trans, labels, _ = self.pose_head(feat_n, src, tgt, logits, testing)
+            final_trans, labels, _ = self.pose_head(feat_n, src, tgt, logits, testing, seed_buffers=bufs)
             M = None
             if not testing:
                 M = similarity_matrix(feat_n, self._weights(feat_n.device).sigma)
diff --git a/include/gmf_hip.h b/include/gmf_hip.h
--- a/include/gmf_hip.h
+++ b/include/gmf_hip.h
@@ -120,6 +120,11 @@
                         const float* tgt_keypts, const float* p_tokens, const float* q_tokens, int B, int N, int T,
                         float* logits, float* feat_n, float* feat, gmf_stream_t stream);
 
+long long gmf_seed_image_floats(int B, int N);
+int gmf_encoder_forward_seeded(gmf_handle* h, const gmf_encoder_weights* w, const float* corr_pos, const float* src_keypts,
+                               const float* tgt_keypts, const float* p_tokens, const float* q_tokens, int B, int N, int T,
+                               float* logits, float* feat_n, float* feat, float* seed_img, float* nms_keys, gmf_stream_t stream);
+
 int gmf_encoder_forward_ragged(gmf_handle* h, const gmf_encoder_weights* w, const float* corr_pos, const float* src_keypts,
                                const float* tgt_keypts, const float* p_tokens, const float* q_tokens, const int* n_points, int B,
                                int T, float* logits, float* feat_n, float* feat, gmf_stream_t stream);
@@ -151,6 +156,11 @@
                   const float* tgt_keypts, const float* logits, const int* seeds_in, int B, int N, float* final_trans,
                   float* final_labels, int* seeds_out, int* knn_out, float* seed_trans, float* fitness,
                   gmf_stream_t stream);
+
+int gmf_pose_head_seeded(gmf_handle* h, const gmf_pose_params* p, const float* feat_n, const float* src_keypts,
+                         const float* tgt_keypts, const float* logits, const int* seeds_in, int B, int N, const float* seed_img,
+                         float* nms_keys, float* final_trans, float* final_labels, int* seeds_out, int* knn_out, float* seed_trans,
+                         float* fitness, gmf_stream_t stream);
 
 int gmf_pose_head_ragged(gmf_handle* h, const gmf_pose_params* p, double ratio, const float* feat_n, const float* src_keypts,
                          const float* tgt_keypts, const float* logits, const int* n_points, int B, float* final_trans,
```

Measured after the change: 9.774 million (median of 6 runs). No clear change (+0.1%).
